# Rainbowboys/fm_spark

Hardware: AMD Instinct MI355X
Metric: FM SGD train samples/sec at k=16, 1/8 GPUs; % of HBM roofline (higher is better)
Workload: dtype f32; 1 GPU; c3: synthetic hashed 100M features, 39 nnz/row, k=16, batch 256K; num_features=100000000, k=16, batch_rows_per_gpu=262144, global_batch=262144, launch=single

## Files before the change

### fm_spark_amd/_native.py

```python

from __future__ import annotations

import ctypes as C
import os
from pathlib import Path

import numpy as np

_LIB_PATH = Path(__file__).resolve().parent / "lib" / "libfm_hip.so"

FM_OK = 0
FM_NOTHING_TO_DO = 1
FM_PARALLEL_NONE, FM_PARALLEL_SHARDED, FM_PARALLEL_REPLICATED = 0, 1, 2
FM_TRANSPORT_AUTO, FM_TRANSPORT_RCCL, FM_TRANSPORT_COPY = 0, 1, 2
FM_MAX_LOCAL = 16
FM_FUSE_DEFAULT, FM_FUSE_ON, FM_FUSE_OFF = 0, 1, -1
FM_WIRE_FP32, FM_WIRE_FP64 = 0, 1
FM_RANK_MAX_TOP = 1024
FM_RANK_SELECT_ALL, FM_RANK_SELECT_ONLY, FM_RANK_SELECT_EXCEPT = 0, 1, 2


class FMError(RuntimeError):
    """A negative return code of the C-ABI, with fm_last_error()'s message."""


class fm_config(C.Structure):
    _fields_ = [
        ("num_features", C.c_int64),
        ("k", C.c_int32),
        ("device", C.c_int32),
        ("seed", C.c_uint64),
        ("init_sd", C.c_double),
        ("w0", C.c_double),
        ("shard_index", C.c_int32),
        ("shard_count", C.c_int32),
        ("parallel", C.c_int32),
        ("n_gpus", C.c_int32),
        ("devices", C.c_int32 * FM_MAX_LOCAL),
        ("transport", C.c_int32),
        ("n_procs", C.c_int32),
        ("proc_rank", C.c_int32),
        ("comm_id", C.c_uint8 * 128),
        ("fuse_single", C.c_int32),
        ("xchg_chunks", C.c_int32),
        ("wire", C.c_int32),
    ]


class fm_csr(C.Structure):
    _fields_ = [
        ("n_rows", C.c_int64),
        ("nnz", C.c_int64),
        ("row_ptr", C.POINTER(C.c_int64)),
        ("col", C.POINTER(C.c_int32)),
        ("val", C.POINTER(C.c_double)),
        ("label", C.POINTER(C.c_double)),
    ]


class fm_step_out(C.Structure):
    _fields_ = [
        ("loss_sum", C.c_double),
        ("n_rows", C.c_int64),
        ("n_loss_rows", C.c_int64),
        ("n_unique", C.c_int64),
    ]


class fm_eval_out(C.Structure):
    _fields_ = [
        ("n_rows", C.c_int64),
        ("n_unlearned", C.c_int64),
        ("epoch", C.c_int64),
        ("sum_err", C.c_double),
        ("sum_abs_err", C.c_double),
        ("sum_sq_err", C.c_double),
    ]


_P = C.c_void_p
_I64P = C.POINTER(C.c_int64)
_I32P = C.POINTER(C.c_int32)
_DP = C.POINTER(C.c_double)

SIGNATURES = {
    "fm_create": (C.c_int, [C.POINTER(fm_config), C.POINTER(_P)]),
    "fm_destroy": (None, [_P]),
    "fm_last_error": (C.c_char_p, []),
    "fm_comm_unique_id": (C.c_int, [C.POINTER(C.c_uint8)]),
    "fm_set_stream": (C.c_int, [_P, _P]),
    "fm_sync": (C.c_int, [_P]),
    "fm_reserve": (C.c_int, [_P, C.c_int64, C.c_int64]),
    "fm_load_tables": (C.c_int, [_P, _I32P, C.c_int64, _DP, _DP]),
    "fm_init_random": (C.c_int, [_P, _I32P, C.c_int64]),
    "fm_init_random_range": (C.c_int, [_P, C.c_int64, C.c_int64]),
    "fm_export_tables": (C.c_int, [_P, _I32P, _DP, _DP, C.c_int64, _I64P]),
    "fm_export_rows": (C.c_int, [_P, _I32P, C.c_int64, _DP, _DP, C.POINTER(C.c_int8)]),
    "fm_num_present": (C.c_int64, [_P]),
    "fm_epoch": (C.c_int64, [_P]),
    "fm_batch_create": (C.c_int, [_P, C.POINTER(fm_csr), C.POINTER(_P)]),
    "fm_batch_destroy": (None, [_P]),
    "fm_batch_prepare": (C.c_int, [_P, _P]),
    "fm_batch_from_rows": (C.c_int, [_P, _P, _I64P, C.c_int64, C.POINTER(_P)]),
    "fm_batch_create_splits": (C.c_int, [_P, C.POINTER(fm_csr), C.c_int32, _I64P, C.POINTER(_P)]),
    "fm_batch_layout_splits": (C.c_int, [_P, C.POINTER(fm_csr), C.c_int32, _I64P, _I64P, C.POINTER(_P)]),
    "fm_batch_split_view": (C.c_int, [_P, _P, C.c_int32, C.POINTER(_P)]),
    "fm_fuse_active": (C.c_int32, [_P]),
    "fm_batch_rows": (C.c_int64, [_P]),
    "fm_batch_nnz": (C.c_int64, [_P]),
    "fm_step": (C.c_int, [_P, C.POINTER(fm_csr), C.c_int32, C.c_double, C.c_double, C.POINTER(fm_step_out)]),
    "fm_step_batch": (C.c_int, [_P, _P, C.c_int32, C.c_double, C.c_double, C.POINTER(fm_step_out)]),
    "fm_loss_history": (C.c_int, [_P, _DP, C.c_int64, _I64P]),
    "fm_predict": (C.c_int, [_P, C.POINTER(fm_csr), C.c_double, C.c_double, _DP]),
    "fm_predict_batch": (C.c_int, [_P, _P, C.c_double, C.c_double, _DP]),
    "fm_evaluate": (C.c_int, [_P, C.POINTER(fm_csr), C.c_double, C.c_double, _DP, C.POINTER(fm_eval_out)]),
    "fm_evaluate_batch": (C.c_int, [_P, _P, C.c_double, C.c_double, _DP, C.POINTER(fm_eval_out)]),
    "fm_eval_history": (C.c_int, [_P, C.POINTER(fm_eval_out), C.c_int64, _I64P]),
    "fm_rank_candidates": (C.c_int, [_P, C.POINTER(fm_csr), C.POINTER(fm_csr), C.c_int32, C.c_double, C.c_double,
                                     _I32P, _DP]),
    "fm_rank_batch": (C.c_int, [_P, _P, _P, C.c_int32, C.c_double, C.c_double, _I32P, _DP]),
    "fm_rank_candidates_select": (C.c_int, [_P, C.POINTER(fm_csr), C.POINTER(fm_csr), C.c_int32, _I64P, _I32P, C.c_int32,
                                            C.c_double, C.c_double, _I32P, _DP]),
    "fm_rank_batch_select": (C.c_int, [_P, _P, _P, C.c_int32, _I64P, _I32P, C.c_int32, C.c_double, C.c_double, _I32P,
                                       _DP]),
    "fm_rank_positions": (C.c_int, [_P, C.POINTER(fm_csr), C.POINTER(fm_csr), _I64P, _I32P, _I64P, _I32P, C.c_double,
                                    C.c_double, _I32P, _DP]),
    "fm_rank_positions_batch": (C.c_int, [_P, _P, _P, _I64P, _I32P, _I64P, _I32P, C.c_double, C.c_double, _I32P, _DP]),
    "fm_init_from_batch": (C.c_int, [_P, _P, _I64P]),
    "fm_loss_grad": (C.c_int, [_P, C.POINTER(fm_csr), _DP, _DP, _DP, _DP]),
    "fm_calc_loss_grad": (C.c_int, [_P, C.POINTER(fm_csr), C.c_double, C.c_uint64, _DP, _DP, _DP, _DP]),
    "fm_vector_sum_by_key": (C.c_int, [_P, _I32P, C.c_int64, _DP, C.c_int32, _I32P, _DP, _I64P]),
    "fm_profile_enable": (C.c_int, [_P, C.c_int32]),
    "fm_profile_read": (C.c_int, [_P, C.c_char_p, C.c_int64, _DP, _I64P, C.c_int64, _I64P]),
    "fm_profile_reset": (C.c_int, [_P]),
    "fm_device_bytes_live": (C.c_int64, []),
    "fm_device_allocs_live": (C.c_int64, []),
    "fm_read_libsvm": (C.c_int, [C.c_char_p, C.c_int64, C.c_int64, _DP, _I64P, _I32P, _DP, _I64P, _I64P, _I64P]),
    "fm_random_split": (
        C.c_int,
        [C.c_int32, _I64P, C.c_char_p, _DP, C.POINTER(C.c_int8), _I32P, _I64P, _I32P, _DP, _I64P,
         C.c_int32, _DP, C.c_int64, _I32P, _I64P, _I64P],
    ),
    "fm_xorshift_hash_seed": (C.c_int64, [C.c_int64]),
    "fm_murmur3_bytes_hash": (C.c_int32, [C.POINTER(C.c_uint8), C.c_int64, C.c_int32]),
    "fm_xorshift_next_doubles": (C.c_int, [C.c_int64, C.c_int64, _DP]),
    "fm_set_side_stream": (C.c_int, [_P, _P]),
    "fm_shard_route": (C.c_int, [_P, _P, _P, _P, _I64P]),
    "fm_shard_owner_prepare": (C.c_int, [_P, _P, _P, _P, C.c_int64, _I64P, _I64P]),
    "fm_shard_owner_forward": (C.c_int, [_P, _P, _P]),
    "fm_shard_combine": (C.c_int, [_P, _P, _P, _P]),
    "fm_shard_owner_update": (C.c_int, [_P, _P, _P, C.c_int32, C.c_double, C.c_double, C.c_int64]),
    "fm_repl_grad": (C.c_int, [_P, _P, _P]),
    "fm_repl_apply": (C.c_int, [_P, _P, C.c_int32, C.c_double, C.c_double, C.c_int64]),
    "fm_last_stats": (C.c_int, [_P, _DP, _I64P, _I64P]),
}

_lib = None


def lib_path() -> Path:
    return _LIB_PATH


def load() -> C.CDLL:
    global _lib
    if _lib is not None:
        return _lib
    path = Path(os.environ.get("FM_HIP_LIB") or _LIB_PATH)
    if not path.exists():
        raise FMError(f"{path} is missing: run __graft_entry__.build() (hipcc, gfx950)")
    if os.environ.get("FM_NO_TORCH_PRELOAD") != "1":
        try:
            import torch
        except Exception:
            pass
    lib = C.CDLL(str(path), mode=C.RTLD_GLOBAL)
    for name, (res, args) in SIGNATURES.items():
        fn = getattr(lib, name)
        fn.restype = res
        fn.argtypes = args
    _lib = lib
    return lib


def check(rc: int, what: str = "") -> int:
    if rc < 0:
        msg = load().fm_last_error()
        raise FMError(f"{what} failed ({rc}): {msg.decode() if msg else ''}")
    return rc


def ptr(a: np.ndarray, ctype):
    return a.ctypes.data_as(C.POINTER(ctype))


class CSRHost:

    def __init__(self, row_ptr, col, val, label):
        self.row_ptr = np.ascontiguousarray(row_ptr, dtype=np.int64)
        self.col = np.ascontiguousarray(col, dtype=np.int32)
        self.val = np.ascontiguousarray(val, dtype=np.float64)
        self.label = np.ascontiguousarray(label, dtype=np.float64)
        if len(self.row_ptr) == 0:
            self.row_ptr = np.zeros(1, dtype=np.int64)
        self.c = fm_csr(
            n_rows=len(self.label),
            nnz=len(self.col),
            row_ptr=ptr(self.row_ptr, C.c_int64),
            col=ptr(self.col, C.c_int32),
            val=ptr(self.val, C.c_double),
            label=ptr(self.label, C.c_double),
        )

    @property
    def n_rows(self) -> int:
        return len(self.label)

    @property
    def nnz(self) -> int:
        return len(self.col)
```

### fm_spark_amd/csrc/fm_capi.hip

```cpp
#include <algorithm>
#include <chrono>
#include <cstdlib>
#include <cmath>
#include <cstring>
#include <atomic>
#include <condition_variable>
#include <cstdio>
#include <functional>
#include <map>
#include <memory>
#include <set>
#include <thread>
#include <utility>

#include "fm_context.h"
#include "fm_hostpool.h"

namespace fmhip {

static thread_local std::string g_last_error;
void set_error(const std::string& msg) { g_last_error = msg; }

void report_stale(hipError_t e) {
  if (e == hipSuccess) return;
// ... 21 lines not shown
  if (p && !borrowed) {
    (void)hipFree(p);
    g_dev_bytes_live.fetch_sub((int64_t)bytes, std::memory_order_relaxed);
    g_dev_allocs_live.fetch_sub(1, std::memory_order_relaxed);
  }
  p = nullptr;
  bytes = 0;
  borrowed = false;
}

static int64_t chunk_count(int64_t n, int64_t min_per_thread) {
  return std::max<int64_t>(1, std::min<int64_t>(HostPool::get().threads(), n / std::max<int64_t>(min_per_thread, 1)));
}

template <class F>
static void parallel_chunks_t(int64_t n, int64_t T, F&& f) {
  if (T <= 1) {
    f(int64_t(0), int64_t(0), n);
    return;
  }
  const std::function<void(int)> job = [&](int t) { f((int64_t)t, n * t / T, n * (t + 1) / T); };
  HostPool::get().run((int)T, job);
}

template <class F>
static void parallel_chunks(int64_t n, int64_t min_per_thread, F&& f) {
  parallel_chunks_t(n, chunk_count(n, min_per_thread), [&](int64_t, int64_t lo, int64_t hi) { f(lo, hi); });
}

static bool selection_row_ptr(const int64_t* hrp, int64_t Bd, const int64_t* rows, int64_t n, int64_t* hrows,
                              int64_t* rp) {
  rp[0] = 0;
  const int64_t T = chunk_count(n, 8192);
  std::vector<int64_t> tot(T + 1, 0);
  std::atomic<int> bad{0};
  parallel_chunks_t(n, T, [&](int64_t t, int64_t lo, int64_t hi) {
    int64_t acc = 0;
    for (int64_t i = lo; i < hi; ++i) {
      const int64_t r = rows[i];
      if (r < 0 || r >= Bd) {
        bad.store(1);
        return;
      }
      hrows[i] = r;
      acc += hrp[r + 1] - hrp[r];
      rp[i + 1] = acc;
    }
    tot[t + 1] = acc;
  });
  if (bad.load()) return false;
  for (int64_t t = 0; t < T; ++t) tot[t + 1] += tot[t];
  if (T > 1)
    parallel_chunks_t(n, T, [&](int64_t t, int64_t lo, int64_t hi) {
      const int64_t add = tot[t];
      if (add)
        for (int64_t i = lo; i < hi; ++i) rp[i + 1] += add;
    });
  return true;
}

struct Staged {
  int64_t B = 0, N = 0, M = 0, max_id = -1, max_len = 0;
  size_t o_lab = 0, o_xoff = 0, o_col = 0, o_x = 0, bytes = 0;
  size_t o_extra = 0;
  int nruns = 0;
  int64_t run_at[16] = {0}, run_n[16] = {0};
  CsrImage view(void* base) const {
    char* p = reinterpret_cast<char*>(base);
    return {reinterpret_cast<int64_t*>(p), reinterpret_cast<double*>(p + o_lab), reinterpret_cast<int32_t*>(p + o_xoff),
            reinterpret_cast<uint32_t*>(p + o_col), reinterpret_cast<float*>(p + o_x)};
  }
  void enqueue_copies(void* dev, const void* pin, hipStream_t st) const {
    FM_HIP_CHECK(hipMemcpyAsync(dev, pin, bytes, hipMemcpyHostToDevice, st));
    for (int r = 0; r < nruns; ++r)
      if (run_n[r] > 0)
        FM_HIP_CHECK(hipMemcpyAsync(reinterpret_cast<char*>(dev) + o_x + sizeof(float) * run_at[r],
                                    reinterpret_cast<const char*>(pin) + o_x + sizeof(float) * run_at[r],
                                    sizeof(float) * run_n[r], hipMemcpyHostToDevice, st));
  }
};

void check_csr(const fm_csr* c) {
  FM_REQUIRE(c != nullptr, "null fm_csr");
  FM_REQUIRE(c->n_rows >= 0 && c->nnz >= 0, "negative n_rows / nnz");
  FM_REQUIRE(c->n_rows < (int64_t(1) << 31), "n_rows must be < 2^31");
  FM_REQUIRE(c->nnz < (int64_t(1) << 31), "nnz must be < 2^31 per batch");
  FM_REQUIRE(c->n_rows == 0 || (c->row_ptr && c->label), "null row_ptr / label");
  FM_REQUIRE(c->nnz == 0 || (c->col && c->val), "null col / val");
  const int64_t B = c->n_rows;
  if (B > 0) {
    FM_REQUIRE(c->row_ptr[0] == 0, "row_ptr[0] must be 0");
    FM_REQUIRE(c->row_ptr[B] == c->nnz, "row_ptr[n_rows] must equal nnz");
    for (int64_t i = 0; i < B; ++i) FM_REQUIRE(c->row_ptr[i] <= c->row_ptr[i + 1], "row_ptr must be non-decreasing");
  } else {
    FM_REQUIRE(c->nnz == 0, "nnz > 0 with n_rows == 0");
  }
}

static Staged stage_csr(fm_ctx* ctx, const fm_csr* c, bool check_range, Pinned& pin, size_t extra = 0) {
  check_csr(c);
  Staged g;
  const int64_t B = c->n_rows, N = c->nnz;
  g.B = B;
  g.N = N;
  g.o_lab = sizeof(int64_t) * (B + 1);
  g.o_xoff = g.o_lab + sizeof(double) * B;
  g.o_col = (g.o_xoff + sizeof(int32_t) * B + 15) / 16 * 16;
  g.o_x = (g.o_col + sizeof(uint32_t) * N + 15) / 16 * 16;
  g.o_extra = (g.o_x + sizeof(float) * N + 16 + 15) / 16 * 16;
  pin.ensure_slack(g.o_extra + extra);
  const CsrImage im = g.view(pin.p);
  if (B > 0) std::memcpy(im.row_ptr, c->row_ptr, sizeof(int64_t) * (B + 1));
  else im.row_ptr[0] = 0;
  const int64_t F = ctx->cfg.num_features;
  std::atomic<int> bad{0};
  std::atomic<int64_t> mx{-1}, mlen{0};
  std::atomic<int> nrun{0};
  parallel_chunks(B, 4096, [&](int64_t r0, int64_t r1) {
    const int64_t x0 = B > 0 ? c->row_ptr[r0] : 0;
    int64_t lmx = -1, m = x0, llen = 0;
    int lbad = 0;
    for (int64_t i = r0; i < r1; ++i) {
      im.label[i] = c->label[i];
      llen = std::max<int64_t>(llen, c->row_ptr[i + 1] - c->row_ptr[i]);
      im.xoff[i] = (int32_t)m;
      for (int64_t e = c->row_ptr[i]; e < c->row_ptr[i + 1]; ++e) {
        const int32_t id = c->col[e];
        if (id < 0) lbad |= 1;
        else if (check_range && id >= F) lbad |= 2;
        const float x = (float)c->val[e];
        const uint32_t valued = x != 1.0f;
        im.col[e] = (uint32_t)id | (valued << 31);
        im.x[m] = x;
        m += valued;
        lmx = std::max<int64_t>(lmx, id);
      }
    }
    const int ri = nrun.fetch_add(1);
    g.run_at[ri] = x0;
    g.run_n[ri] = m - x0;
    if (lbad) bad.fetch_or(lbad);
    int64_t cur = mx.load();
    while (lmx > cur && !mx.compare_exchange_weak(cur, lmx)) {
    }
    cur = mlen.load();
    while (llen > cur && !mlen.compare_exchange_weak(cur, llen)) {
    }
  });
  FM_REQUIRE(!(bad.load() & 1), "negative feature id");
  FM_REQUIRE(!(bad.load() & 2), "feature id >= num_features");
  g.nruns = nrun.load();
  for (int r = 0; r < g.nruns; ++r) g.M += g.run_n[r];
  g.bytes = g.o_col + sizeof(uint32_t) * N;
  g.max_id = mx.load();
  g.max_len = mlen.load();
  return g;
}

bool fuse_rule(const fm_ctx* ctx) {
  if (ctx->cfg.fuse_single == FM_FUSE_OFF || ctx->kp > 16) return false;
  const double table_bytes = (double)ctx->rows * ctx->stride * sizeof(float);
  return ctx->cfg.fuse_single == FM_FUSE_ON || table_bytes > 256.0 * 1024 * 1024;
}

static bool fuse_on(const fm_ctx* ctx) { return ctx->cfg.shard_count == 1 && fuse_rule(ctx); }

static bool batch_fits(const fm_batch* b, const Staged& g) {
  const BatchBytes z = batch_bytes(g.B, g.N);
  return b->dev.row_ptr.bytes >= z.row_ptr && b->dev.col.bytes >= z.col && b->dev.ent.bytes >= z.ent &&
         b->dev.xs.bytes >= z.xs && b->dev.label.bytes >= z.label && b->up.bytes >= g.o_x + sizeof(float) * g.N + 16;
}

static void copy_staged(fm_ctx* ctx, const Staged& g, const Pinned& pin, fm_batch* b, hipStream_t st) {
  b->owner = ctx;
  b->device = ctx->cfg.device;
  b->max_id = g.max_id;
  size_batch(b->dev, g.B, g.N);
  b->up.ensure_slack(g.o_x + sizeof(float) * g.N + 16);
  g.enqueue_copies(b->up.p, pin.p, st);
  launch_explode(g.view(b->up.p), g.B, g.N, b->dev, st);
}

void upload_batch(fm_ctx* ctx, const fm_csr* c, fm_batch* b, bool check_range) {
  FM_HIP_CHECK(hipStreamSynchronize(ctx->stream));
  const Staged g = stage_csr(ctx, c, check_range, ctx->up_pin);
  copy_staged(ctx, g, ctx->up_pin, b, ctx->stream);
  FM_HIP_CHECK(hipStreamSynchronize(ctx->stream));
}

fm_batch* host_batch(fm_ctx* ctx) {
  if (!ctx->host_batch) ctx->host_batch.reset(new fm_batch());
  return ctx->host_batch.get();
}

OutBatch out_batch(fm_ctx* ctx, const fm_batch* data, fm_batch** out, bool group) {
  OutBatch o;
  o.out = out;
  o.b = *out;
  if (o.b == nullptr) {
    o.fresh.reset(group ? new_group_batch(ctx) : new fm_batch());
    o.b = o.fresh.get();
    o.b->owner = ctx;
    o.b->device = ctx->cfg.device;
  } else {
    FM_REQUIRE(o.b->owner == ctx && o.b != data && !o.b->grp == !group && o.b->split_rows.empty(),
               "out must be a batch of this context other than data");
  }
  return o;
}

void wait_built(const fm_batch* b, hipStream_t st) {
  if (b->built) FM_HIP_CHECK(hipStreamWaitEvent(st, b->built, 0));
}

double* eval_next_slot(fm_ctx* ctx) {
  ctx->ensure_eval_hist(ctx->eval_n + 1);
  return ctx->eval_hist.as<double>() + kEvalRec * ctx->eval_n;
}

void eval_read(const double* rec, int64_t epoch, fm_eval_out* out) {
  out->n_rows = (int64_t)rec[0];
  out->n_unlearned = (int64_t)rec[1];
  out->epoch = epoch;
  out->sum_err = rec[2];
  out->sum_abs_err = rec[3];
  out->sum_sq_err = rec[4];
}

void eval_commit(fm_ctx* ctx, fm_eval_out* out) {
  const double* slot = ctx->eval_hist.as<double>() + kEvalRec * ctx->eval_n;
  ctx->eval_epoch.push_back(ctx->epoch);
  ctx->eval_n += 1;
  if (!out) return;
  ctx->pinned.ensure(64);
  FM_HIP_CHECK(hipMemcpyAsync(ctx->pinned.p, slot, sizeof(double) * kEvalRec, hipMemcpyDeviceToHost, ctx->stream));
  FM_HIP_CHECK(hipStreamSynchronize(ctx->stream));
  eval_read(reinterpret_cast<const double*>(ctx->pinned.p), ctx->epoch, out);
}

void reserve_work(fm_ctx* ctx, int64_t B, int64_t N) {
  StepWork& w = ctx->work;
  w.S.ensure_slack(sizeof(float) * (size_t)std::max<int64_t>(B, 1) * s_rec_floats(ctx->kp));
  w.yl.ensure_slack(sizeof(float2) * (size_t)std::max<int64_t>(B, 1));
  w.sort.ensure(std::max<int64_t>(N, 1));
  const int64_t nranges = (N + 255) / 256;
  w.part.ensure_slack(sizeof(double) * (size_t)std::max<int64_t>(nranges, 1) * 2 * (ctx->kp + 2));
  w.ucnt.ensure_slack(sizeof(uint32_t) * (size_t)std::max<int64_t>((N + 1023) / 1024, 1));
  w.loss_part.ensure(sizeof(double2) * kLossPartBlocks);
}

}

namespace {

int step_impl(fm_ctx* ctx, fm_batch* b, int32_t t, double step_size, double reg_param, fm_step_out* out,
              float* emit = nullptr) {
  FM_REQUIRE(b != nullptr, "null batch");
  FM_REQUIRE(b->owner == ctx, "batch belongs to another context");
  FM_REQUIRE(ctx->cfg.shard_count == 1, "sharded contexts step through the fm_shard_* entry points");
  FM_REQUIRE(b->split_rows.empty(), "a dataset made by fm_batch_create_splits is stepped through its split views");
  if (emit) FM_HIP_CHECK(hipMemsetAsync(emit, 0, sizeof(float) * (size_t)ctx->rows * (ctx->kp + 4), ctx->stream));
  if (b->dev.n_rows == 0) return FM_NOTHING_TO_DO;
  FM_REQUIRE(t >= 1, "iteration index t must be >= 1");
  FM_REQUIRE(std::isfinite(step_size) && std::isfinite(reg_param), "non-finite step size / regParam");
  const int64_t B = b->dev.n_rows, N = b->dev.nnz;
  reserve_work(ctx, B, N);
  ctx->ensure_hist(ctx->epoch + 1);
  StepParams p;
  p.n_rows = B;
  p.eta = step_size / std::sqrt((double)t);
  p.lam = p.eta * reg_param;
  p.m = (double)B;
  p.scale_v = p.eta / (double)B;
  p.epoch = ctx->epoch;
  p.cumE = ctx->cum_host.back();
  p.cum_next = p.cumE + p.lam;
  p.w0 = ctx->cfg.w0;
  const TableView T = ctx->view();
  wait_built(b, ctx->stream);
  int64_t nfwd = 0;
  const uint32_t* skeys = nullptr;
  const uint2* sents = nullptr;
  const bool prepared = b->prepared;
  const bool fused = prepared && b->split;
  FM_REQUIRE(!(fused && emit), "a batch prepared for the fused step cannot feed fm_repl_grad");
  FM_REQUIRE(ctx->epoch < (1 << 29), "epoch count beyond the multi tags' range (2^29 steps)");
  if (prepared) {
    skeys = b->skeys.as<uint32_t>();
    sents = b->sents.as<uint2>();
  } else {
    FM_HIP_CHECK(hipEventRecord(ctx->ev_fork, ctx->stream));
    FM_HIP_CHECK(hipStreamWaitEvent(ctx->side, ctx->ev_fork, 0));
    hipEvent_t es = ctx->prof_begin(ctx->side);
    radix_sort_pairs64(ctx->work.sort, b->dev.col.as<uint32_t>(), b->dev.ent.as<uint2>(), N, bits_for(ctx->rows - 1),
                       ctx->side, &skeys, &sents);
    ctx->prof_end("sort", es, ctx->side);
    FM_HIP_CHECK(hipEventRecord(ctx->ev_join, ctx->side));
  }
  hipEvent_t e0 = nullptr;
  FwdOut fx{};
  if (fused) {
    FM_HIP_CHECK(hipStreamWaitEvent(ctx->stream, b->ready, 0));
    e0 = ctx->prof_begin(ctx->stream);
    launch_split(b->fkeys.as<uint32_t>(), b->fents.as<uint2>(), N, ctx->split_work, b->skeys.as<uint32_t>(),
                 b->sents.as<uint2>(), b->split_n.as<int64_t>(), ctx->stream, T, p.epoch);
    ctx->prof_end("split", e0, ctx->stream);
    fx.mode = kTrainFused;
  }
  e0 = ctx->prof_begin(ctx->stream);
  launch_forward(T, b->dev, ctx->work, p, ctx->stream, &nfwd, nullptr, fused ? &fx : nullptr);
  ctx->prof_end("forward", e0, ctx->stream);
  if (!fused) FM_HIP_CHECK(hipStreamWaitEvent(ctx->stream, prepared ? b->ready : ctx->ev_join, 0));
  e0 = ctx->prof_begin(ctx->stream);
  double* stats = ctx->loss_hist.as<double>() + 3 * (int64_t)ctx->epoch;
  launch_segment_update(T, b->dev, ctx->work, p, skeys, sents, nfwd, stats, ctx->stream, emit,
                        fused ? b->split_n.as<int64_t>() : nullptr);
  if (!prepared) FM_HIP_CHECK(hipEventRecord(ctx->ev_upd_done, ctx->stream));
  if (b->last_use) FM_HIP_CHECK(hipEventRecord(b->last_use, ctx->stream));
  b->prepared = false;
  ctx->prof_end("update", e0, ctx->stream);
  if (emit) return FM_OK;
  ctx->epoch += 1;
  ctx->cum_host.push_back(p.cum_next);
  if (out) {
    ctx->pinned.ensure(64);
    FM_HIP_CHECK(hipMemcpyAsync(ctx->pinned.p, stats, sizeof(double) * 3, hipMemcpyDeviceToHost, ctx->stream));
    FM_HIP_CHECK(hipStreamSynchronize(ctx->stream));
    const double* h = reinterpret_cast<const double*>(ctx->pinned.p);
    out->loss_sum = h[0];
    out->n_loss_rows = (int64_t)h[1];
    out->n_unique = (int64_t)h[2];
    out->n_rows = B;
  }
  return FM_OK;
}

}

extern "C" {

const char* fm_last_error(void) { return g_last_error.c_str(); }

int64_t fm_device_bytes_live(void) { return g_dev_bytes_live.load(std::memory_order_relaxed); }
int64_t fm_device_allocs_live(void) { return g_dev_allocs_live.load(std::memory_order_relaxed); }

int fm_create(const fm_config* cfg, fm_ctx** out) {
  return guarded_free([&]() -> int {
    FM_REQUIRE(cfg && out, "null argument");
    FM_REQUIRE(cfg->wire == FM_WIRE_FP32 || cfg->wire == FM_WIRE_FP64, "wire must be FM_WIRE_FP32 or FM_WIRE_FP64");
    FM_REQUIRE(cfg->wire != FM_WIRE_FP64 || cfg->parallel != FM_PARALLEL_REPLICATED,
               "wire = FM_WIRE_FP64 applies to the sharded step only: the replicated gradient all-reduce is fp32");
    if (cfg->parallel != FM_PARALLEL_NONE) return group_create(cfg, out);
    FM_REQUIRE(cfg->num_features >= 1 && cfg->num_features <= (int64_t(1) << 31), "num_features must be in [1, 2^31]");
    FM_REQUIRE(cfg->k >= 1 && cfg->k <= 256, "dimFactorization must be in [1, 256]");
    FM_REQUIRE(cfg->shard_count >= 1 && cfg->shard_index >= 0 && cfg->shard_index < cfg->shard_count,
               "bad shard_index / shard_count");
    FM_REQUIRE(cfg->init_sd >= 0.0, "init_sd must be >= 0");
    FM_REQUIRE(cfg->fuse_single == FM_FUSE_DEFAULT || cfg->fuse_single == FM_FUSE_ON || cfg->fuse_single == FM_FUSE_OFF,
               "fuse_single must be FM_FUSE_DEFAULT, FM_FUSE_ON or FM_FUSE_OFF");
    int ndev = 0;
    FM_HIP_CHECK(hipGetDeviceCount(&ndev));
    FM_REQUIRE(cfg->device >= 0 && cfg->device < ndev, "device ordinal out of range");
    FM_HIP_CHECK(hipSetDevice(cfg->device));
    std::unique_ptr<fm_ctx> c(new fm_ctx());
    c->cfg = *cfg;
    c->kp = (cfg->k + 3) / 4 * 4;
    c->rows = (cfg->num_features - cfg->shard_index + cfg->shard_count - 1) / cfg->shard_count;
    FM_HIP_CHECK(hipStreamCreateWithFlags(&c->stream, hipStreamNonBlocking));
    c->own_stream = true;
    FM_HIP_CHECK(hipStreamCreateWithFlags(&c->side_own, hipStreamNonBlocking));
    c->side = c->side_own;
    FM_HIP_CHECK(hipEventCreateWithFlags(&c->ev_fork, hipEventDisableTiming));
    FM_HIP_CHECK(hipEventCreateWithFlags(&c->ev_join, hipEventDisableTiming));
    FM_HIP_CHECK(hipEventCreateWithFlags(&c->ev_upd_done, hipEventDisableTiming));
    FM_HIP_CHECK(hipEventRecord(c->ev_upd_done, c->stream));
    c->stride = record_stride(c->kp);
    c->rec.ensure(sizeof(float) * (size_t)std::max<int64_t>(c->rows, 1) * c->stride);
    c->ensure_hist(4096);
    launch_table_reset(c->view(), c->stream);
    FM_HIP_CHECK(hipStreamSynchronize(c->stream));
    *out = c.release();
    return FM_OK;
  });
}

void fm_destroy(fm_ctx* ctx) {
  if (!ctx) return;
  try {
    delete ctx;
  } catch (...) {
  }
}

int fm_set_stream(fm_ctx* ctx, void* s) {
  if (ctx && ctx->group) {
    if (ctx->cfg.n_gpus != 1) {
      set_error("fm_set_stream on a context with several local ranks");
      return FM_ERR_ARG;
    }
    return fm_set_stream(group_member0(ctx), s);
  }
  return guarded(ctx, [&]() -> int {
    FM_HIP_CHECK(hipStreamSynchronize(ctx->stream));
    if (ctx->own_stream && ctx->stream) FM_HIP_CHECK(hipStreamDestroy(ctx->stream));
    ctx->stream = reinterpret_cast<hipStream_t>(s);
    ctx->own_stream = false;
    return FM_OK;
  });
}

int fm_set_side_stream(fm_ctx* ctx, void* s) {
  if (ctx && ctx->group) {
    if (ctx->cfg.n_gpus != 1) {
      set_error("fm_set_side_stream on a context with several local ranks");
      return FM_ERR_ARG;
    }
    return fm_set_side_stream(group_member0(ctx), s);
  }
  return guarded(ctx, [&]() -> int {
    FM_HIP_CHECK(hipStreamSynchronize(ctx->side));
    ctx->side = s ? reinterpret_cast<hipStream_t>(s) : ctx->side_own;
    return FM_OK;
  });
}

int fm_sync(fm_ctx* ctx) {
  return guarded(ctx, [&]() -> int {
    if (ctx->group) return group_sync(ctx);
    FM_HIP_CHECK(hipStreamSynchronize(ctx->stream));
    FM_HIP_CHECK(hipStreamSynchronize(ctx->side));
    if (ctx->copy_stream) FM_HIP_CHECK(hipStreamSynchronize(ctx->copy_stream));
    return FM_OK;
  });
}

int fm_reserve(fm_ctx* ctx, int64_t max_rows, int64_t max_nnz) {
  return guarded(ctx, [&]() -> int {
    FM_REQUIRE(max_rows >= 0 && max_nnz >= 0, "negative reserve");
    if (ctx->group) return group_reserve(ctx, max_rows, max_nnz);
    reserve_work(ctx, max_rows, max_nnz);
    return FM_OK;
  });
}

int fm_load_tables(fm_ctx* ctx, const int32_t* ids, int64_t n, const double* w, const double* V) {
  return guarded(ctx, [&]() -> int {
    FM_REQUIRE(n >= 0, "negative n");
    if (n == 0) return FM_OK;
    if (ctx->group) return group_load_tables(ctx, ids, n, w, V);
    FM_REQUIRE(ids && w && V, "null argument");
    for (int64_t i = 0; i < n; ++i)
      FM_REQUIRE(ids[i] >= 0 && ids[i] < ctx->cfg.num_features, "id out of [0, num_features)");
    DevBuf di, dw, dv;
    di.ensure(sizeof(int32_t) * n);
    dw.ensure(sizeof(double) * n);
    dv.ensure(sizeof(double) * n * ctx->cfg.k);
    FM_HIP_CHECK(hipMemcpy(di.p, ids, sizeof(int32_t) * n, hipMemcpyHostToDevice));
    FM_HIP_CHECK(hipMemcpy(dw.p, w, sizeof(double) * n, hipMemcpyHostToDevice));
    FM_HIP_CHECK(hipMemcpy(dv.p, V, sizeof(double) * n * ctx->cfg.k, hipMemcpyHostToDevice));
    launch_load_rows(ctx->view(), di.as<int32_t>(), n, dw.as<double>(), dv.as<double>(), ctx->epoch,
                     ctx->cum_host.back(), ctx->stream);
    FM_HIP_CHECK(hipStreamSynchronize(ctx->stream));
    return FM_OK;
  });
}

int fm_init_random(fm_ctx* ctx, const int32_t* ids, int64_t n) {
  return guarded(ctx, [&]() -> int {
    FM_REQUIRE(n >= 0, "negative n");
    if (n == 0) return FM_OK;
    FM_REQUIRE(ids, "null ids");
    if (ctx->group) return group_init_random(ctx, ids, n, 0, 0);
    for (int64_t i = 0; i < n; ++i)
      FM_REQUIRE(ids[i] >= 0 && ids[i] < ctx->cfg.num_features, "id out of [0, num_features)");
    DevBuf di;
    di.ensure(sizeof(int32_t) * n);
    FM_HIP_CHECK(hipMemcpy(di.p, ids, sizeof(int32_t) * n, hipMemcpyHostToDevice));
    launch_init_random(ctx->view(), di.as<int32_t>(), n, 0, ctx->cfg.seed, ctx->cfg.init_sd, ctx->epoch,
                       ctx->cum_host.back(), ctx->stream);
    FM_HIP_CHECK(hipStreamSynchronize(ctx->stream));
    return FM_OK;
  });
}

int fm_init_random_range(fm_ctx* ctx, int64_t b, int64_t e) {
  return guarded(ctx, [&]() -> int {
    FM_REQUIRE(b >= 0 && e >= b && e <= ctx->cfg.num_features, "bad id range");
    if (ctx->group) return group_init_random(ctx, nullptr, 0, b, e);
    launch_init_random(ctx->view(), nullptr, e - b, b, ctx->cfg.seed, ctx->cfg.init_sd, ctx->epoch,
                       ctx->cum_host.back(), ctx->stream);
    FM_HIP_CHECK(hipStreamSynchronize(ctx->stream));
    return FM_OK;
  });
}

int64_t fm_num_present(fm_ctx* ctx) {
  int64_t n = -1;
  int rc = guarded(ctx, [&]() -> int {
    if (ctx->group) {
      n = group_num_present(ctx);
      return FM_OK;
    }
    DevBuf d;
    d.ensure(sizeof(int64_t));
    launch_count_present(ctx->view(), d.as<int64_t>(), ctx->stream);
    FM_HIP_CHECK(hipMemcpyAsync(&n, d.p, sizeof(int64_t), hipMemcpyDeviceToHost, ctx->stream));
    FM_HIP_CHECK(hipStreamSynchronize(ctx->stream));
    return FM_OK;
  });
  return rc == FM_OK ? n : rc;
}

int64_t fm_epoch(fm_ctx* ctx) { return ctx ? ctx->epoch : -1; }

int fm_export_tables(fm_ctx* ctx, int32_t* ids, double* w, double* V, int64_t cap, int64_t* n) {
  return guarded(ctx, [&]() -> int {
    FM_REQUIRE(n != nullptr && cap >= 0, "bad arguments");
    if (ctx->group) return group_export_tables(ctx, ids, w, V, cap, n);
    launch_flush(ctx->view(), ctx->epoch, ctx->cum_host.back(), ctx->stream);
    FM_HIP_CHECK(hipStreamSynchronize(ctx->stream));
    const int k = ctx->cfg.k, kp = ctx->kp, S = ctx->stride;
    const int64_t chunk_rows = std::max<int64_t>(1, (int64_t(64) << 20) / (4 * S));
    std::vector<float> hv;
    int64_t cnt = 0, o = 0;
    const bool fill = cap > 0;
    for (int64_t r0 = 0; r0 < ctx->rows; r0 += chunk_rows) {
      const int64_t r1 = std::min(ctx->rows, r0 + chunk_rows);
      hv.resize((size_t)(r1 - r0) * S);
      FM_HIP_CHECK(hipMemcpy(hv.data(), ctx->rec.as<float>() + r0 * S, sizeof(float) * (r1 - r0) * S,
                             hipMemcpyDeviceToHost));
      for (int64_t i = r0; i < r1; ++i) {
        const float* row = hv.data() + (size_t)(i - r0) * S;
        RowHdr hd;
        std::memcpy(&hd, row + kp, sizeof(RowHdr));
        if (hd.t < 0) continue;
        ++cnt;
        if (!fill) continue;
        FM_REQUIRE(o < cap && ids && w && V, "export buffers too small or null");
        ids[o] = (int32_t)(i * ctx->cfg.shard_count + ctx->cfg.shard_index);
        w[o] = hd.w;
        for (int f = 0; f < k; ++f) V[o * k + f] = row[f];
        ++o;
      }
    }
    *n = cnt;
    return FM_OK;
  });
}

int fm_export_rows(fm_ctx* ctx, const int32_t* ids, int64_t n, double* w, double* V, int8_t* present) {
  return guarded(ctx, [&]() -> int {
    FM_REQUIRE(n >= 0, "negative n");
    if (n == 0) return FM_OK;
    FM_REQUIRE(ids && w && V && present, "null argument");
    if (ctx->group) return group_export_rows(ctx, ids, n, w, V, present);
    const int R = ctx->cfg.shard_count;
    for (int64_t i = 0; i < n; ++i) {
      FM_REQUIRE(ids[i] >= 0 && ids[i] < ctx->cfg.num_features, "id out of [0, num_features)");
      FM_REQUIRE(ids[i] % R == ctx->cfg.shard_index, "id not owned by this shard");
    }
    const int k = ctx->cfg.k;
    DevBuf di, dw, dv, dp;
    di.ensure(sizeof(int32_t) * n);
    dw.ensure(sizeof(double) * n);
    dv.ensure(sizeof(double) * n * k);
    dp.ensure(sizeof(int8_t) * n);
    FM_HIP_CHECK(hipMemcpyAsync(di.p, ids, sizeof(int32_t) * n, hipMemcpyHostToDevice, ctx->stream));
    launch_gather_rows(ctx->view(), di.as<int32_t>(), n, ctx->cum_host.back(), dw.as<double>(), dv.as<double>(),
                       dp.as<int8_t>(), ctx->stream);
    FM_HIP_CHECK(hipMemcpyAsync(w, dw.p, sizeof(double) * n, hipMemcpyDeviceToHost, ctx->stream));
    FM_HIP_CHECK(hipMemcpyAsync(V, dv.p, sizeof(double) * n * k, hipMemcpyDeviceToHost, ctx->stream));
    FM_HIP_CHECK(hipMemcpyAsync(present, dp.p, sizeof(int8_t) * n, hipMemcpyDeviceToHost, ctx->stream));
    FM_HIP_CHECK(hipStreamSynchronize(ctx->stream));
    return FM_OK;
  });
}

int fm_batch_create(fm_ctx* ctx, const fm_csr* csr, fm_batch** out) {
  return guarded(ctx, [&]() -> int {
    FM_REQUIRE(out != nullptr, "null out");
    if (ctx->group) return group_batch_create(ctx, csr, out);
    std::unique_ptr<fm_batch> b(new fm_batch());
    upload_batch(ctx, csr, b.get(), true);
    b->host_rp.assign(csr->row_ptr, csr->row_ptr + csr->n_rows + 1);
    *out = b.release();
    return FM_OK;
  });
}

void fm_batch_destroy(fm_batch* b) {
  if (!b) return;
  try {
    delete b;
  } catch (...) {
  }
}

int fm_batch_prepare(fm_ctx* ctx, fm_batch* b) {
  return guarded(ctx, [&]() -> int {
    FM_REQUIRE(b != nullptr && b->owner == ctx, "batch belongs to another context");
    if (ctx->group) return group_batch_prepare(ctx, b);
    FM_REQUIRE(ctx->cfg.shard_count == 1, "fm_batch_prepare is for single-table contexts");
    FM_REQUIRE(b->split_rows.empty(), "a dataset made by fm_batch_create_splits is prepared through its split views");
    const int64_t N = b->dev.nnz;
    if (N == 0) return FM_OK;
    b->ensure_events(ctx->stream);
    b->skeys.ensure_slack(sizeof(uint32_t) * N);
    b->sents.ensure_slack(sizeof(uint2) * N);
    FM_HIP_CHECK(hipStreamWaitEvent(ctx->side, ctx->ev_upd_done, 0));
    FM_HIP_CHECK(hipStreamWaitEvent(ctx->side, b->last_use, 0));
    wait_built(b, ctx->side);
    hipEvent_t es = ctx->prof_begin(ctx->side);
    const uint32_t* sk = nullptr;
    const uint2* sv = nullptr;
    b->split = fuse_on(ctx);
    const int kb = bits_for(ctx->rows - 1);
    const uint32_t* col = b->dev.col.as<uint32_t>();
    const uint2* ent = b->dev.ent.as<uint2>();
    if (b->split) {
      b->split_n.ensure(2 * sizeof(int64_t));
      b->fkeys.ensure_slack(sizeof(uint32_t) * N);
      b->fents.ensure_slack(sizeof(uint2) * N);
      radix_sort_pairs64(ctx->work.sort, col, ent, N, kb, ctx->side, &sk, &sv, b->fkeys.as<uint32_t>(),
                         b->fents.as<uint2>());
    } else {
      radix_sort_pairs64(ctx->work.sort, col, ent, N, kb, ctx->side, &sk, &sv, b->skeys.as<uint32_t>(),
                         b->sents.as<uint2>());
    }
    ctx->prof_end("sort", es, ctx->side);
    FM_HIP_CHECK(hipEventRecord(b->ready, ctx->side));
    b->prepared = true;
    return FM_OK;
  });
}

int fm_batch_from_rows(fm_ctx* ctx, const fm_batch* data, const int64_t* rows, int64_t n, fm_batch** out) {
  return guarded(ctx, [&]() -> int {
    FM_REQUIRE(out != nullptr && data != nullptr, "null argument");
    FM_REQUIRE(data->owner == ctx, "data belongs to another context");
    FM_REQUIRE(n >= 0 && n < (int64_t(1) << 31), "n out of range");
    FM_REQUIRE(n == 0 || rows != nullptr, "null rows");
    if (ctx->group) return group_batch_from_rows(ctx, data, rows, n, out);
    const int64_t Bd = data->dev.n_rows;
    FM_REQUIRE((int64_t)data->host_rp.size() == Bd + 1,
               "data must be a batch made by fm_batch_create");
    OutBatch res = out_batch(ctx, data, out, false);
    fm_batch* b = res.b;
    b->detach_view();
    b->ensure_events(ctx->stream);
    if (!b->built) {
      FM_HIP_CHECK(hipEventCreateWithFlags(&b->built, hipEventDisableTiming));
      FM_HIP_CHECK(hipEventCreateWithFlags(&b->sel_copied, hipEventDisableTiming));
      FM_HIP_CHECK(hipEventRecord(b->sel_copied, ctx->side));
    }
    FM_HIP_CHECK(hipEventSynchronize(b->sel_copied));
    const size_t img = sizeof(int64_t) * (2 * (size_t)n + 1);
    b->sel_pin.ensure_slack(img);
    int64_t* hrows = reinterpret_cast<int64_t*>(b->sel_pin.p);
    int64_t* rp = hrows + n;
    FM_REQUIRE(selection_row_ptr(data->host_rp.data(), Bd, rows, n, hrows, rp), "row index out of [0, rows of data)");
    const int64_t N = rp[n];
    FM_REQUIRE(N < (int64_t(1) << 31), "nnz must be < 2^31 per batch");
    if (!ctx->copy_stream) FM_HIP_CHECK(hipStreamCreateWithFlags(&ctx->copy_stream, hipStreamNonBlocking));
    hipStream_t gs = ctx->copy_stream;
    FM_HIP_CHECK(hipStreamWaitEvent(gs, b->last_use, 0));
    if (b->sh && b->sh->last_use) FM_HIP_CHECK(hipStreamWaitEvent(gs, b->sh->last_use, 0));
    if (b->prepared && b->ready) FM_HIP_CHECK(hipStreamWaitEvent(gs, b->ready, 0));
    b->max_id = data->max_id;
    size_batch(b->dev, n, N);
    b->up.ensure_slack(img + 16);
    FM_HIP_CHECK(hipMemcpyAsync(b->up.p, b->sel_pin.p, img, hipMemcpyHostToDevice, gs));
    FM_HIP_CHECK(hipEventRecord(b->sel_copied, gs));
    if (n > 0) {
      const int64_t* up = b->up.as<int64_t>();
      launch_select_rows(data->dev, up, up + n, n, b->dev, gs);
    } else {
      FM_HIP_CHECK(hipMemcpyAsync(b->dev.row_ptr.p, b->up.as<int64_t>(), sizeof(int64_t), hipMemcpyDeviceToDevice, gs));
    }
    FM_HIP_CHECK(hipEventRecord(b->built, gs));
    b->prepared = false;
    b->host_rp.clear();
    res.commit();
    return FM_OK;
  });
}

int fm_batch_create_splits(fm_ctx* ctx, const fm_csr* csr, int32_t n_splits, const int64_t* split_rows,
                           fm_batch** out) {
  return guarded(ctx, [&]() -> int {
    FM_REQUIRE(out != nullptr && csr != nullptr, "null argument");
    FM_REQUIRE(n_splits >= 1 && split_rows != nullptr, "n_splits must be >= 1");
    FM_REQUIRE(split_rows[0] == 0 && split_rows[n_splits] == csr->n_rows, "split_rows must run from 0 to n_rows");
    for (int32_t i = 0; i < n_splits; ++i) FM_REQUIRE(split_rows[i] <= split_rows[i + 1], "split_rows must be non-decreasing");
    if (ctx->group) return group_batch_create_splits(ctx, csr, n_splits, split_rows, out);
    std::unique_ptr<fm_batch> b(new fm_batch());
    upload_batch(ctx, csr, b.get(), true);
    b->host_rp.assign(csr->row_ptr, csr->row_ptr + csr->n_rows + 1);
    b->split_rows.assign(split_rows, split_rows + n_splits + 1);
    DevBuf dsr;
    dsr.ensure(sizeof(int64_t) * (n_splits + 1));
    FM_HIP_CHECK(hipMemcpyAsync(dsr.p, split_rows, sizeof(int64_t) * (n_splits + 1), hipMemcpyHostToDevice, ctx->stream));
    b->split_rp.ensure(sizeof(int64_t) * (csr->n_rows + n_splits));
    launch_split_rebase(b->dev, dsr.as<int64_t>(), n_splits, b->split_rp.as<int64_t>(), ctx->stream);
    FM_HIP_CHECK(hipStreamSynchronize(ctx->stream));
    *out = b.release();
    return FM_OK;
  });
}

int fm_batch_layout_splits(fm_ctx* ctx, const fm_csr* csr, int32_t n_splits, const int64_t* split_rows,
                           const int64_t* order, fm_batch** out) {
  return guarded(ctx, [&]() -> int {
    FM_REQUIRE(out != nullptr && csr != nullptr, "null argument");
    FM_REQUIRE(n_splits >= 1 && split_rows != nullptr, "n_splits must be >= 1");
    FM_REQUIRE(split_rows[0] == 0, "split_rows must start at 0");
    for (int32_t i = 0; i < n_splits; ++i) FM_REQUIRE(split_rows[i] <= split_rows[i + 1], "split_rows must be non-decreasing");
    const int64_t n = split_rows[n_splits];
    FM_REQUIRE(n < (int64_t(1) << 31), "laid-out rows must be < 2^31");
    FM_REQUIRE(n == 0 || order != nullptr, "null order");
    if (ctx->group) return group_batch_layout_splits(ctx, csr, n_splits, split_rows, order, out);
    std::unique_ptr<fm_batch> b(new fm_batch());
    FM_HIP_CHECK(hipStreamSynchronize(ctx->stream));
    const size_t extra = sizeof(int64_t) * (2 * (size_t)n + 1 + (size_t)n_splits + 1);
    const Staged g = stage_csr(ctx, csr, true, ctx->up_pin, extra);
    const int64_t D = g.B;
    int64_t* hord = reinterpret_cast<int64_t*>(reinterpret_cast<char*>(ctx->up_pin.p) + g.o_extra);
    int64_t* rp = hord + n;
    int64_t* hsr = rp + n + 1;
    FM_REQUIRE(selection_row_ptr(csr->row_ptr, D, order, n, hord, rp), "row index out of [0, n_rows of csr)");
    const int64_t N = rp[n];
    FM_REQUIRE(N < (int64_t(1) << 31), "nnz must be < 2^31 per batch");
    std::copy(split_rows, split_rows + n_splits + 1, hsr);
    hipStream_t st = ctx->stream;
    b->owner = ctx;
    b->device = ctx->cfg.device;
    b->max_id = g.max_id;
    size_batch(b->dev, n, N);
    b->split_rp.ensure(sizeof(int64_t) * (n + n_splits));
    b->up.ensure(g.o_extra + extra);
    g.enqueue_copies(b->up.p, ctx->up_pin.p, st);
    int64_t* dord = reinterpret_cast<int64_t*>(b->up.as<char>() + g.o_extra);
    FM_HIP_CHECK(hipMemcpyAsync(dord, hord, extra, hipMemcpyHostToDevice, st));
    launch_layout_splits(g.view(b->up.p), dord, dord + n, dord + 2 * n + 1, n_splits, n, b->dev, b->split_rp.as<int64_t>(),
                         st);
    b->host_rp.assign(rp, rp + n + 1);
    b->split_rows.assign(split_rows, split_rows + n_splits + 1);
    FM_HIP_CHECK(hipStreamSynchronize(st));
    b->up.release();
    *out = b.release();
    return FM_OK;
  });
}

int fm_batch_split_view(fm_ctx* ctx, const fm_batch* data, int32_t split, fm_batch** out) {
  return guarded(ctx, [&]() -> int {
    FM_REQUIRE(out != nullptr && data != nullptr, "null argument");
    FM_REQUIRE(data->owner == ctx, "data belongs to another context");
    if (ctx->group) return group_batch_split_view(ctx, data, split, out);
    const int64_t ns = (int64_t)data->split_rows.size() - 1;
    FM_REQUIRE(ns >= 1, "data must be a dataset made by fm_batch_create_splits");
    FM_REQUIRE(split >= 0 && split < ns, "split index out of range");
    OutBatch res = out_batch(ctx, data, out, false);
    fm_batch* b = res.b;
    if (!b->view_of) {
      for (hipEvent_t e : {b->last_use, b->ready, b->built, b->sel_copied})
        if (e) FM_HIP_CHECK(hipEventSynchronize(e));
      for (DevBuf* d : {&b->dev.row_ptr, &b->dev.col, &b->dev.ent, &b->dev.xs, &b->dev.label, &b->up}) d->release();
    }
    b->ensure_events(ctx->stream);
    const int64_t r0 = data->split_rows[split], r1 = data->split_rows[split + 1];
    const int64_t e0 = data->host_rp[r0], e1 = data->host_rp[r1];
    b->view_of = data;
    b->dev.n_rows = r1 - r0;
    b->dev.nnz = e1 - e0;
    b->dev.row_ptr.borrow(data->split_rp.as<int64_t>() + r0 + split, sizeof(int64_t) * (r1 - r0 + 1));
    b->dev.col.borrow(data->dev.col.as<uint32_t>() + e0, sizeof(uint32_t) * (e1 - e0));
    b->dev.ent.borrow(data->dev.ent.as<uint2>() + e0, sizeof(uint2) * (e1 - e0));
    b->dev.xs.borrow(data->dev.xs.as<float>() + e0, sizeof(float) * (e1 - e0));
    b->dev.label.borrow(data->dev.label.as<double>() + r0, sizeof(double) * (r1 - r0));
    b->max_id = data->max_id;
    b->prepared = false;
    b->host_rp.clear();
    res.commit();
    return FM_OK;
  });
}

int32_t fm_fuse_active(fm_ctx* ctx) {
  if (!ctx) return -1;
  if (ctx->group) return 0;
  return fuse_on(ctx) ? 1 : 0;
}

int64_t fm_batch_rows(const fm_batch* b) { return b ? b->dev.n_rows : -1; }
int64_t fm_batch_nnz(const fm_batch* b) { return b ? b->dev.nnz : -1; }

int fm_step_batch(fm_ctx* ctx, fm_batch* batch, int32_t t, double step_size, double reg_param,
                  fm_step_out* out) {
  return guarded(ctx, [&]() -> int {
    if (ctx->group) return group_step_batch(ctx, batch, t, step_size, reg_param, out);
    return step_impl(ctx, batch, t, step_size, reg_param, out);
  });
}

int fm_step(fm_ctx* ctx, const fm_csr* csr, int32_t t, double step_size, double reg_param, fm_step_out* out) {
  return guarded(ctx, [&]() -> int {
    FM_REQUIRE(csr != nullptr, "null batch");
    if (csr->n_rows == 0) {
      if (out) {
        out->loss_sum = 0.0;
        out->n_rows = 0;
        out->n_loss_rows = 0;
        out->n_unique = 0;
      }
      if (!ctx->group) return FM_NOTHING_TO_DO;
    }
    if (ctx->group) return group_step(ctx, csr, t, step_size, reg_param, out);
    HostSlot& h = ctx->hslot[ctx->hnext];
    ctx->hnext ^= 1;
    if (!h.batch) {
      h.batch.reset(new fm_batch());
      FM_HIP_CHECK(hipEventCreateWithFlags(&h.copied, hipEventDisableTiming));
      FM_HIP_CHECK(hipEventCreateWithFlags(&h.consumed, hipEventDisableTiming));
      FM_HIP_CHECK(hipEventRecord(h.copied, ctx->stream));
      FM_HIP_CHECK(hipEventRecord(h.consumed, ctx->stream));
    }
    if (!ctx->copy_stream) FM_HIP_CHECK(hipStreamCreateWithFlags(&ctx->copy_stream, hipStreamNonBlocking));
    FM_HIP_CHECK(hipEventSynchronize(h.copied));
    const Staged g = stage_csr(ctx, csr, true, h.pin);
    if (!batch_fits(h.batch.get(), g)) FM_HIP_CHECK(hipEventSynchronize(h.consumed));
    FM_HIP_CHECK(hipStreamWaitEvent(ctx->copy_stream, h.consumed, 0));
    copy_staged(ctx, g, h.pin, h.batch.get(), ctx->copy_stream);
    FM_HIP_CHECK(hipEventRecord(h.copied, ctx->copy_stream));
    FM_HIP_CHECK(hipStreamWaitEvent(ctx->stream, h.copied, 0));
    const int rc = step_impl(ctx, h.batch.get(), t, step_size, reg_param, out);
    FM_HIP_CHECK(hipEventRecord(h.consumed, ctx->stream));
    return rc;
  });
}

int fm_loss_history(fm_ctx* ctx, double* loss, int64_t cap, int64_t* n) {
  return guarded(ctx, [&]() -> int {
    FM_REQUIRE(n != nullptr, "null n");
    if (ctx->group) return group_loss_history(ctx, loss, cap, n);
    *n = ctx->epoch;
    if (cap == 0 || ctx->epoch == 0) return FM_OK;
    FM_REQUIRE(loss != nullptr, "null loss buffer");
    const int64_t m = std::min<int64_t>(cap, ctx->epoch);
    std::vector<double> h(3 * m);
    FM_HIP_CHECK(hipMemcpyAsync(h.data(), ctx->loss_hist.p, sizeof(double) * 3 * m, hipMemcpyDeviceToHost, ctx->stream));
    FM_HIP_CHECK(hipStreamSynchronize(ctx->stream));
    for (int64_t i = 0; i < m; ++i) loss[i] = h[3 * i];
    return FM_OK;
  });
}

int fm_predict(fm_ctx* ctx, const fm_csr* csr, double lo, double hi, double* pred) {
  return guarded(ctx, [&]() -> int {
    FM_REQUIRE(csr != nullptr && (csr->n_rows == 0 || pred), "null argument");
    if (ctx->group) return group_predict(ctx, csr, lo, hi, pred);
    if (csr->n_rows == 0) return FM_OK;
    fm_batch* b = host_batch(ctx);
    upload_batch(ctx, csr, b, false);
    DevBuf dp;
    dp.ensure(sizeof(double) * csr->n_rows);
    launch_predict(ctx->view(), b->dev, ctx->cum_host.back(), ctx->cfg.w0, lo, hi, dp.as<double>(), ctx->stream);
    FM_HIP_CHECK(hipMemcpyAsync(pred, dp.p, sizeof(double) * csr->n_rows, hipMemcpyDeviceToHost, ctx->stream));
    FM_HIP_CHECK(hipStreamSynchronize(ctx->stream));
    return FM_OK;
  });
}

int fm_predict_batch(fm_ctx* ctx, fm_batch* b, double lo, double hi, double* pred) {
  return guarded(ctx, [&]() -> int {
    FM_REQUIRE(b != nullptr && b->owner == ctx, "batch belongs to another context");
    if (ctx->group) return group_predict_batch(ctx, b, lo, hi, pred);
    const int64_t B = b->dev.n_rows;
    FM_REQUIRE(B == 0 || pred, "null argument");
    if (B == 0) return FM_OK;
    DevBuf dp;
    dp.ensure(sizeof(double) * B);
    wait_built(b, ctx->stream);
    hipEvent_t e0 = ctx->prof_begin(ctx->stream);
    launch_predict(ctx->view(), b->dev, ctx->cum_host.back(), ctx->cfg.w0, lo, hi, dp.as<double>(), ctx->stream);
    ctx->prof_end("predict", e0, ctx->stream);
    FM_HIP_CHECK(hipMemcpyAsync(pred, dp.p, sizeof(double) * B, hipMemcpyDeviceToHost, ctx->stream));
    FM_HIP_CHECK(hipStreamSynchronize(ctx->stream));
    return FM_OK;
  });
}

static int evaluate_impl(fm_ctx* ctx, fm_batch* b, double lo, double hi, double* pred, fm_eval_out* out) {
  const int64_t B = b->dev.n_rows;
  hipStream_t st = ctx->stream;
  double* slot = eval_next_slot(ctx);
  if (pred) ctx->eval_pred.ensure_slack(sizeof(double) * B);
  wait_built(b, st);
  hipEvent_t e0 = ctx->prof_begin(st);
  const int64_t nblk = launch_evaluate(ctx->view(), b->dev, ctx->work, ctx->cum_host.back(), ctx->cfg.w0, lo, hi,
                                       pred ? ctx->eval_pred.as<double>() : nullptr, st);
  hipEvent_t ef = ctx->prof_begin(st);
  launch_eval_fold(ctx->work.eval_part.as<double>(), nblk, slot, st);
  ctx->prof_end("eval_fold", ef, st);
  ctx->prof_end("evaluate", e0, st);
  if (b->last_use) FM_HIP_CHECK(hipEventRecord(b->last_use, st));
  if (pred) FM_HIP_CHECK(hipMemcpyAsync(pred, ctx->eval_pred.p, sizeof(double) * B, hipMemcpyDeviceToHost, st));
  eval_commit(ctx, out);
  return FM_OK;
}

int fm_evaluate(fm_ctx* ctx, const fm_csr* csr, double lo, double hi, double* pred, fm_eval_out* out) {
  return guarded(ctx, [&]() -> int {
    FM_REQUIRE(csr != nullptr && out != nullptr, "null argument");
    *out = fm_eval_out{};
    if (ctx->group) return group_evaluate(ctx, csr, lo, hi, pred, out);
    if (csr->n_rows == 0) return FM_NOTHING_TO_DO;
    fm_batch* b = host_batch(ctx);
    upload_batch(ctx, csr, b, false);
    return evaluate_impl(ctx, b, lo, hi, pred, out);
  });
}

int fm_evaluate_batch(fm_ctx* ctx, fm_batch* b, double lo, double hi, double* pred, fm_eval_out* out) {
  return guarded(ctx, [&]() -> int {
    FM_REQUIRE(b != nullptr && b->owner == ctx, "batch belongs to another context");
    FM_REQUIRE(out != nullptr || pred == nullptr, "pred needs out: an evaluation that only enqueues returns no predictions");
    FM_REQUIRE(b->split_rows.empty(), "a dataset made by fm_batch_create_splits is evaluated by split");
    if (out) *out = fm_eval_out{};
    if (ctx->group) return group_evaluate_batch(ctx, b, lo, hi, pred, out);
    if (b->dev.n_rows == 0) return FM_NOTHING_TO_DO;
    return evaluate_impl(ctx, b, lo, hi, pred, out);
  });
}

// ... 570 lines not shown
```

### fm_spark_amd/csrc/fm_context.h

```cpp
#pragma once

#include <map>
#include <memory>
#include <utility>

#include "fm_internal.h"

namespace fmhip {

struct Pinned {
  void* p = nullptr;
  size_t bytes = 0;
  void ensure(size_t n) {
    if (n <= bytes && p) return;
    if (p) (void)hipHostFree(p);
    p = nullptr;
    FM_HIP_CHECK(hipHostMalloc(&p, n, hipHostMallocDefault));
    bytes = n;
  }
  void ensure_slack(size_t n) {
    if (n > bytes || !p) ensure(n + n / 8 + 4096);
  }
  ~Pinned() {
    if (p) (void)hipHostFree(p);
  }
};

struct HostSlot {
  std::unique_ptr<fm_batch> batch;
  Pinned pin;
  hipEvent_t copied = nullptr;
  hipEvent_t consumed = nullptr;
};

struct ProfEntry {
  double ms = 0.0;
  int64_t n = 0;
};

struct ShardBatchState {
  DevBuf pairidx;
  std::vector<int64_t> pairs_out;
  int64_t route_nnz = -1;
  DevBuf poff;
  int64_t loss_blocks = 0;
  hipEvent_t fwd_e0 = nullptr;
  bool combined = false;
  bool prepared = false;
  const uint32_t* recv_slot = nullptr;
  const uint2* recv_ent = nullptr;
  int64_t n = 0, P = 0;
  Pinned pin_off;
  DevBuf src_off;
  DevBuf pair_ptr;
  DevBuf skeys, sents;
  hipEvent_t ready_fwd = nullptr;
  hipEvent_t ready_upd = nullptr;
  hipEvent_t last_use = nullptr;
  void release(int device) {
    (void)hipSetDevice(device);
    for (hipEvent_t e : {ready_fwd, ready_upd, last_use})
      if (e) (void)hipEventSynchronize(e);
    for (hipEvent_t e : {ready_fwd, ready_upd, last_use})
      if (e) (void)hipEventDestroy(e);
    ready_fwd = ready_upd = last_use = nullptr;
    for (DevBuf* b : {&pairidx, &poff, &src_off, &pair_ptr, &skeys, &sents}) b->release();
  }
};

struct Group;
struct GroupBatch;
struct GroupDeleter {
  void operator()(Group* g) const;
};
struct GroupBatchDeleter {
  void operator()(GroupBatch* g) const;
};

}

using namespace fmhip;

struct fm_batch {
  fm_ctx* owner = nullptr;
  int device = 0;
  BatchDev dev;
  int64_t max_id = -1;
  DevBuf up;
  DevBuf skeys, sents;
  DevBuf fkeys, fents;
  DevBuf split_n;
  bool split = false;
  hipEvent_t ready = nullptr;
  hipEvent_t last_use = nullptr;
  void ensure_events(hipStream_t main) {
    if (ready) return;
    FM_HIP_CHECK(hipEventCreateWithFlags(&ready, hipEventDisableTiming));
    FM_HIP_CHECK(hipEventCreateWithFlags(&last_use, hipEventDisableTiming));
    FM_HIP_CHECK(hipEventRecord(last_use, main));
  }
  bool prepared = false;
  std::vector<int64_t> host_rp;
  Pinned sel_pin;
  hipEvent_t sel_copied = nullptr, built = nullptr;
  std::vector<int64_t> split_rows;
  DevBuf split_rp;
  const fm_batch* view_of = nullptr;
  void detach_view() {
    if (!view_of) return;
    for (DevBuf* d : {&dev.row_ptr, &dev.col, &dev.ent, &dev.xs, &dev.label}) d->release();
    view_of = nullptr;
  }
  std::unique_ptr<ShardBatchState> sh;
  std::unique_ptr<GroupBatch, GroupBatchDeleter> grp;
  ~fm_batch() {
    grp.reset();
    (void)hipSetDevice(device);
    if (sh) sh->release(device);
    for (hipEvent_t e : {ready, last_use, sel_copied, built})
      if (e) (void)hipEventSynchronize(e);
    for (hipEvent_t e : {ready, last_use, sel_copied, built})
      if (e) (void)hipEventDestroy(e);
    detach_view();
    split_rp.release();
    skeys.release();
    sents.release();
    fkeys.release();
    fents.release();
    split_n.release();
    up.release();
    dev.row_ptr.release();
    dev.col.release();
    dev.ent.release();
    dev.xs.release();
    dev.label.release();
  }
};

struct fm_ctx {
  std::mutex mu;
  fm_config cfg{};
  std::unique_ptr<Group, GroupDeleter> group;
  int32_t kp = 0;
  int64_t rows = 0;
  hipStream_t stream = nullptr;
  bool own_stream = false;
  hipStream_t side = nullptr;
  hipStream_t side_own = nullptr;
  hipEvent_t ev_fork = nullptr, ev_join = nullptr;
  hipEvent_t ev_upd_done = nullptr;
  DevBuf rec;
  int32_t stride = 0;
  std::vector<double> cum_host{0.0};
  int32_t epoch = 0;
  DevBuf loss_hist;
  int64_t hist_cap = 0;
  DevBuf eval_hist;
  int64_t eval_cap = 0, eval_n = 0;
  std::vector<int64_t> eval_epoch;
  std::vector<fm_eval_out> eval_host;
  DevBuf eval_pred;
  StepWork work;
  Pinned pinned;
  Pinned up_pin;
  std::unique_ptr<fm_batch> host_batch;
  std::unique_ptr<fm_batch> host_batch2;
  RankWork rank;
  HostSlot hslot[2];
  int hnext = 0;
  hipStream_t copy_stream = nullptr;
  bool prof = false;
  std::vector<std::pair<std::string, std::pair<hipEvent_t, hipEvent_t>>> pending;
  std::vector<hipEvent_t> free_events;
  std::map<std::string, ProfEntry> prof_acc;
  std::vector<std::string> prof_order;
  DevBuf sh_okey;
  DevBuf sh_mask;
  DevBuf sh_tcnt;
  DevBuf sh_tot;
  DevBuf sh_pay;
  DevBuf sh_skey;
  DevBuf sh_ent2;
  SortWork side_sort;
  SortWork route_sort;
  SplitWork split_work;
  Pinned side_pinned;
  DevBuf repl_cnt;
  bool repl_pending = false;

  TableView view() const {
    TableView T;
    T.rec = rec.as<float>();
    T.rows = rows;
    T.stride = stride;
    T.k = cfg.k;
    T.kp = kp;
    T.shard_count = cfg.shard_count;
    T.shard_index = cfg.shard_index;
    return T;
  }

  hipEvent_t get_event() {
    if (!free_events.empty()) {
      hipEvent_t e = free_events.back();
      free_events.pop_back();
      return e;
    }
    hipEvent_t e;
    FM_HIP_CHECK(hipEventCreate(&e));
    return e;
  }

  hipEvent_t prof_begin(hipStream_t s) {
    if (!prof) return nullptr;
    hipEvent_t e = get_event();
    FM_HIP_CHECK(hipEventRecord(e, s));
    return e;
  }
  void prof_end(const char* name, hipEvent_t e0, hipStream_t s) {
    if (!prof || !e0) return;
    hipEvent_t e1 = get_event();
    FM_HIP_CHECK(hipEventRecord(e1, s));
    pending.push_back({name, {e0, e1}});
    if (pending.size() > 4096) resolve_profile();
  }
  void prof_host(const char* name, double ms) {
    if (!prof) return;
    auto it = prof_acc.find(name);
    if (it == prof_acc.end()) {
      prof_order.push_back(name);
      it = prof_acc.emplace(name, ProfEntry{}).first;
    }
    it->second.ms += ms;
    it->second.n += 1;
  }
  void resolve_profile() {
    if (pending.empty()) return;
    FM_HIP_CHECK(hipStreamSynchronize(stream));
    FM_HIP_CHECK(hipStreamSynchronize(side));
    for (auto& pe : pending) {
      float ms = 0.f;
      FM_HIP_CHECK(hipEventElapsedTime(&ms, pe.second.first, pe.second.second));
      auto it = prof_acc.find(pe.first);
      if (it == prof_acc.end()) {
        prof_order.push_back(pe.first);
        it = prof_acc.emplace(pe.first, ProfEntry{}).first;
      }
      it->second.ms += ms;
      it->second.n += 1;
      free_events.push_back(pe.second.first);
      free_events.push_back(pe.second.second);
    }
    pending.clear();
  }

  void ensure_hist(int64_t need) {
    if (need <= hist_cap) return;
    int64_t c = std::max<int64_t>(4096, hist_cap);
    while (c < need) c *= 2;
    FM_HIP_CHECK(hipStreamSynchronize(stream));
    DevBuf nb;
    nb.ensure(sizeof(double) * 3 * c);
    FM_HIP_CHECK(hipMemset(nb.p, 0, sizeof(double) * 3 * c));
    if (hist_cap > 0)
      FM_HIP_CHECK(hipMemcpy(nb.p, loss_hist.p, sizeof(double) * 3 * hist_cap, hipMemcpyDeviceToDevice));
    loss_hist = std::move(nb);
    hist_cap = c;
  }

  void ensure_eval_hist(int64_t need) {
    if (need <= eval_cap) return;
    int64_t c = std::max<int64_t>(4096, eval_cap);
    while (c < need) c *= 2;
    FM_HIP_CHECK(hipStreamSynchronize(stream));
    DevBuf nb;
    nb.ensure(sizeof(double) * kEvalRec * c);
    FM_HIP_CHECK(hipMemset(nb.p, 0, sizeof(double) * kEvalRec * c));
    if (eval_cap > 0)
      FM_HIP_CHECK(hipMemcpy(nb.p, eval_hist.p, sizeof(double) * kEvalRec * eval_cap, hipMemcpyDeviceToDevice));
    eval_hist = std::move(nb);
    eval_cap = c;
  }

  ~fm_ctx() {
    group.reset();
    (void)hipSetDevice(cfg.device);
    if (stream) (void)hipStreamSynchronize(stream);
    if (copy_stream) (void)hipStreamSynchronize(copy_stream);
    for (auto& h : hslot) {
      if (h.copied) (void)hipEventDestroy(h.copied);
      if (h.consumed) (void)hipEventDestroy(h.consumed);
    }
    if (copy_stream) (void)hipStreamDestroy(copy_stream);
    for (auto& pe : pending) {
      (void)hipEventDestroy(pe.second.first);
      (void)hipEventDestroy(pe.second.second);
    }
    for (auto e : free_events) (void)hipEventDestroy(e);
    if (side) (void)hipStreamSynchronize(side);
    if (ev_fork) (void)hipEventDestroy(ev_fork);
    if (ev_join) (void)hipEventDestroy(ev_join);
    if (ev_upd_done) (void)hipEventDestroy(ev_upd_done);
    if (side_own) (void)hipStreamSynchronize(side_own);
    if (side_own) (void)hipStreamDestroy(side_own);
    rec.release();
    loss_hist.release();
    eval_hist.release();
    DevBuf* bufs[] = {&work.S, &work.yl, &work.loss_part, &work.part, &work.ucnt, &work.eval_part, &eval_pred,
                      &work.sort.keys_a, &work.sort.keys_b, &work.sort.vals_a, &work.sort.vals_b,
                      &work.sort.counts, &work.sort.digit_tot, &side_sort.keys_a, &side_sort.keys_b,
                      &side_sort.vals_a, &side_sort.vals_b, &side_sort.counts, &side_sort.digit_tot,
                      &route_sort.keys_a, &route_sort.keys_b, &route_sort.vals_a, &route_sort.vals_b,
                      &route_sort.counts, &route_sort.digit_tot,
                      &sh_okey, &sh_mask, &sh_tcnt, &sh_tot, &sh_pay, &sh_skey, &sh_ent2, &repl_cnt,
                      &split_work.cnt, &split_work.off, &rank.sum_u, &rank.sum_c, &rank.cnt_u, &rank.cnt_c,
                      &rank.bias_u, &rank.bias_c, &rank.lkey, &rank.lidx, &rank.out_idx, &rank.out_score,
                      &rank.sel_ptr, &rank.sel_rows, &rank.tgt_ptr, &rank.tgt_rows, &rank.position, &rank.pos_score};
    for (auto* b : bufs) b->release();
    if (own_stream && stream) (void)hipStreamDestroy(stream);
  }
};


namespace fmhip {
void report_stale(hipError_t e);

template <class F>
int guarded(fm_ctx* ctx, F&& f) {
  if (!ctx) {
    set_error("null fm_ctx");
    return FM_ERR_ARG;
  }
  std::lock_guard<std::mutex> lk(ctx->mu);
  int prev_dev = -1;
  if (hipGetDevice(&prev_dev) != hipSuccess) prev_dev = -1;
  struct Restore {
    int d;
    ~Restore() {
      if (d >= 0) (void)hipSetDevice(d);
    }
  } restore{prev_dev};
  try {
    report_stale(hipGetLastError());
    FM_HIP_CHECK(hipSetDevice(ctx->cfg.device));
    return f();
  } catch (const Error& e) {
    set_error(e.msg);
    return e.code;
  } catch (const std::bad_alloc&) {
    set_error("host allocation failed");
    return FM_ERR_OOM;
  } catch (const std::exception& e) {
    set_error(e.what());
    return FM_ERR_HIP;
  } catch (...) {
    set_error("unknown error");
    return FM_ERR_HIP;
  }
}

template <class F>
int guarded_free(F&& f) {
  try {
    return f();
  } catch (const Error& e) {
    set_error(e.msg);
    return e.code;
  } catch (const std::bad_alloc&) {
    set_error("host allocation failed");
    return FM_ERR_OOM;
  } catch (const std::exception& e) {
    set_error(e.what());
    return FM_ERR_HIP;
  } catch (...) {
    set_error("unknown error");
    return FM_ERR_HIP;
  }
}

inline int bits_for(int64_t max_value) {
  int b = 1;
  while (b < 63 && (int64_t(1) << b) <= max_value) ++b;
  return b;
}

bool fuse_rule(const fm_ctx* ctx);
void wait_built(const fm_batch* b, hipStream_t st);
void upload_batch(fm_ctx* ctx, const fm_csr* c, fm_batch* b, bool check_range);
void check_csr(const fm_csr* c);
struct OutBatch {
  fm_batch* b = nullptr;
  std::unique_ptr<fm_batch> fresh;
  fm_batch** out = nullptr;
  void commit() {
    if (fresh) *out = fresh.release();
// ... 49 lines not shown
```

### fm_spark_amd/csrc/fm_internal.h

```cpp
#pragma once

#include <hip/hip_runtime.h>

#include <cstdint>
#include <mutex>
#include <string>
#include <vector>

#include "../../include/fm_hip.h"

namespace fmhip {

void set_error(const std::string& msg);

struct Error {
  int code;
  std::string msg;
};

#define FM_HIP_CHECK(expr)                                                            \
  do {                                                                                \
    hipError_t _e = (expr);                                                           \
    if (_e != hipSuccess)                                                             \
      throw ::fmhip::Error{_e == hipErrorOutOfMemory ? FM_ERR_OOM : FM_ERR_HIP,        \
                           std::string(#expr) + ": " + hipGetErrorString(_e)};        \
  } while (0)

#define FM_REQUIRE(cond, msg)                                \
  do {                                                       \
    if (!(cond)) throw ::fmhip::Error{FM_ERR_ARG, (msg)};    \
  } while (0)

struct alignas(16) RowHdr {
  float w;
  int32_t t;
  double cum;
};

struct TableView {
  float* rec;
  int64_t rows;
  int32_t k;
  int32_t kp;
  int32_t stride;
  int32_t shard_count;
  int32_t shard_index;
  __host__ __device__ float* v(int64_t slot) const { return rec + slot * stride; }
  __host__ __device__ RowHdr* hdr(int64_t slot) const {
    return reinterpret_cast<RowHdr*>(rec + slot * stride + kp);
  }
};

inline int32_t record_stride(int32_t kp) {
  const int32_t need = kp + 4;
  if (need <= 16) return 16;
  if (need <= 32) return 32;
  return (need + 31) / 32 * 32;
}

struct DevBuf {
  void* p = nullptr;
  size_t bytes = 0;
  bool borrowed = false;
  DevBuf() = default;
  DevBuf(const DevBuf&) = delete;
  DevBuf& operator=(const DevBuf&) = delete;
  DevBuf(DevBuf&& o) noexcept : p(o.p), bytes(o.bytes), borrowed(o.borrowed) {
    o.p = nullptr;
    o.bytes = 0;
    o.borrowed = false;
  }
  DevBuf& operator=(DevBuf&& o) noexcept {
    if (this != &o) {
      release();
      p = o.p;
      bytes = o.bytes;
      borrowed = o.borrowed;
      o.p = nullptr;
      o.bytes = 0;
      o.borrowed = false;
    }
    return *this;
  }
  ~DevBuf() { release(); }
  void borrow(const void* q, size_t n) {
    release();
    p = const_cast<void*>(q);
    bytes = n;
    borrowed = true;
  }
  void ensure(size_t n);
  void ensure_slack(size_t n) {
    if (n > bytes || !p) ensure(n + n / 8 + 4096);
  }
  void release();
  template <class T>
  T* as() const { return reinterpret_cast<T*>(p); }
};

struct SortWork {
  DevBuf keys_a, keys_b, vals_a, vals_b, counts, digit_tot;
  int64_t cap = 0;
  void ensure(int64_t n);
};

void radix_sort_pairs(SortWork& w, const uint32_t* keys_in, const uint32_t* vals_in, int64_t n,
                      int key_bits, hipStream_t st, const uint32_t** keys_out,
                      const uint32_t** vals_out);
void radix_sort_pairs64(SortWork& w, const uint32_t* keys_in, const uint2* vals_in, int64_t n,
                        int key_bits, hipStream_t st, const uint32_t** keys_out,
                        const uint2** vals_out, uint32_t* final_keys = nullptr,
                        uint2* final_vals = nullptr);
void radix_sort_pairs64_bits(SortWork& w, const uint32_t* keys_in, const uint2* vals_in, int64_t n, int lo_bit,
                             int hi_bit, hipStream_t st, uint32_t* final_keys, uint2* final_vals);

struct BatchDev {
  int64_t n_rows = 0, nnz = 0;
  DevBuf row_ptr, col, ent, label;
  DevBuf xs;
};
struct BatchBytes {
  size_t row_ptr, col, ent, xs, label;
};
inline BatchBytes batch_bytes(int64_t B, int64_t N) {
  const size_t n = (size_t)(N > 4 ? N : 4), b = (size_t)(B > 4 ? B : 4);
  return {sizeof(int64_t) * (size_t)(B + 1), sizeof(uint32_t) * n + 16, sizeof(uint2) * n + 16, sizeof(float) * n + 16,
          sizeof(double) * b + 16};
}
inline void size_batch(BatchDev& d, int64_t B, int64_t N) {
  const BatchBytes z = batch_bytes(B, N);
  d.n_rows = B;
  d.nnz = N;
  d.row_ptr.ensure_slack(z.row_ptr);
  d.col.ensure_slack(z.col);
  d.ent.ensure_slack(z.ent);
  d.xs.ensure_slack(z.xs);
  d.label.ensure_slack(z.label);
}

inline bool s_rec_yl(int kp) { return kp <= 16; }
inline int s_rec_floats(int kp) { return s_rec_yl(kp) ? (kp + 2 <= 16 ? 16 : 32) : kp; }

struct StepWork {
  DevBuf S;
  DevBuf yl;
  DevBuf loss_part;
  DevBuf part;
  DevBuf ucnt;
  DevBuf eval_part;
  SortWork sort;
};

struct StepParams {
  int64_t n_rows;
  double eta;
  double lam;
  double scale_v;
  double m;
  int32_t epoch;
  double cumE;
  double cum_next;
  double w0;
};

enum FwdMode : int {
  kTrain = 0, kPartial = 1, kPredict = 2, kLossGrad = 3, kTrainFused = 4, kPartial64 = 5, kSummary = 6, kEvaluate = 7
};
constexpr int kEvalRec = 5;
struct FwdOut {
  int mode = kTrain;
  double lo = 0.0, hi = 0.0;
  double* pred = nullptr;
  double* loss = nullptr;
  double* dw = nullptr;
  double* dv = nullptr;
  int32_t* absent = nullptr;
  uint32_t* pcount = nullptr;
  double* summary = nullptr;
  const int64_t* ch_off = nullptr;
  int32_t ch_R = 0, ch_c = 0, ch_C = 1;
  double fill_sd = 0.0;
  uint64_t fill_seed = 0;
  StepParams sp{};
};
constexpr int kMaxChunkSources = 64;
void launch_forward(const TableView& T, const BatchDev& b, StepWork& w, const StepParams& p,
                    hipStream_t st, int64_t* n_fwd_blocks, float* partial_out = nullptr,
                    const FwdOut* pred = nullptr, bool partial_wide = false);
struct FwdLaunchRec {
  int32_t mode, gs, team, u;
  int32_t chunk, chunks;
  int64_t blocks, rows;
};
constexpr int kFwdLogCap = 256;
struct FwdConsts {
  int32_t grid, block, fuse_ns, fuse_u;
};
void set_forward_grid_cap(int64_t blocks);
void clear_forward_log();
int read_forward_log(FwdLaunchRec* out, int cap);
FwdConsts forward_consts();

struct SegSource {
  const float* S;
  int64_t s_stride;
  const float2* yl;
  int64_t yl_stride;
  const int64_t* n_dev = nullptr;
};
void launch_segment_update(const TableView& T, const BatchDev& b, StepWork& w, const StepParams& p,
                           const uint32_t* skeys, const uint2* sents, int64_t n_fwd_blocks,
                           double* stats_out, hipStream_t st, float* emit = nullptr, const int64_t* n_dev = nullptr);
struct SplitWork {
  DevBuf cnt, off;
};
void launch_split(const uint32_t* skeys, const uint2* sents, int64_t N, SplitWork& sw, uint32_t* mkeys, uint2* ments,
                  int64_t* n_out, hipStream_t st, const TableView& tag_T, int32_t epoch);
void launch_segment_update(const TableView& T, int64_t N, const SegSource& src, StepWork& w, const StepParams& p,
                           const uint32_t* skeys, const uint2* sents, int64_t n_loss_blocks, double* stats_out,
                           hipStream_t st, float* emit = nullptr);
struct UpdGeometry {
  int32_t wave_entries;
  int32_t group_entries;
  int32_t block_entries;
  int32_t paired;
  int32_t comb_lanes;
  int32_t comb_cols;
  int32_t split_chunk;
  int32_t scan_round_chunks;
};
UpdGeometry update_geometry(int kp);
constexpr int kReplApplyBlocks = 256 * 16;
constexpr int kLossPartBlocks = 256 * 8;
void launch_repl_apply(const TableView& T, const float* grad, const StepParams& p, uint32_t* blk_touched,
                       double* n_touched, hipStream_t st);

void launch_init_random(const TableView& T, const int32_t* ids, int64_t n, int64_t id_begin,
                        uint64_t seed, double sd, int32_t epoch, double cumE, hipStream_t st);
void launch_load_rows(const TableView& T, const int32_t* ids, int64_t n, const double* w,
                      const double* V, int32_t epoch, double cumE, hipStream_t st);
void launch_flush(const TableView& T, int32_t epoch, double cumE, hipStream_t st);
void launch_gather_rows(const TableView& T, const int32_t* ids, int64_t n, double cumE, double* w, double* V,
                        int8_t* present, hipStream_t st);
void launch_table_reset(const TableView& T, hipStream_t st);
void launch_predict(const TableView& T, const BatchDev& b, double cumE, double w0, double lo, double hi,
                    double* pred, hipStream_t st);
int64_t launch_evaluate(const TableView& T, const BatchDev& b, StepWork& w, double cumE, double w0, double lo, double hi,
                        double* pred, hipStream_t st);
void launch_eval_fold(const double* part, int64_t n_blocks, double* out, hipStream_t st);
void launch_summary(const TableView& T, const BatchDev& b, double cumE, double* summary, uint32_t* present,
                    hipStream_t st);
void launch_init_entries(const TableView& T, const uint32_t* col, int64_t n, uint64_t seed, double sd,
                         int32_t epoch, double cumE, hipStream_t st);
void launch_loss_grad(const TableView& T, const BatchDev& b, double cumE, double w0, double* pred,
                      double* loss, double* dw, double* dv, int32_t* absent_flag, hipStream_t st,
                      double fill_sd = 0.0, uint64_t fill_seed = 0);
void launch_segment_sum(const uint32_t* skeys, const uint32_t* svals, int64_t n, const double* vecs,
                        int32_t k, uint32_t* run_index, int32_t* out_keys, double* out_sums,
                        int64_t* n_out_dev, hipStream_t st);
void launch_count_present(const TableView& T, int64_t* out, hipStream_t st);
struct CsrImage {
  int64_t* row_ptr;
  double* label;
  int32_t* xoff;
  uint32_t* col;
  float* x;
};
void launch_explode(const CsrImage& in, int64_t B, int64_t N, BatchDev& dst, hipStream_t st);
void launch_layout_splits(const CsrImage& src, const int64_t* order, const int64_t* row_ptr_in, const int64_t* split_rows,
                          int32_t n_splits, int64_t B, BatchDev& dst, int64_t* split_rp, hipStream_t st);

struct RankWork {
  DevBuf sum_u, sum_c;
  DevBuf cnt_u, cnt_c;
  DevBuf bias_u, bias_c;
  DevBuf lkey, lidx;
  DevBuf out_idx, out_score;
  DevBuf sel_ptr, sel_rows;
  DevBuf tgt_ptr, tgt_rows;
  DevBuf position, pos_score;
};
struct RankSelect {
  int32_t mode = FM_RANK_SELECT_ALL;
  const int64_t* ptr = nullptr;
  const int32_t* rows = nullptr;
  int64_t longest = 0;
};
int rank_splits(int64_t C, int64_t U);
int64_t rank_ctx_tile(int splits, int n_top);
void launch_rank_bias(const double* summary, int64_t n, int kp, double* bias, hipStream_t st);
void launch_rank_score(const double* sum_u, const double* bias_u, const uint32_t* cnt_u, int64_t Ut,
                       const double* sum_c, const double* bias_c, const uint32_t* cnt_c, int64_t C, int kp, int splits,
                       int n_top, double w0, uint64_t* lkey, uint32_t* lidx, hipStream_t st);
void launch_rank_score_select(int select, const double* sum_u, const double* bias_u, const uint32_t* cnt_u, int64_t Ut,
                              const double* sum_c, const double* bias_c, const uint32_t* cnt_c, int64_t C,
                              const int64_t* sel_ptr, const int32_t* sel_rows, int kp, int splits, int n_top, double w0,
                              uint64_t* lkey, uint32_t* lidx, hipStream_t st);
void launch_rank_merge(const uint64_t* lkey, const uint32_t* lidx, int64_t Ut, int splits, int n_top,
                       const uint32_t* cnt_u, const uint32_t* cnt_c, double w0, double lo, double hi, int32_t* out_idx,
                       double* out_score, hipStream_t st);
int64_t rank_position_ctx_tile();
void launch_rank_position(const double* sum_u, const double* bias_u, const uint32_t* cnt_u, int64_t Ut, const double* sum_c,
                          const double* bias_c, const uint32_t* cnt_c, int64_t C, const int64_t* tgt_ptr,
                          const int32_t* tgt_rows, int64_t longest, const int64_t* ex_ptr, const int32_t* ex_rows, int kp,
                          int splits, double w0, double lo, double hi, int32_t* position, double* score, hipStream_t st);

void launch_select_rows(const BatchDev& src, const int64_t* rows, const int64_t* row_ptr_in, int64_t B, BatchDev& dst,
                        hipStream_t st);
void launch_split_rebase(const BatchDev& b, const int64_t* split_rows, int32_t n_splits, int64_t* split_rp,
                         hipStream_t st);

}
```

### fm_spark_amd/csrc/fm_sort.hip

```cpp
#include <type_traits>

#include "fm_device.h"
#include "fm_internal.h"

namespace fmhip {

namespace {

constexpr int kMaxRB = 10;
constexpr int kSortBlock = 512;
constexpr int kWaves = kSortBlock / 64;
constexpr int kMinRB = 9;
template <int R>
constexpr int digits_per_thread() { return R >= kSortBlock ? R / kSortBlock : 1; }
constexpr int kRounds = 8;
constexpr int kTile = kSortBlock * kRounds;
constexpr int kMaxRadix = 1 << kMaxRB;
constexpr int kChunk = 16;

__device__ __forceinline__ int64_t tile_of_block(int64_t ntiles) {
  const int64_t per = (ntiles + 7) / 8;
  return (int64_t)(blockIdx.x % 8) * per + blockIdx.x / 8;
}

inline int64_t blocks_for_tiles(int64_t ntiles) { return (ntiles + 7) / 8 * 8; }

static_assert(kTile % (4 * kSortBlock) == 0, "count block must divide the tile into uint4 rounds");

struct TileGeo {
  int64_t tile, base, end;
};

__device__ __forceinline__ bool tile_geo(TileGeo& g, int64_t n, int64_t ntiles) {
  g.tile = tile_of_block(ntiles);
  if (g.tile >= ntiles) return false;
  g.base = g.tile * kTile;
  g.end = n;
  return true;
}

template <int RB>
__global__ __launch_bounds__(kSortBlock) void k_radix_count(const uint32_t* __restrict__ keys, int64_t n, int shift,
                                                        uint32_t* __restrict__ counts, int64_t ntiles, bool vec) {
  constexpr int R = 1 << RB;
  constexpr uint32_t M = R - 1;
  __shared__ uint32_t hist[R];
  TileGeo g;
  if (!tile_geo(g, n, ntiles)) return;
  const int64_t base = g.base;
  constexpr int NV = kTile / (4 * kSortBlock), NS = kTile / kSortBlock;
  const bool wide = vec && base + kTile <= g.end;
  uint4 q[NV];
  uint32_t kk[NS];
  if (wide) {
    const uint4* k4 = reinterpret_cast<const uint4*>(keys + base);
#pragma unroll
    for (int i = 0; i < NV; ++i) q[i] = k4[i * kSortBlock + threadIdx.x];
  } else {
#pragma unroll
    for (int i = 0; i < NS; ++i) {
      const int64_t idx = base + (int64_t)i * kSortBlock + threadIdx.x;
      kk[i] = keys[idx < g.end ? idx : g.end - 1];
    }
  }
  for (int d = threadIdx.x; d < R; d += kSortBlock) hist[d] = 0;
  lds_barrier();
  if (wide) {
#pragma unroll
    for (int i = 0; i < NV; ++i) {
      atomicAdd(&hist[(q[i].x >> shift) & M], 1u);
      atomicAdd(&hist[(q[i].y >> shift) & M], 1u);
      atomicAdd(&hist[(q[i].z >> shift) & M], 1u);
      atomicAdd(&hist[(q[i].w >> shift) & M], 1u);
    }
  } else {
#pragma unroll
    for (int i = 0; i < NS; ++i)
      if (base + (int64_t)i * kSortBlock + threadIdx.x < g.end) atomicAdd(&hist[(kk[i] >> shift) & M], 1u);
  }
  lds_barrier();
  for (int d = threadIdx.x; d < R; d += kSortBlock) counts[g.tile * R + d] = hist[d];
}

__device__ __forceinline__ uint32_t wave_incl_scan_u32(uint32_t v, int lane) {
#pragma unroll
  for (int o = 1; o < 64; o <<= 1) {
    const uint32_t t = __shfl_up(v, o);
    if (lane >= o) v += t;
  }
  return v;
}

template <int RB>
__global__ __launch_bounds__(256) void k_radix_chunk_scan(uint32_t* __restrict__ counts, int64_t ntiles,
                                                             uint32_t* __restrict__ csum) {
  constexpr int R = 1 << RB;
  constexpr int TB = R < 256 ? R : 256;
  constexpr int S = R / TB;
  const int64_t c = blockIdx.x / S;
  const int d = (int)(blockIdx.x % S) * TB + threadIdx.x;
  const int64_t t0 = c * kChunk;
  uint32_t v[kChunk];
#pragma unroll
  for (int j = 0; j < kChunk; ++j) v[j] = t0 + j < ntiles ? counts[(t0 + j) * R + d] : 0u;
  uint32_t run = 0;
#pragma unroll
  for (int j = 0; j < kChunk; ++j) {
    if (t0 + j < ntiles) counts[(t0 + j) * R + d] = run;
    run += v[j];
  }
  csum[c * R + d] = run;
}


__global__ __launch_bounds__(256) void k_radix_chunk_top(uint32_t* __restrict__ csum, int64_t nchunks, int R,
                                                         uint32_t* __restrict__ digit_tot) {
  constexpr int kDig = 32, kSl = 8;
  __shared__ uint32_t part[kSl][kDig];
  const int dl = threadIdx.x % kDig, sl = threadIdx.x / kDig;
  const int d = blockIdx.x * kDig + dl;
  const int64_t nch = nchunks;
  const int64_t per = (nch + kSl - 1) / kSl;
  const int64_t c0 = min(nch, sl * per), c1 = min(nch, c0 + per);
  constexpr int kTopLd = 8;
  uint32_t s = 0;
  for (int64_t cb = c0; cb < c1; cb += kTopLd) {
    uint32_t x[kTopLd];
#pragma unroll
    for (int j = 0; j < kTopLd; ++j) x[j] = csum[(cb + j < c1 ? cb + j : c1 - 1) * R + d];
#pragma unroll
    for (int j = 0; j < kTopLd; ++j) s += cb + j < c1 ? x[j] : 0u;
  }
  part[sl][dl] = s;
  __syncthreads();
  if (sl == 0) {
    uint32_t run = 0;
#pragma unroll
    for (int q = 0; q < kSl; ++q) {
      const uint32_t x = part[q][dl];
      part[q][dl] = run;
      run += x;
    }
    digit_tot[d] = run;
  }
  __syncthreads();
  uint32_t run = part[sl][dl];
  for (int64_t cb = c0; cb < c1; cb += kTopLd) {
    uint32_t x[kTopLd];
#pragma unroll
    for (int j = 0; j < kTopLd; ++j) x[j] = csum[(cb + j < c1 ? cb + j : c1 - 1) * R + d];
#pragma unroll
    for (int j = 0; j < kTopLd; ++j) {
      if (cb + j < c1) csum[(cb + j) * R + d] = run;
      run += cb + j < c1 ? x[j] : 0u;
    }
  }
}

template <int D>
__device__ __forceinline__ void block_excl_scan(uint32_t (&v)[D], uint32_t* wsum, int lane, int wave) {
  uint32_t t = 0;
#pragma unroll
  for (int i = 0; i < D; ++i) t += v[i];
  const uint32_t incl = wave_incl_scan_u32(t, lane);
  if (lane == 63) wsum[wave] = incl;
  lds_barrier();
  uint32_t run = incl - t;
#pragma unroll
  for (int w = 0; w < kWaves; ++w) run += (w < wave) ? wsum[w] : 0u;
#pragma unroll
  for (int i = 0; i < D; ++i) {
    const uint32_t c = v[i];
    v[i] = run;
    run += c;
  }
}

template <class P>
__device__ __forceinline__ P implicit_payload(int64_t idx);
template <>
__device__ __forceinline__ uint32_t implicit_payload<uint32_t>(int64_t idx) {
  return (uint32_t)idx;
}
template <>
__device__ __forceinline__ uint2 implicit_payload<uint2>(int64_t idx) {
  return make_uint2((uint32_t)idx, 0u);
}

template <class P, int RB, bool IMPLICIT>
__global__ __launch_bounds__(kSortBlock) void k_radix_scatter(const uint32_t* __restrict__ keys_in,
                                                          const P* __restrict__ vals_in,
                                                          uint32_t* __restrict__ keys_out,
                                                          P* __restrict__ vals_out, int64_t n,
                                                          int shift, const uint32_t* __restrict__ counts,
                                                          const uint32_t* __restrict__ csum,
                                                          const uint32_t* __restrict__ digit_tot,
                                                          int64_t ntiles) {
  constexpr int R = 1 << RB;
  constexpr uint32_t M = R - 1;
  constexpr int D = digits_per_thread<R>();
  const bool own = R >= kSortBlock || (int)threadIdx.x * D < R;
  using HistT = typename std::conditional<(RB >= 10), uint16_t, uint32_t>::type;
  static_assert(kTile < 65536 || RB < 10, "16-bit tile histograms need tiles below 64K keys");
  __shared__ uint32_t s_keys[kTile];
  __shared__ P s_vals[kTile];
  __shared__ HistT wave_hist[kWaves][R];
  __shared__ uint32_t tile_start[R];
  __shared__ uint32_t glob_off[R];
  __shared__ uint32_t wsum[kWaves];

  TileGeo g;
  if (!tile_geo(g, n, ntiles)) return;
  const int64_t tile = g.tile;
  const int tid = threadIdx.x, lane = tid & 63, wave = tid >> 6;
  const uint64_t lt_mask = (lane == 0) ? 0ull : (~0ull >> (64 - lane));
  const int64_t tile_base = g.base;
  const int64_t wbase = tile_base + (int64_t)wave * (kTile / kWaves);
  uint32_t my_key[kRounds], my_rank[kRounds];
  P my_val[kRounds];
  uint32_t tot[D], pcs[D], pct[D];
#pragma unroll
  for (int i = 0; i < D; ++i) {
    const int d = own ? tid * D + i : 0;
    tot[i] = digit_tot[d];
    pcs[i] = csum[(tile / kChunk) * R + d];
    pct[i] = counts[tile * R + d];
  }
#pragma unroll
  for (int r = 0; r < kRounds; ++r) {
    const int64_t idx = wbase + (int64_t)r * 64 + lane;
    my_key[r] = keys_in[idx < g.end ? idx : g.end - 1];
  }
#pragma unroll
  for (int r = 0; r < kRounds; ++r) {
    const int64_t idx = wbase + (int64_t)r * 64 + lane;
    if constexpr (IMPLICIT) my_val[r] = P{};
    else my_val[r] = vals_in[idx < g.end ? idx : g.end - 1];
  }
  __builtin_amdgcn_sched_barrier(0);
#pragma unroll
  for (int w = 0; w < kWaves; ++w)
    for (int d = tid; d < R; d += kSortBlock) wave_hist[w][d] = 0;

  {
    uint32_t v[D];
#pragma unroll
    for (int i = 0; i < D; ++i) v[i] = own ? tot[i] : 0u;
    block_excl_scan<D>(v, wsum, lane, wave);
#pragma unroll
    for (int i = 0; i < D; ++i)
      if (own) glob_off[tid * D + i] = v[i] + (pcs[i] + pct[i]);
  }
  lds_barrier();

#pragma unroll
  for (int r = 0; r < kRounds; ++r) {
    const int64_t idx = wbase + (int64_t)r * 64 + lane;
    const bool valid = idx < g.end;
    const uint32_t d = (my_key[r] >> shift) & M;
    uint64_t peers = __ballot(valid);
#pragma unroll
    for (int b = 0; b < RB; ++b) {
      const bool bit = (d >> b) & 1u;
      const uint64_t m = __ballot(bit);
      peers &= bit ? m : ~m;
    }
    const uint32_t below = (uint32_t)__popcll(peers & lt_mask);
    const uint32_t cnt = (uint32_t)__popcll(peers);
    const uint32_t prev = wave_hist[wave][d];
    __builtin_amdgcn_wave_barrier();
    if (valid && below == 0) wave_hist[wave][d] = (HistT)(prev + cnt);
    __builtin_amdgcn_wave_barrier();
    my_rank[r] = valid ? prev + below : 0xFFFFFFFFu;
  }
  lds_barrier();

  {
    uint32_t v[D];
#pragma unroll
    for (int i = 0; i < D; ++i) {
      const int d = tid * D + i;
      uint32_t acc = 0;
      if (own) {
#pragma unroll
        for (int w = 0; w < kWaves; ++w) {
          const uint32_t c = wave_hist[w][d];
          wave_hist[w][d] = (HistT)acc;
          acc += c;
        }
      }
      v[i] = acc;
    }
    block_excl_scan<D>(v, wsum, lane, wave);
#pragma unroll
    for (int i = 0; i < D; ++i) {
      if (own) {
        tile_start[tid * D + i] = v[i];
        glob_off[tid * D + i] -= v[i];
      }
    }
  }
  lds_barrier();

#pragma unroll
  for (int r = 0; r < kRounds; ++r) {
    if (my_rank[r] != 0xFFFFFFFFu) {
      const uint32_t d = (my_key[r] >> shift) & M;
      const uint32_t pos = tile_start[d] + wave_hist[wave][d] + my_rank[r];
      s_keys[pos] = my_key[r];
      s_vals[pos] = IMPLICIT ? implicit_payload<P>(wbase + (int64_t)r * 64 + lane) : my_val[r];
    }
  }
  lds_barrier();

  const int64_t rem = g.end - tile_base;
  const int tile_n = rem < kTile ? (int)rem : kTile;
#pragma unroll
  for (int r = 0; r < kRounds; ++r) {
    const int j = r * kSortBlock + tid;
    if (j >= tile_n) break;
    const uint32_t key = s_keys[j];
    const uint32_t d = (key >> shift) & M;
    const uint32_t dest = glob_off[d] + (uint32_t)j;
    keys_out[dest] = key;
    vals_out[dest] = s_vals[j];
  }
}

}

inline int64_t count_rows(int64_t ntiles) { return ntiles + 1 + (ntiles + 1 + kChunk - 1) / kChunk; }

void SortWork::ensure(int64_t n) {
  if (n <= cap) return;
  const int64_t c = n + n / 8 + 4096;
  keys_a.ensure(sizeof(uint32_t) * c);
  keys_b.ensure(sizeof(uint32_t) * c);
  vals_a.ensure(sizeof(uint64_t) * c);
  vals_b.ensure(sizeof(uint64_t) * c);
  const int64_t ntiles = (c + kTile - 1) / kTile;
  counts.ensure(sizeof(uint32_t) * kMaxRadix * count_rows(ntiles));
  digit_tot.ensure(sizeof(uint32_t) * kMaxRadix);
  cap = c;
}

template <class P, int RB>
static void radix_pass_impl(const uint32_t* kin, const P* vin, uint32_t* ko, P* vo, int64_t n, int shift,
                       SortWork& w, int64_t ntiles, hipStream_t st) {
  uint32_t* counts = w.counts.as<uint32_t>();
  uint32_t* csum = counts + (ntiles + 1) * (int64_t(1) << RB);
  const int64_t nchunks = (ntiles + kChunk - 1) / kChunk;
  const bool vec = (reinterpret_cast<uintptr_t>(kin) & 15u) == 0;
  hipLaunchKernelGGL(k_radix_count<RB>, dim3((unsigned)blocks_for_tiles(ntiles)), dim3(kSortBlock), 0, st, kin, n, shift,
                     counts, ntiles, vec);
  constexpr int TB = (1 << RB) < 256 ? (1 << RB) : 256;
  hipLaunchKernelGGL(k_radix_chunk_scan<RB>, dim3((unsigned)(nchunks * ((1 << RB) / TB))), dim3(TB), 0, st, counts,
                     ntiles, csum);
  hipLaunchKernelGGL(k_radix_chunk_top, dim3((1u << RB) / 32), dim3(256), 0, st, csum, nchunks, 1 << RB,
                     w.digit_tot.as<uint32_t>());
  auto scatter = vin ? k_radix_scatter<P, RB, false> : k_radix_scatter<P, RB, true>;
  hipLaunchKernelGGL(scatter, dim3((unsigned)blocks_for_tiles(ntiles)), dim3(kSortBlock), 0, st, kin, vin, ko, vo, n,
                     shift, (const uint32_t*)counts, (const uint32_t*)csum,
                     (const uint32_t*)w.digit_tot.as<uint32_t>(), ntiles);
  FM_HIP_CHECK(hipGetLastError());
}

template <class P, int RB>
static void radix_pass(const uint32_t* kin, const P* vin, uint32_t* ko, P* vo, int64_t n, int shift,
                       SortWork& w, int64_t ntiles, hipStream_t st) {
  radix_pass_impl<P, RB>(kin, vin, ko, vo, n, shift, w, ntiles, st);
}

inline int digit_bits(int key_bits, int* passes) {
  const int kb = key_bits < 1 ? 1 : key_bits;
  int p = (kb + kMaxRB - 1) / kMaxRB;
  int rb = (kb + p - 1) / p;
  if (rb < kMinRB) rb = kMinRB;
  p = (kb + rb - 1) / rb;
  *passes = p;
  return rb;
}

template <class P>
static void radix_sort_impl(SortWork& w, const uint32_t* keys_in, const P* vals_in, int64_t n, int key_bits,
                            hipStream_t st, const uint32_t** keys_out, const P** vals_out,
                            uint32_t* final_keys = nullptr, P* final_vals = nullptr, int lo_bit = 0) {
  FM_REQUIRE(n >= 0 && n < (int64_t(1) << 32) - 1, "sort size out of range");
  w.ensure(n > 0 ? n : 1);
  if (n == 0) {
    *keys_out = w.keys_a.as<uint32_t>();
    *vals_out = w.vals_a.as<P>();
    return;
  }
  int passes = 0;
  const int rb = digit_bits(key_bits, &passes);
  const int64_t ntiles = (n + kTile - 1) / kTile;
  FM_REQUIRE(ntiles < (int64_t(1) << 31), "too many sort tiles");
  const uint32_t* kin = keys_in;
  const P* vin = vals_in;
  uint32_t* kbuf[2] = {w.keys_a.as<uint32_t>(), w.keys_b.as<uint32_t>()};
  P* vbuf[2] = {w.vals_a.as<P>(), w.vals_b.as<P>()};
  int which = 0;
  for (int p = 0; p < passes; ++p) {
    const int shift = lo_bit + rb * p;
    const bool last = p == passes - 1 && final_keys != nullptr;
    uint32_t* ko = last ? final_keys : kbuf[which];
    P* vo = last ? final_vals : vbuf[which];
    switch (rb) {
      case 6: radix_pass<P, 6>(kin, vin, ko, vo, n, shift, w, ntiles, st); break;
      case 7: radix_pass<P, 7>(kin, vin, ko, vo, n, shift, w, ntiles, st); break;
      case 8: radix_pass<P, 8>(kin, vin, ko, vo, n, shift, w, ntiles, st); break;
      case 9: radix_pass<P, 9>(kin, vin, ko, vo, n, shift, w, ntiles, st); break;
      default: radix_pass<P, 10>(kin, vin, ko, vo, n, shift, w, ntiles, st); break;
    }
    kin = ko;
    vin = vo;
    which ^= 1;
  }
  *keys_out = kin;
  *vals_out = vin;
}

void radix_sort_pairs(SortWork& w, const uint32_t* keys_in, const uint32_t* vals_in, int64_t n, int key_bits,
                      hipStream_t st, const uint32_t** keys_out, const uint32_t** vals_out) {
  radix_sort_impl<uint32_t>(w, keys_in, vals_in, n, key_bits, st, keys_out, vals_out);
}

void radix_sort_pairs64_bits(SortWork& w, const uint32_t* keys_in, const uint2* vals_in, int64_t n, int lo_bit,
                             int hi_bit, hipStream_t st, uint32_t* final_keys, uint2* final_vals) {
  FM_REQUIRE(lo_bit >= 0 && hi_bit > lo_bit && hi_bit <= 32, "bad sort bit range");
  const uint32_t* ko = nullptr;
  const uint2* vo = nullptr;
  radix_sort_impl<uint2>(w, keys_in, vals_in, n, hi_bit - lo_bit, st, &ko, &vo, final_keys, final_vals, lo_bit);
}

void radix_sort_pairs64(SortWork& w, const uint32_t* keys_in, const uint2* vals_in, int64_t n, int key_bits,
                        hipStream_t st, const uint32_t** keys_out, const uint2** vals_out, uint32_t* final_keys,
                        uint2* final_vals) {
  radix_sort_impl<uint2>(w, keys_in, vals_in, n, key_bits, st, keys_out, vals_out, final_keys, final_vals);
}

}
```

### fm_spark_amd/csrc/fm_update.hip

```cpp
#include <algorithm>
#include <cstdlib>

#include "fm_device.h"

namespace fmhip {

namespace {

constexpr int kWaveEnt = 256;
constexpr int kUpdD = 2;
constexpr int kUpdD4 = 1;
constexpr int kUpdD2 = 1;

struct SegArgs {
  TableView T;
  const uint32_t* skeys;
  const uint2* sents;
  int64_t N;
  const float* S;
  const float2* yl;
  int64_t s_stride;
  int64_t yl_stride;
  double* part;
  int64_t nranges;
// ... 300 lines not shown
    }
    if (tail) {
      if (extend(acc, accb, accw, g + 1)) {
        float4 vq[NF];
#pragma unroll
        for (int n = 0; n < NF; ++n) {
          const int c = 4 * (q + Q * n);
          vq[n] = c < kp ? *reinterpret_cast<const float4*>(T.v(lastkey) + c) : make_float4(0.f, 0.f, 0.f, 0.f);
        }
        const float4 hq = *reinterpret_cast<const float4*>(T.hdr(lastkey));
        close_run(lastkey, vq, hq, acc, accb, accw, false);
      } else {
        write_part(1, acc, accb, accw);
      }
    }
  }
  if (lane == 0) wcnt[wave] = ucount;
  __syncthreads();
  if (threadIdx.x == 0) {
    uint32_t t = 0;
#pragma unroll
    for (int w = 0; w < kBlock / 64; ++w) t += wcnt[w];
    a.ucnt[lblk] = t;
  }
  __syncthreads();
  }
}

struct RowCur {
  bool present;
  double ac;
  float w;
};
__device__ __forceinline__ RowCur row_current(const SegArgs& a, uint32_t key) {
  const RowHdr h = *a.T.hdr(key);
  RowCur r;
  r.present = h.t >= 0;
  r.ac = r.present ? a.p.cumE - h.cum : 0.0;
  r.w = r.present ? h.w : 0.f;
  if (r.ac > 0.0) r.w = shrink_f(r.w, r.ac);
  return r;
}
__device__ __forceinline__ void close_col(const SegArgs& a, uint32_t key, const RowCur& rc, int c, float vraw, double b,
                                          double sum) {
  float v = rc.present ? vraw : 0.f;
  if (rc.ac > 0.0) v = shrink_f(v, rc.ac);
  const double gv = sum - (double)v * b;
  if (a.emit) a.emit[(int64_t)key * (a.T.kp + 4) + c] = (float)gv;
  else a.T.v(key)[c] = upd_v(v, gv, a.p);
}
__device__ __forceinline__ void close_cols(const SegArgs& a, uint32_t key, const RowCur& rc, int c_lo, int c_hi,
                                           int c_step, double b, const double* sums) {
  const float* vrow = a.T.v(key);
  for (int c = c_lo, j = 0; c < c_hi; c += c_step, ++j) close_col(a, key, rc, c, vrow[c], b, sums[j]);
}
__device__ __forceinline__ void close_hdr(const SegArgs& a, uint32_t key, const RowCur& rc, double gw) {
  const int kp = a.T.kp;
  if (a.emit) {
    *reinterpret_cast<float2*>(a.emit + (int64_t)key * (kp + 4) + kp) = make_float2((float)gw, 1.f);
  } else {
    store_hdr(a.T, key, next_hdr(upd_w(rc.w, gw, a.p), a.p));
  }
}

constexpr int kStatLd = 8;
constexpr int kCombLanes = 16;
constexpr int kCombCols = 10;
__global__ __launch_bounds__(kBlock) void k_segment_combine(SegArgs a, const double2* __restrict__ loss_part,
                                                            int64_t n_loss_blocks, int64_t n_ucnt,
                                                            double* __restrict__ stats_out) {
  const int tid = threadIdx.x, lane = tid & 63, wave = tid >> 6;
  const int kp = a.T.kp;
  const int64_t W = kp + 2;
  const int64_t N = a.n_dev ? a.n_dev[0] : a.N;
  const int64_t nranges = (N + a.L - 1) / a.L;
  __shared__ double run_sum[kBlock / 64][258];
  if (blockIdx.x == 0) {
    __shared__ double rl[kBlock], rc[kBlock], ru[kBlock];
    double l = 0.0, c = 0.0, u = 0.0;
    for (int64_t i0 = tid; i0 < n_loss_blocks; i0 += kStatLd * kBlock) {
      double2 v[kStatLd];
#pragma unroll
      for (int j = 0; j < kStatLd; ++j) {
        const int64_t i = i0 + j * kBlock;
        v[j] = loss_part[i < n_loss_blocks ? i : n_loss_blocks - 1];
      }
#pragma unroll
      for (int j = 0; j < kStatLd; ++j) {
        const bool in = i0 + j * kBlock < n_loss_blocks;
        l += in ? v[j].x : 0.0;
        c += in ? v[j].y : 0.0;
      }
    }
    const int64_t per_blk = (int64_t)kWaveEnt * (kBlock / 64);
    const int64_t nu = a.n_dev ? min(n_ucnt, (N + per_blk - 1) / per_blk) : n_ucnt;
    for (int64_t i0 = tid; i0 < nu; i0 += kStatLd * kBlock) {
      uint32_t v[kStatLd];
#pragma unroll
      for (int j = 0; j < kStatLd; ++j) {
        const int64_t i = i0 + j * kBlock;
        v[j] = a.ucnt[i < nu ? i : nu - 1];
      }
#pragma unroll
      for (int j = 0; j < kStatLd; ++j) u += i0 + j * kBlock < nu ? (double)v[j] : 0.0;
    }
    if (a.n_dev && tid == 0) u += (double)a.n_dev[1];
    rl[tid] = l;
    rc[tid] = c;
    ru[tid] = u;
    __syncthreads();
    for (int o = kBlock / 2; o > 0; o >>= 1) {
      if (tid < o) {
        rl[tid] += rl[tid + o];
        rc[tid] += rc[tid + o];
        ru[tid] += ru[tid + o];
      }
      __syncthreads();
    }
    if (tid == 0) {
      stats_out[0] = rl[0];
      stats_out[1] = rc[0];
      stats_out[2] = ru[0];
    }
  }
  const int64_t chunk = ((int64_t)blockIdx.x * kBlock + tid) / kCombLanes;
  const int f = tid & (kCombLanes - 1);
  const int64_t L = a.L;
  bool owner = false, two = false;
  uint32_t key = 0;
  if (chunk < nranges) {
    const int64_t p0 = chunk * L;
    const int64_t p1 = p0 + L < N ? p0 + L : N;
    if (p1 < N) {
      const int64_t p2 = (chunk + 2) * L;
      const uint32_t kl = a.skeys[p1 - 1], kn = a.skeys[p1], kf = a.skeys[p0];
      const uint32_t kb = a.skeys[p0 > 0 ? p0 - 1 : 0], k2 = a.skeys[p2 < N ? p2 : N - 1];
      key = kl;
      owner = kn == kl && !(kf == kl && p0 > 0 && kb == kl);
      two = owner && !(p2 < N && k2 == kl);
    }
  }
  if (owner && two) {
    const double* pt = a.part + (chunk * 2 + 1) * W;
    const double* ph = a.part + ((chunk + 1) * 2) * W;
    const int cf = f < kp ? f : kp - 1;
    const double bt = pt[kp + 1], bh = ph[kp + 1], wt = pt[0], wh = ph[0];
    const double st = pt[1 + cf], sh = ph[1 + cf];
    const float vf = a.T.v(key)[cf];
    const RowCur rc = row_current(a, key);
    const double b = bt + bh;
    if (f < kp) close_col(a, key, rc, f, vf, b, st + sh);
    for (int c = f + kCombLanes; c < kp; c += kCombLanes) {
      const double sm = pt[1 + c] + ph[1 + c];
      close_cols(a, key, rc, c, c + 1, 1, b, &sm);
    }
    if (f == 0) close_hdr(a, key, rc, wt + wh);
  }
  uint64_t owners = __ballot(owner && !two && f == 0);
  while (owners) {
    const int l = __ffsll((unsigned long long)owners) - 1;
    owners &= owners - 1;
    const int64_t c0 = __shfl(chunk, l);
    const uint32_t k0 = __shfl(key, l);
    int64_t cend = c0 + 1;
    for (;;) {
      const int64_t c = cend + lane;
      const bool cont = c < nranges && a.skeys[c * L] == k0;
      const uint64_t m = __ballot(cont);
      if (m == ~0ull) {
        cend += 64;
        continue;
      }
      cend += __ffsll((unsigned long long)~m) - 1;
      break;
    }
    for (int col0 = 0; col0 < (int)W; col0 += kCombCols) {
      double s[kCombCols];
#pragma unroll
      for (int j = 0; j < kCombCols; ++j) s[j] = 0.0;
      for (int64_t c = c0 + 1 + lane; c < cend; c += 64) {
        const double* pr = a.part + (c * 2) * W;
#pragma unroll
        for (int j = 0; j < kCombCols / 2; ++j) {
          const int cc = col0 + 2 * j;
          const double2 v = *reinterpret_cast<const double2*>(pr + (cc < (int)W ? cc : (int)W - 2));
          s[2 * j] += cc < (int)W ? v.x : 0.0;
          s[2 * j + 1] += cc < (int)W ? v.y : 0.0;
        }
      }
#pragma unroll
      for (int o = 1; o < 64; o <<= 1)
#pragma unroll
        for (int j = 0; j < kCombCols; ++j) s[j] += __shfl_xor(s[j], o);
      if (lane == 0) {
#pragma unroll
        for (int j = 0; j < kCombCols; ++j)
          if (col0 + j < (int)W) run_sum[wave][col0 + j] = s[j];
      }
    }
    wave_lds_sync();
    for (int col = lane; col < (int)W; col += 64) run_sum[wave][col] = a.part[(c0 * 2 + 1) * W + col] + run_sum[wave][col];
    wave_lds_sync();
    const double gw = run_sum[wave][0], b = run_sum[wave][kp + 1];
    double sums[4];
    int j = 0;
    for (int col = lane; col < kp; col += 64, ++j) sums[j] = run_sum[wave][1 + col];
    const RowCur rc = row_current(a, k0);
    close_cols(a, k0, rc, lane, kp, 64, b, sums);
    if (lane == 0) close_hdr(a, k0, rc, gw);
    wave_lds_sync();
  }
}

template <int G>
__global__ __launch_bounds__(kBlock) void k_repl_apply(TableView T, const float* __restrict__ grad, StepParams p,
                                                       uint32_t* __restrict__ blk_touched) {
  const int g = threadIdx.x % G;
  const int kp = T.kp, nq = kp >> 2, W = kp + 4;
  uint32_t touched = 0;
  for (int64_t i = ((int64_t)blockIdx.x * kBlock + threadIdx.x) / G; i < T.rows;
       i += (int64_t)gridDim.x * kBlock / G) {
    const float* gr = grad + i * W;
    const float2 wt = *reinterpret_cast<const float2*>(gr + kp);
    if (wt.y == 0.f) continue;
    touched += g == 0 ? 1u : 0u;
    const RowHdr h = *T.hdr(i);
    const bool present = h.t >= 0;
    const double ac = present ? p.cumE - h.cum : 0.0;
    float4* rec = reinterpret_cast<float4*>(T.v(i));
    for (int q = g; q < nq; q += G) {
      float4 v = present ? rec[q] : make_float4(0.f, 0.f, 0.f, 0.f);
      if (ac > 0.0) v = shrink4(v, ac);
      const float4 d = reinterpret_cast<const float4*>(gr)[q];
      rec[q] = make_float4(upd_v(v.x, d.x, p), upd_v(v.y, d.y, p), upd_v(v.z, d.z, p), upd_v(v.w, d.w, p));
    }
    if (g == 0) {
      float w = present ? h.w : 0.f;
      if (ac > 0.0) w = shrink_f(w, ac);
      store_hdr(T, i, next_hdr(upd_w(w, (double)wt.x, p), p));
    }
  }
  __shared__ uint32_t wt[kBlock / 64];
#pragma unroll
  for (int o = 32; o > 0; o >>= 1) touched += __shfl_xor(touched, o);
  if ((threadIdx.x & 63) == 0) wt[threadIdx.x >> 6] = touched;
  __syncthreads();
  if (threadIdx.x == 0) {
    uint32_t t = 0;
    for (int w = 0; w < kBlock / 64; ++w) t += wt[w];
    blk_touched[blockIdx.x] = t;
  }
}

__global__ __launch_bounds__(kBlock) void k_sum_counts(const uint32_t* __restrict__ c, int64_t n, double* __restrict__ out) {
  __shared__ uint64_t ws[kBlock / 64];
  uint64_t t = 0;
  for (int64_t i = threadIdx.x; i < n; i += kBlock) t += c[i];
#pragma unroll
  for (int o = 32; o > 0; o >>= 1) t += __shfl_xor(t, o);
  if ((threadIdx.x & 63) == 0) ws[threadIdx.x >> 6] = t;
  __syncthreads();
  if (threadIdx.x == 0) {
    uint64_t a = 0;
    for (int w = 0; w < kBlock / 64; ++w) a += ws[w];
    *out = (double)a;
  }
}
}

constexpr int kSplitChunk = 1024;

constexpr int kSplitRows = kSplitChunk / 64;
constexpr uint32_t kSplitNone = 0xFFFFFFFFu;
struct SplitChunk {
  uint32_t key[kSplitRows];
  uint32_t multi = 0, first = 0;
};
__device__ __forceinline__ void split_chunk(const uint32_t* __restrict__ skeys, int64_t N, int64_t c, int lane,
                                            SplitChunk& sc) {
  const int64_t base = c * kSplitChunk;
#pragma unroll
  for (int r = 0; r < kSplitRows; ++r) {
    const int64_t p = base + r * 64 + lane;
    sc.key[r] = skeys[p < N ? p : N - 1];
  }
  const int64_t eb = lane == 0 ? (base > 0 ? base - 1 : 0) : (base + kSplitChunk < N ? base + kSplitChunk : N - 1);
  const uint32_t edge = skeys[eb];
  const uint32_t before = base > 0 ? __shfl(edge, 0) : kSplitNone;
  const uint32_t after = base + kSplitChunk < N ? __shfl(edge, 1) : kSplitNone;
#pragma unroll
  for (int r = 0; r < kSplitRows; ++r) {
    const int64_t p = base + r * 64 + lane;
    const uint32_t up = __shfl_up(sc.key[r], 1), dn = __shfl_down(sc.key[r], 1);
    const uint32_t pl = r > 0 ? __shfl(sc.key[r > 0 ? r - 1 : 0], 63) : before;
    const uint32_t nf = r + 1 < kSplitRows ? __shfl(sc.key[r + 1 < kSplitRows ? r + 1 : r], 0) : after;
    const uint32_t prev = lane == 0 ? pl : up;
    const uint32_t next = p + 1 >= N ? kSplitNone : (lane == 63 ? nf : dn);
    const bool valid = p < N;
    sc.multi |= (uint32_t)(valid && (prev == sc.key[r] || next == sc.key[r])) << r;
    sc.first |= (uint32_t)(valid && prev != sc.key[r]) << r;
  }
}

__global__ __launch_bounds__(kBlock) void k_split_count(const uint32_t* __restrict__ skeys, int64_t N,
                                                        uint2* __restrict__ cnt, int64_t nchunks, TableView T,
                                                        int32_t epoch) {
  const int lane = threadIdx.x & 63;
  const int64_t c = (int64_t)blockIdx.x * (kBlock / 64) + (threadIdx.x >> 6);
  if (c >= nchunks) return;
  SplitChunk sc;
  split_chunk(skeys, N, c, lane, sc);
  const uint32_t tag = sc.multi & sc.first;
  int32_t tv[kSplitRows];
#pragma unroll
  for (int r = 0; r < kSplitRows; ++r) tv[r] = T.hdr((tag >> r) & 1u ? sc.key[r] : 0u)->t;
#pragma unroll
  for (int r = 0; r < kSplitRows; ++r)
    if ((tag >> r) & 1u) T.hdr(sc.key[r])->t = multi_tag(epoch, tv[r] >= 0);
  uint32_t nm = 0, ns = 0;
  const int64_t base = c * kSplitChunk;
#pragma unroll
  for (int r = 0; r < kSplitRows; ++r) {
    const bool valid = base + r * 64 + lane < N;
    const bool m = (sc.multi >> r) & 1u;
    nm += (uint32_t)__popcll(__ballot(m));
    ns += (uint32_t)__popcll(__ballot(valid && !m));
  }
  if (lane == 0) cnt[c] = make_uint2(nm, ns);
}

constexpr int kSplitPer = 12;
constexpr int kSplitScanNT = 1024;
__global__ __launch_bounds__(kSplitScanNT) void k_split_scan(const uint2* __restrict__ cnt, int64_t nchunks,
                                                             int64_t* __restrict__ off, int64_t* __restrict__ n_out) {
  constexpr int NW = kSplitScanNT / 64;
  __shared__ int64_t wsum[NW], ssum[NW];
  const int lane = threadIdx.x & 63, wave = threadIdx.x >> 6;
  int64_t carry = 0, singles = 0;
  for (int64_t b = 0; b < nchunks; b += kSplitScanNT * kSplitPer) {
    const int64_t i0 = b + (int64_t)threadIdx.x * kSplitPer;
    uint2 v[kSplitPer];
#pragma unroll
    for (int j = 0; j < kSplitPer; ++j) v[j] = cnt[i0 + j < nchunks ? i0 + j : nchunks - 1];
#pragma unroll
    for (int j = 0; j < kSplitPer; ++j)
      if (i0 + j >= nchunks) v[j] = make_uint2(0u, 0u);
    int64_t t = 0, sg = 0;
#pragma unroll
    for (int j = 0; j < kSplitPer; ++j) {
      t += v[j].x;
      sg += v[j].y;
    }
    int64_t incl = t;
#pragma unroll
    for (int o = 1; o < 64; o <<= 1) {
      const int64_t u = __shfl_up(incl, o);
      if (lane >= o) incl += u;
    }
#pragma unroll
    for (int o = 32; o > 0; o >>= 1) sg += __shfl_xor(sg, o);
    if (lane == 63) wsum[wave] = incl;
    if (lane == 0) ssum[wave] = sg;
    __syncthreads();
    int64_t wpre = 0, tot = 0, stot = 0;
    for (int w = 0; w < NW; ++w) {
      wpre += w < wave ? wsum[w] : 0;
      tot += wsum[w];
      stot += ssum[w];
    }
    int64_t run = carry + wpre + incl - t;
#pragma unroll
    for (int j = 0; j < kSplitPer; ++j) {
      if (i0 + j < nchunks) off[i0 + j] = run;
      run += v[j].x;
    }
    carry += tot;
    singles += stot;
    __syncthreads();
  }
  if (threadIdx.x == 0) {
    n_out[0] = carry;
    n_out[1] = singles;
  }
}

__global__ __launch_bounds__(kBlock) void k_split_scatter(const uint32_t* __restrict__ skeys,
                                                          const uint2* __restrict__ sents, int64_t N,
                                                          const int64_t* __restrict__ off, int64_t nchunks,
                                                          uint32_t* __restrict__ mkeys, uint2* __restrict__ ments) {
  const int lane = threadIdx.x & 63;
  const int64_t c = (int64_t)blockIdx.x * (kBlock / 64) + (threadIdx.x >> 6);
  if (c >= nchunks) return;
  const uint64_t lt = lane == 0 ? 0ull : (~0ull >> (64 - lane));
  const int64_t base = c * kSplitChunk;
  uint2 en[kSplitRows];
#pragma unroll
  for (int r = 0; r < kSplitRows; ++r) {
    const int64_t p = base + r * 64 + lane;
    en[r] = sents[p < N ? p : N - 1];
  }
  int64_t o = off[c];
  SplitChunk sc;
  split_chunk(skeys, N, c, lane, sc);
#pragma unroll
  for (int r = 0; r < kSplitRows; ++r) {
    const bool m = (sc.multi >> r) & 1u;
    const uint64_t bm = __ballot(m);
    if (m) {
      const int64_t d = o + __popcll(bm & lt);
      mkeys[d] = sc.key[r];
      ments[d] = en[r];
    }
    o += __popcll(bm);
  }
}

void launch_split(const uint32_t* skeys, const uint2* sents, int64_t N, SplitWork& sw, uint32_t* mkeys, uint2* ments,
                  int64_t* n_out, hipStream_t st, const TableView& tag_T, int32_t epoch) {
  const int64_t nchunks = (N + kSplitChunk - 1) / kSplitChunk;
  sw.cnt.ensure_slack(sizeof(uint2) * (size_t)std::max<int64_t>(nchunks, 1));
  sw.off.ensure_slack(sizeof(int64_t) * (size_t)std::max<int64_t>(nchunks, 1));
  if (N <= 0) {
    FM_HIP_CHECK(hipMemsetAsync(n_out, 0, 2 * sizeof(int64_t), st));
    return;
  }
  const unsigned blocks = (unsigned)((nchunks + kBlock / 64 - 1) / (kBlock / 64));
  hipLaunchKernelGGL(k_split_count, dim3(blocks), dim3(kBlock), 0, st, skeys, N, sw.cnt.as<uint2>(), nchunks, tag_T,
                     epoch);
  hipLaunchKernelGGL(k_split_scan, dim3(1), dim3(kSplitScanNT), 0, st, sw.cnt.as<uint2>(), nchunks, sw.off.as<int64_t>(), n_out);
  hipLaunchKernelGGL(k_split_scatter, dim3(blocks), dim3(kBlock), 0, st, skeys, sents, N, sw.off.as<int64_t>(), nchunks,
                     mkeys, ments);
  FM_HIP_CHECK(hipGetLastError());
}
void launch_segment_update(const TableView& T, const BatchDev& b, StepWork& w, const StepParams& p,
                           const uint32_t* skeys, const uint2* sents, int64_t n_fwd_blocks,
                           double* stats_out, hipStream_t st, float* emit, const int64_t* n_dev) {
  SegSource src{w.S.as<float>(), s_rec_floats(T.kp),
                 s_rec_yl(T.kp) ? reinterpret_cast<const float2*>(w.S.as<float>() + T.kp) : w.yl.as<float2>(),
                 s_rec_yl(T.kp) ? s_rec_floats(T.kp) / 2 : 1};
  src.n_dev = n_dev;
  launch_segment_update(T, b.nnz, src, w, p, skeys, sents, n_fwd_blocks, stats_out, st, emit);
}

void launch_segment_update(const TableView& T, int64_t N, const SegSource& src, StepWork& w, const StepParams& p,
                           const uint32_t* skeys, const uint2* sents, int64_t n_fwd_blocks, double* stats_out,
                           hipStream_t st, float* emit) {
  const int64_t L = kWaveEnt;
  const int64_t nranges = (N + L - 1) / L;
  w.part.ensure(sizeof(double) * (size_t)(nranges > 0 ? nranges : 1) * 2 * (T.kp + 2));
  const int64_t per_block = (int64_t)kWaveEnt * (kBlock / 64);
  const int64_t ublocks = (N + per_block - 1) / per_block;
  w.ucnt.ensure(sizeof(uint32_t) * (size_t)(ublocks > 0 ? ublocks : 1));
  SegArgs a;
  a.T = T;
  a.skeys = skeys;
  a.sents = sents;
  a.N = N;
  a.S = src.S;
  a.yl = src.yl;
  a.s_stride = src.s_stride;
  a.yl_stride = src.yl_stride;
  a.part = w.part.as<double>();
  a.nranges = nranges;
  a.L = L;
  a.p = p;
  a.ucnt = w.ucnt.as<uint32_t>();
  a.emit = emit;
  a.n_dev = src.n_dev;
  if (ublocks > 0) {
    const dim3 grid((unsigned)ublocks), blk(kBlock);
    with_update_cfg(T.kp, [&](auto cfg) {
      using Cfg = decltype(cfg);
      hipLaunchKernelGGL((k_segment_update<Cfg::Q, Cfg::NF, Cfg::D>), grid, blk, 0, st, a);
    });
    FM_HIP_CHECK(hipGetLastError());
  }
  int64_t cblocks = (nranges * kCombLanes + kBlock - 1) / kBlock;
  if (cblocks < 1) cblocks = 1;
  hipLaunchKernelGGL(k_segment_combine, dim3((unsigned)cblocks), dim3(kBlock), 0, st, a,
                     w.loss_part.as<double2>(), n_fwd_blocks, ublocks, stats_out);
  FM_HIP_CHECK(hipGetLastError());
}

UpdGeometry update_geometry(int kp) {
  UpdGeometry g{};
  g.wave_entries = kWaveEnt;
  g.block_entries = kWaveEnt * (kBlock / 64);
  with_update_cfg(kp, [&](auto cfg) {
    using Geo = UpdGeom<decltype(cfg)::Q, decltype(cfg)::NF>;
    g.group_entries = Geo::RL;
    g.paired = Geo::PAIR && kp == 4 * decltype(cfg)::Q;
  });
  g.comb_lanes = kCombLanes;
  g.comb_cols = kCombCols;
  g.split_chunk = kSplitChunk;
  g.scan_round_chunks = kSplitScanNT * kSplitPer;
  return g;
}

void launch_repl_apply(const TableView& T, const float* grad, const StepParams& p, uint32_t* blk_touched,
                       double* n_touched, hipStream_t st) {
  if (T.rows <= 0) {
    FM_HIP_CHECK(hipMemsetAsync(n_touched, 0, sizeof(double), st));
    return;
  }
  const int nq = T.kp / 4;
  const int G = nq <= 1 ? 1 : nq <= 2 ? 2 : nq <= 4 ? 4 : nq <= 8 ? 8 : 16;
  const unsigned grid = grid_for(T.rows * G, kBlock);
  switch (G) {
    case 1: hipLaunchKernelGGL(k_repl_apply<1>, dim3(grid), dim3(kBlock), 0, st, T, grad, p, blk_touched); break;
    case 2: hipLaunchKernelGGL(k_repl_apply<2>, dim3(grid), dim3(kBlock), 0, st, T, grad, p, blk_touched); break;
    case 4: hipLaunchKernelGGL(k_repl_apply<4>, dim3(grid), dim3(kBlock), 0, st, T, grad, p, blk_touched); break;
    case 8: hipLaunchKernelGGL(k_repl_apply<8>, dim3(grid), dim3(kBlock), 0, st, T, grad, p, blk_touched); break;
    default: hipLaunchKernelGGL(k_repl_apply<16>, dim3(grid), dim3(kBlock), 0, st, T, grad, p, blk_touched); break;
  }
  hipLaunchKernelGGL(k_sum_counts, dim3(1), dim3(kBlock), 0, st, blk_touched, (int64_t)grid, n_touched);
  FM_HIP_CHECK(hipGetLastError());
}

}
```

### fm_spark_amd/engine.py

```python

from __future__ import annotations

import ctypes as C
from dataclasses import dataclass

import numpy as np

from . import _native as N


@dataclass
class StepOut:
    loss_sum: float
    n_rows: int
    n_loss_rows: int
    n_unique: int
    executed: bool = True


@dataclass(frozen=True)
class EvalSums:

    n_rows: int
    n_unlearned: int
    epoch: int
    sum_err: float
    sum_abs_err: float
    sum_sq_err: float
    executed: bool = True

    @staticmethod
    def from_struct(o: "N.fm_eval_out", executed: bool = True) -> "EvalSums":
        return EvalSums(int(o.n_rows), int(o.n_unlearned), int(o.epoch), float(o.sum_err), float(o.sum_abs_err),
                        float(o.sum_sq_err), executed)

    @property
    def mae(self) -> float:
        return self.sum_abs_err / self.n_rows

    @property
    def mse(self) -> float:
        return self.sum_sq_err / self.n_rows

    @property
    def rmse(self) -> float:
        return float(np.sqrt(self.mse))

    @property
    def bias(self) -> float:
        return self.sum_err / self.n_rows

    def r2(self, ss_tot: float) -> float:
        return 1.0 - self.sum_sq_err / ss_tot


class DeviceBatch:

    def __init__(self, ctx: "FMContext", csr: N.CSRHost | None):
        self._lib = N.load()
        self.ctx = ctx
        h = C.c_void_p()
        self.handle = h
        self.n_rows = self.nnz = 0
        if csr is not None:
            N.check(self._lib.fm_batch_create(ctx.handle, C.byref(csr.c), C.byref(h)), "fm_batch_create")
            self.n_rows = csr.n_rows
            self.nnz = csr.nnz

    def select_rows(self, data: "DeviceBatch", rows):
        rows = np.ascontiguousarray(rows, dtype=np.int64)
        h = self.handle if self.handle else C.c_void_p()
        N.check(self._lib.fm_batch_from_rows(self.ctx.handle, data.handle, N.ptr(rows, C.c_int64), len(rows),
                                             C.byref(h)), "fm_batch_from_rows")
        self.handle = h
        self.n_rows = len(rows)
        self.nnz = int(self._lib.fm_batch_nnz(h))
        self._data = data
        return self

    def view_split(self, data: "DeviceBatch", split: int):
        h = self.handle if self.handle else C.c_void_p()
        N.check(self._lib.fm_batch_split_view(self.ctx.handle, data.handle, int(split), C.byref(h)),
                "fm_batch_split_view")
        self.handle = h
        self.n_rows = int(self._lib.fm_batch_rows(h))
        self.nnz = int(self._lib.fm_batch_nnz(h))
        self._data = data
        return self

    def prepare(self):
        N.check(self._lib.fm_batch_prepare(self.ctx.handle, self.handle), "fm_batch_prepare")

    def close(self):
        if self.handle:
            self._lib.fm_batch_destroy(self.handle)
            self.handle = None

    def __del__(self):
        try:
            self.close()
        except Exception:
            pass


def comm_unique_id() -> bytes:
    lib = N.load()
    buf = (C.c_uint8 * 128)()
    N.check(lib.fm_comm_unique_id(buf), "fm_comm_unique_id")
    return bytes(buf)


def normalize_row_lists(lists, n_ctx: int):
    if (isinstance(lists, tuple) and len(lists) == 2 and all(isinstance(a, np.ndarray) and a.ndim == 1 for a in lists)
            and len(lists[0]) == n_ctx + 1):
        ptr, flat = lists
        if ptr.dtype.kind not in "iu" or (flat.size and flat.dtype.kind not in "iu"):
            raise ValueError("row lists must hold integers")
        ptr = ptr.astype(np.int64)
        if ptr[0] != 0 or np.any(np.diff(ptr) < 0) or ptr[-1] != flat.size:
            raise ValueError("(ptr, rows): ptr must start at 0, not decrease and end at len(rows)")
        parts = [flat[ptr[u]:ptr[u + 1]] for u in range(n_ctx)]
    else:
        parts = [np.asarray(r) for r in lists]
        if len(parts) != n_ctx:
            raise ValueError(f"expected one row list per context ({n_ctx}), got {len(parts)}")
    out = []
    for u, r in enumerate(parts):
        if r.ndim != 1 or (r.size and r.dtype.kind not in "iu"):
            raise ValueError(f"row list of context {u} must be a flat sequence of integers")
        r = np.unique(r.astype(np.int64))
        if r.size and (r[0] < -2**31 or r[-1] >= 2**31):
            raise ValueError(f"row list of context {u} holds a row outside int32")
        out.append(r.astype(np.int32))
    ptr = np.zeros(n_ctx + 1, dtype=np.int64)
    np.cumsum([len(r) for r in out], out=ptr[1:])
    rows = np.concatenate(out) if out else np.zeros(0, np.int32)
    return ptr, np.ascontiguousarray(rows, dtype=np.int32)


class FMContext:

    _PAR = {None: N.FM_PARALLEL_NONE, "none": N.FM_PARALLEL_NONE, "sharded": N.FM_PARALLEL_SHARDED,
            "replicated": N.FM_PARALLEL_REPLICATED}
    _TR = {"auto": N.FM_TRANSPORT_AUTO, "rccl": N.FM_TRANSPORT_RCCL, "copy": N.FM_TRANSPORT_COPY}
    _WIRE = {"fp32": N.FM_WIRE_FP32, "fp64": N.FM_WIRE_FP64}

    def __init__(self, num_features: int, k: int, *, device: int = 0, seed: int = 0, init_sd: float = 0.01,
                 w0: float = 0.0, shard_index: int = 0, shard_count: int = 1, parallel: str | None = None,
                 n_gpus: int = 1, devices=None, transport: str = "auto", n_procs: int = 1, proc_rank: int = 0,
                 comm_id: bytes | None = None, fuse: bool | None = None, xchg_chunks: int = 0, wire: str = "fp32"):
        self._lib = N.load()
        if wire not in self._WIRE:
            raise ValueError('wire must be "fp32" or "fp64"')
        cfg = N.fm_config(num_features=int(num_features), k=int(k), device=int(device), seed=int(seed) & (2**64 - 1),
                          init_sd=float(init_sd), w0=float(w0), shard_index=int(shard_index),
                          shard_count=int(shard_count))
        cfg.parallel = self._PAR[parallel]
        cfg.n_gpus = int(n_gpus)
        devs = list(devices) if devices is not None else [int(device) + i for i in range(int(n_gpus))]
        if cfg.parallel != N.FM_PARALLEL_NONE and len(devs) != n_gpus:
            raise ValueError("devices must list n_gpus devices")
        for i, d in enumerate(devs[: N.FM_MAX_LOCAL]):
            cfg.devices[i] = int(d)
        if cfg.parallel != N.FM_PARALLEL_NONE:
            cfg.device = int(devs[0])
        cfg.transport = self._TR[transport]
        cfg.fuse_single = N.FM_FUSE_DEFAULT if fuse is None else (N.FM_FUSE_ON if fuse else N.FM_FUSE_OFF)
        cfg.xchg_chunks = int(xchg_chunks)
        cfg.wire = self._WIRE[wire]
        cfg.n_procs = int(n_procs)
        cfg.proc_rank = int(proc_rank)
        if comm_id is not None:
            if len(comm_id) != 128:
                raise ValueError("comm_id must be 128 bytes")
            for i, b in enumerate(comm_id):
                cfg.comm_id[i] = b
        self.parallel = parallel if parallel not in (None, "none") else None
        self.n_gpus = int(n_gpus)
        h = C.c_void_p()
        N.check(self._lib.fm_create(C.byref(cfg), C.byref(h)), "fm_create")
        self.handle = h
        self.num_features = int(num_features)
        self.k = int(k)
        self.w0 = float(w0)
        self.shard_index = int(shard_index)
        self.shard_count = int(shard_count)
        self.wire = wire

    def close(self):
        if getattr(self, "handle", None):
            self._lib.fm_destroy(self.handle)
            self.handle = None

    def __del__(self):
        try:
            self.close()
        except Exception:
            pass

    def set_stream(self, stream_ptr: int | None):
        N.check(self._lib.fm_set_stream(self.handle, C.c_void_p(stream_ptr or None)), "fm_set_stream")

    def sync(self):
        N.check(self._lib.fm_sync(self.handle), "fm_sync")

    def reserve(self, max_rows: int, max_nnz: int):
        N.check(self._lib.fm_reserve(self.handle, int(max_rows), int(max_nnz)), "fm_reserve")

    def load_tables(self, ids, w, V):
        ids = np.ascontiguousarray(ids, dtype=np.int32)
        w = np.ascontiguousarray(w, dtype=np.float64)
        V = np.ascontiguousarray(V, dtype=np.float64).reshape(len(ids), self.k)
        N.check(self._lib.fm_load_tables(self.handle, N.ptr(ids, C.c_int32), len(ids), N.ptr(w, C.c_double),
                                         N.ptr(V, C.c_double)), "fm_load_tables")

    def init_random(self, ids):
        ids = np.ascontiguousarray(ids, dtype=np.int32)
        N.check(self._lib.fm_init_random(self.handle, N.ptr(ids, C.c_int32), len(ids)), "fm_init_random")

    def init_random_range(self, begin: int, end: int):
        N.check(self._lib.fm_init_random_range(self.handle, int(begin), int(end)), "fm_init_random_range")

    def init_from_batch(self, b: "DeviceBatch") -> int:
        n = C.c_int64()
        N.check(self._lib.fm_init_from_batch(self.handle, b.handle, C.byref(n)), "fm_init_from_batch")
        return n.value

    def export_tables(self):
        n = C.c_int64()
        N.check(self._lib.fm_export_tables(self.handle, None, None, None, 0, C.byref(n)), "fm_export_tables")
        cnt = n.value
        ids = np.zeros(max(cnt, 1), dtype=np.int32)
        w = np.zeros(max(cnt, 1))
        V = np.zeros((max(cnt, 1), self.k))
        if cnt:
            N.check(self._lib.fm_export_tables(self.handle, N.ptr(ids, C.c_int32), N.ptr(w, C.c_double),
                                               N.ptr(V, C.c_double), cnt, C.byref(n)), "fm_export_tables")
        return ids[:cnt], w[:cnt], V[:cnt]

    def export_rows(self, ids):
        ids = np.ascontiguousarray(ids, dtype=np.int32)
        n = len(ids)
        w = np.zeros(max(n, 1))
        V = np.zeros((max(n, 1), self.k))
        pres = np.zeros(max(n, 1), dtype=np.int8)
        N.check(self._lib.fm_export_rows(self.handle, N.ptr(ids, C.c_int32), n, N.ptr(w, C.c_double),
                                         N.ptr(V, C.c_double), N.ptr(pres, C.c_int8)), "fm_export_rows")
        return w[:n], V[:n], pres[:n].astype(bool)

    def num_present(self) -> int:
        return N.check(self._lib.fm_num_present(self.handle), "fm_num_present")

    @property
    def epoch(self) -> int:
        return int(self._lib.fm_epoch(self.handle))

    def batch(self, csr: N.CSRHost) -> DeviceBatch:
        return DeviceBatch(self, csr)

    def batch_splits(self, csr: N.CSRHost, split_rows) -> DeviceBatch:
        sr = np.ascontiguousarray(split_rows, dtype=np.int64)
        b = DeviceBatch(self, None)
        h = C.c_void_p()
        N.check(self._lib.fm_batch_create_splits(self.handle, C.byref(csr.c), len(sr) - 1, N.ptr(sr, C.c_int64),
                                                 C.byref(h)), "fm_batch_create_splits")
        b.handle = h
        b.n_rows, b.nnz = csr.n_rows, csr.nnz
        b.split_rows = sr
        return b

    def batch_layout_splits(self, csr: N.CSRHost, split_rows, order) -> DeviceBatch:
        sr = np.ascontiguousarray(split_rows, dtype=np.int64)
        od = np.ascontiguousarray(order, dtype=np.int64)
        if len(sr) < 2 or len(od) != sr[-1]:
            raise ValueError("order must hold split_rows[-1] row indices")
        b = DeviceBatch(self, None)
        h = C.c_void_p()
        N.check(self._lib.fm_batch_layout_splits(self.handle, C.byref(csr.c), len(sr) - 1, N.ptr(sr, C.c_int64),
                                                 N.ptr(od, C.c_int64), C.byref(h)), "fm_batch_layout_splits")
        b.handle = h
        b.n_rows = int(self._lib.fm_batch_rows(h))
        b.nnz = int(self._lib.fm_batch_nnz(h))
        b.split_rows = sr
        return b

    def split_view(self, data: DeviceBatch, split: int, into: DeviceBatch | None = None) -> DeviceBatch:
        b = into if into is not None else DeviceBatch(self, None)
        return b.view_split(data, split)

    def batch_from_rows(self, data: DeviceBatch, rows, into: DeviceBatch | None = None) -> DeviceBatch:
        b = into if into is not None else DeviceBatch(self, None)
        return b.select_rows(data, rows)

    @property
    def fuse_active(self) -> bool:
        return int(self._lib.fm_fuse_active(self.handle)) == 1

    def step(self, csr: N.CSRHost, t: int, step_size: float, reg_param: float, sync: bool = True):
        if not sync:
            N.check(self._lib.fm_step(self.handle, C.byref(csr.c), int(t), float(step_size), float(reg_param), None),
                    "fm_step")
            return None
        out = N.fm_step_out()
        rc = N.check(self._lib.fm_step(self.handle, C.byref(csr.c), int(t), float(step_size), float(reg_param),
                                       C.byref(out)), "fm_step")
        if rc == N.FM_NOTHING_TO_DO:
            return StepOut(0.0, 0, 0, 0, executed=False)
        return StepOut(out.loss_sum, out.n_rows, out.n_loss_rows, out.n_unique)

    def step_batch(self, b: DeviceBatch, t: int, step_size: float, reg_param: float, sync: bool = True):
        if sync:
            out = N.fm_step_out()
            rc = N.check(self._lib.fm_step_batch(self.handle, b.handle, int(t), float(step_size), float(reg_param),
                                                 C.byref(out)), "fm_step_batch")
            if rc == N.FM_NOTHING_TO_DO:
                return StepOut(0.0, 0, 0, 0, executed=False)
            return StepOut(out.loss_sum, out.n_rows, out.n_loss_rows, out.n_unique)
        N.check(self._lib.fm_step_batch(self.handle, b.handle, int(t), float(step_size), float(reg_param), None),
                "fm_step_batch")
        return None

    def loss_history(self) -> np.ndarray:
        n = C.c_int64()
        N.check(self._lib.fm_loss_history(self.handle, None, 0, C.byref(n)), "fm_loss_history")
        out = np.zeros(max(n.value, 1))
        if n.value:
            N.check(self._lib.fm_loss_history(self.handle, N.ptr(out, C.c_double), n.value, C.byref(n)),
                    "fm_loss_history")
        return out[: n.value]

    def predict(self, csr: N.CSRHost, min_label: float, max_label: float) -> np.ndarray:
        out = np.zeros(max(csr.n_rows, 1))
        N.check(self._lib.fm_predict(self.handle, C.byref(csr.c), float(min_label), float(max_label),
                                     N.ptr(out, C.c_double)), "fm_predict")
        return out[: csr.n_rows]

    def predict_batch(self, b: DeviceBatch, min_label: float, max_label: float) -> np.ndarray:
        out = np.zeros(max(b.n_rows, 1))
        N.check(self._lib.fm_predict_batch(self.handle, b.handle, float(min_label), float(max_label),
                                           N.ptr(out, C.c_double)), "fm_predict_batch")
        return out[: b.n_rows]

    def evaluate(self, csr: N.CSRHost, min_label: float, max_label: float, want_pred: bool = False):
        return self._evaluate(self._lib.fm_evaluate, "fm_evaluate", C.byref(csr.c), csr.n_rows, min_label, max_label,
                              True, want_pred)

    def evaluate_batch(self, b: DeviceBatch, min_label: float, max_label: float, sync: bool = True,
                       want_pred: bool = False):
        if not sync and want_pred:
            raise ValueError("want_pred needs sync=True")
        return self._evaluate(self._lib.fm_evaluate_batch, "fm_evaluate_batch", b.handle, b.n_rows, min_label,
                              max_label, sync, want_pred)

    def _evaluate(self, fn, what, rows, n_rows, min_label, max_label, sync, want_pred):
        pred = np.zeros(max(n_rows, 1)) if want_pred else None
        pp = N.ptr(pred, C.c_double) if want_pred else None
        if not sync:
            N.check(fn(self.handle, rows, float(min_label), float(max_label), None, None), what)
            return None
        out = N.fm_eval_out()
        rc = N.check(fn(self.handle, rows, float(min_label), float(max_label), pp, C.byref(out)), what)
        sums = EvalSums.from_struct(out, executed=rc != N.FM_NOTHING_TO_DO)
        return (sums, pred[:n_rows]) if want_pred else sums

    def eval_history(self) -> list:
        n = C.c_int64()
        N.check(self._lib.fm_eval_history(self.handle, None, 0, C.byref(n)), "fm_eval_history")
        if not n.value:
            return []
        buf = (N.fm_eval_out * n.value)()
        N.check(self._lib.fm_eval_history(self.handle, buf, n.value, C.byref(n)), "fm_eval_history")
        return [EvalSums.from_struct(o) for o in buf[: n.value]]

    def rank(self, contexts: N.CSRHost, candidates: N.CSRHost, n_top: int, min_label: float, max_label: float, *,
             only=None, exclude=None):
        return self._rank(self._lib.fm_rank_candidates, self._lib.fm_rank_candidates_select, "fm_rank_candidates",
                          C.byref(contexts.c), C.byref(candidates.c), contexts.n_rows, n_top, min_label, max_label,
                          only, exclude)

    def rank_batch(self, contexts: DeviceBatch, candidates: DeviceBatch, n_top: int, min_label: float,
                   max_label: float, *, only=None, exclude=None):
        return self._rank(self._lib.fm_rank_batch, self._lib.fm_rank_batch_select, "fm_rank_batch", contexts.handle,
                          candidates.handle, contexts.n_rows, n_top, min_label, max_label, only, exclude)

    def _rank(self, fn, fn_select, what, contexts, candidates, n_ctx, n_top, min_label, max_label, only, exclude):
        if only is not None and exclude is not None:
            raise ValueError("give only= or exclude=, not both")
        n_top = int(n_top)
        n = max(n_ctx * max(n_top, 0), 1)
        idx = np.zeros(n, dtype=np.int32)
        score = np.zeros(n)
        out = (n_top, float(min_label), float(max_label), N.ptr(idx, C.c_int32), N.ptr(score, C.c_double))
        if only is None and exclude is None:
            N.check(fn(self.handle, contexts, candidates, *out), what)
# ... 73 lines not shown
```

### include/fm_hip.h

```cpp
#ifndef FM_HIP_H
#define FM_HIP_H

#include <stdint.h>

#ifdef __cplusplus
extern "C" {
#endif

#define FM_OK 0
#define FM_NOTHING_TO_DO 1
#define FM_ERR_ARG (-1)
#define FM_ERR_OOM (-2)
#define FM_ERR_HIP (-3)
#define FM_ERR_RCCL (-4)
#define FM_ERR_STATE (-5)

#define FM_PARALLEL_NONE 0
#define FM_PARALLEL_SHARDED 1
#define FM_PARALLEL_REPLICATED 2
#define FM_TRANSPORT_AUTO 0
#define FM_TRANSPORT_RCCL 1
#define FM_TRANSPORT_COPY 2
#define FM_MAX_LOCAL 16
#define FM_FUSE_DEFAULT 0
#define FM_FUSE_ON 1
#define FM_FUSE_OFF (-1)
#define FM_WIRE_FP32 0
#define FM_WIRE_FP64 1

typedef struct fm_ctx fm_ctx;
typedef struct fm_batch fm_batch;

typedef struct fm_config {
  int64_t num_features;
  int32_t k;
  int32_t device;
  uint64_t seed;
  double init_sd;
  double w0;
  int32_t shard_index;
  int32_t shard_count;
  int32_t parallel;
  int32_t n_gpus;
  int32_t devices[FM_MAX_LOCAL];
  int32_t transport;
  int32_t n_procs;
  int32_t proc_rank;
  uint8_t comm_id[128];
  int32_t fuse_single;
  int32_t xchg_chunks;
  int32_t wire;
} fm_config;

typedef struct fm_csr {
  int64_t n_rows;
  int64_t nnz;
  const int64_t* row_ptr;
  const int32_t* col;
  const double* val;
  const double* label;
} fm_csr;

typedef struct fm_step_out {
  double loss_sum;
  int64_t n_rows;
  int64_t n_loss_rows;
  int64_t n_unique;
} fm_step_out;

int fm_create(const fm_config* cfg, fm_ctx** out);
int fm_comm_unique_id(uint8_t* id);
void fm_destroy(fm_ctx* ctx);
const char* fm_last_error(void);
int fm_set_stream(fm_ctx* ctx, void* hip_stream);
int fm_set_side_stream(fm_ctx* ctx, void* hip_stream);
int fm_sync(fm_ctx* ctx);
int fm_reserve(fm_ctx* ctx, int64_t max_rows, int64_t max_nnz);

int fm_load_tables(fm_ctx* ctx, const int32_t* ids, int64_t n, const double* w, const double* V);
int fm_init_random(fm_ctx* ctx, const int32_t* ids, int64_t n);
int fm_init_random_range(fm_ctx* ctx, int64_t id_begin, int64_t id_end);
int fm_init_from_batch(fm_ctx* ctx, fm_batch* data, int64_t* n_present);
int fm_export_tables(fm_ctx* ctx, int32_t* ids, double* w, double* V, int64_t cap, int64_t* n);
int fm_export_rows(fm_ctx* ctx, const int32_t* ids, int64_t n, double* w, double* V, int8_t* present);
int64_t fm_num_present(fm_ctx* ctx);
int64_t fm_epoch(fm_ctx* ctx);

int fm_batch_create(fm_ctx* ctx, const fm_csr* csr, fm_batch** out);
void fm_batch_destroy(fm_batch* b);
int fm_batch_prepare(fm_ctx* ctx, fm_batch* batch);
int fm_batch_from_rows(fm_ctx* ctx, const fm_batch* data, const int64_t* rows, int64_t n, fm_batch** out);
int fm_batch_create_splits(fm_ctx* ctx, const fm_csr* csr, int32_t n_splits, const int64_t* split_rows,
                           fm_batch** out);
int fm_batch_layout_splits(fm_ctx* ctx, const fm_csr* csr, int32_t n_splits, const int64_t* split_rows,
                           const int64_t* order, fm_batch** out);
int fm_batch_split_view(fm_ctx* ctx, const fm_batch* data, int32_t split, fm_batch** out);
int32_t fm_fuse_active(fm_ctx* ctx);
int64_t fm_batch_rows(const fm_batch* b);
int64_t fm_batch_nnz(const fm_batch* b);

int fm_step(fm_ctx* ctx, const fm_csr* batch, int32_t t, double step_size, double reg_param,
            fm_step_out* out);
int fm_step_batch(fm_ctx* ctx, fm_batch* batch, int32_t t, double step_size,
                  double reg_param, fm_step_out* out);
int fm_loss_history(fm_ctx* ctx, double* loss, int64_t cap, int64_t* n);

int fm_predict(fm_ctx* ctx, const fm_csr* csr, double min_label, double max_label, double* pred);
int fm_predict_batch(fm_ctx* ctx, fm_batch* batch, double min_label, double max_label, double* pred);
typedef struct fm_eval_out {
  int64_t n_rows;
  int64_t n_unlearned;
  int64_t epoch;
  double sum_err;
  double sum_abs_err;
  double sum_sq_err;
} fm_eval_out;
int fm_evaluate(fm_ctx* ctx, const fm_csr* csr, double min_label, double max_label, double* pred, fm_eval_out* out);
int fm_evaluate_batch(fm_ctx* ctx, fm_batch* batch, double min_label, double max_label, double* pred,
                      fm_eval_out* out);
int fm_eval_history(fm_ctx* ctx, fm_eval_out* out, int64_t cap, int64_t* n);
#define FM_RANK_MAX_TOP 1024
int fm_rank_candidates(fm_ctx* ctx, const fm_csr* contexts, const fm_csr* candidates, int32_t n_top,
                       double min_label, double max_label, int32_t* top_index, double* top_score);
int fm_rank_batch(fm_ctx* ctx, fm_batch* contexts, fm_batch* candidates, int32_t n_top,
                  double min_label, double max_label, int32_t* top_index, double* top_score);
#define FM_RANK_SELECT_ALL 0
#define FM_RANK_SELECT_ONLY 1
#define FM_RANK_SELECT_EXCEPT 2
int fm_rank_candidates_select(fm_ctx* ctx, const fm_csr* contexts, const fm_csr* candidates, int32_t select,
                              const int64_t* sel_ptr, const int32_t* sel_rows, int32_t n_top,
                              double min_label, double max_label, int32_t* top_index, double* top_score);
int fm_rank_batch_select(fm_ctx* ctx, fm_batch* contexts, fm_batch* candidates, int32_t select,
                         const int64_t* sel_ptr, const int32_t* sel_rows, int32_t n_top,
                         double min_label, double max_label, int32_t* top_index, double* top_score);
int fm_rank_positions(fm_ctx* ctx, const fm_csr* contexts, const fm_csr* candidates, const int64_t* tgt_ptr,
                      const int32_t* tgt_rows, const int64_t* excl_ptr, const int32_t* excl_rows,
                      double min_label, double max_label, int32_t* position, double* score);
int fm_rank_positions_batch(fm_ctx* ctx, fm_batch* contexts, fm_batch* candidates, const int64_t* tgt_ptr,
                            const int32_t* tgt_rows, const int64_t* excl_ptr, const int32_t* excl_rows,
                            double min_label, double max_label, int32_t* position, double* score);
int fm_loss_grad(fm_ctx* ctx, const fm_csr* csr, double* pred, double* loss, double* delta_w,
                 double* delta_v);
int fm_calc_loss_grad(fm_ctx* ctx, const fm_csr* csr, double initial_sd, uint64_t seed, double* pred,
                      double* loss, double* delta_w, double* delta_v);
int fm_vector_sum_by_key(fm_ctx* ctx, const int32_t* keys, int64_t n, const double* vecs,
                         int32_t k, int32_t* out_keys, double* out_sums, int64_t* n_out);

int fm_profile_enable(fm_ctx* ctx, int32_t on);
int fm_profile_read(fm_ctx* ctx, char* names, int64_t names_cap, double* total_ms,
                    int64_t* launches, int64_t cap, int64_t* n);
int fm_profile_reset(fm_ctx* ctx);
int64_t fm_device_bytes_live(void);
int64_t fm_device_allocs_live(void);

int fm_read_libsvm(const char* path, int64_t cap_rows, int64_t cap_nnz, double* label, int64_t* row_ptr,
                   int32_t* col, double* val, int64_t* n_rows, int64_t* nnz, int64_t* num_features);

int fm_random_split(int32_t n_parts, const int64_t* part_ptr, const char* column_order,
                    const double* label, const int8_t* vec_type, const int32_t* vec_size,
                    const int64_t* vec_ptr, const int32_t* vec_idx, const double* vec_val,
                    const int64_t* extra, int32_t n_weights, const double* weights,
                    int64_t seed, int32_t* split_of, int64_t* sample_id, int64_t* order);
int64_t fm_xorshift_hash_seed(int64_t seed);
int32_t fm_murmur3_bytes_hash(const uint8_t* data, int64_t len, int32_t seed);
int fm_xorshift_next_doubles(int64_t seed, int64_t n, double* out);

int fm_shard_route(fm_ctx* ctx, fm_batch* batch, void* send_slot, void* send_ent, int64_t* counts);
int fm_shard_owner_prepare(fm_ctx* ctx, fm_batch* batch, const void* recv_slot, const void* recv_ent,
                           int64_t n, const int64_t* src_entries, const int64_t* src_pairs);
int fm_shard_owner_forward(fm_ctx* ctx, fm_batch* batch, void* partials_out);
int fm_shard_combine(fm_ctx* ctx, fm_batch* batch, const void* partials_in, void* s_send);
int fm_shard_owner_update(fm_ctx* ctx, fm_batch* batch, const void* s_recv, int32_t t, double step_size,
                          double reg_param, int64_t global_rows);

int fm_repl_grad(fm_ctx* ctx, fm_batch* batch, void* grad);
int fm_repl_apply(fm_ctx* ctx, const void* grad, int32_t t, double step_size, double reg_param,
                  int64_t global_rows);

int fm_last_stats(fm_ctx* ctx, double* loss_sum, int64_t* n_loss_rows, int64_t* n_unique);

#ifdef __cplusplus
}
#endif

#endif
```

Measured before the change: 325.3 million samples/s.

## Prune tile-local singleton keys during final radix pass before fused split

The final radix-sort pass for the fused-split path now marks keys that appear only once and sit wholly inside their tile. Those keys are dropped from the scatter, and a device-side kept count feeds the split kernels, which now read N from device memory. This is meant to cut the sort-scatter and split traffic for the many singleton features in a hashed 100M-feature batch. It adds a count-with-keep kernel and mask storage, and forces at least two passes when there are multiple tiles. Dropped singletons are added back to the singles count, so correctness depends on the split path handling them elsewhere.

```diff
diff --git a/fm_spark_amd/_native.py b/fm_spark_amd/_native.py
--- a/fm_spark_amd/_native.py
+++ b/fm_spark_amd/_native.py
@@ -101,6 +101,7 @@
     "fm_batch_create": (C.c_int, [_P, C.POINTER(fm_csr), C.POINTER(_P)]),
     "fm_batch_destroy": (None, [_P]),
     "fm_batch_prepare": (C.c_int, [_P, _P]),
+    "fm_batch_view_stats": (C.c_int, [_P, _P, _I64P]),
     "fm_batch_from_rows": (C.c_int, [_P, _P, _I64P, C.c_int64, C.POINTER(_P)]),
     "fm_batch_create_splits": (C.c_int, [_P, C.POINTER(fm_csr), C.c_int32, _I64P, C.POINTER(_P)]),
     "fm_batch_layout_splits": (C.c_int, [_P, C.POINTER(fm_csr), C.c_int32, _I64P, _I64P, C.POINTER(_P)]),
diff --git a/fm_spark_amd/csrc/fm_capi.hip b/fm_spark_amd/csrc/fm_capi.hip
--- a/fm_spark_amd/csrc/fm_capi.hip
+++ b/fm_spark_amd/csrc/fm_capi.hip
@@ -347,8 +347,8 @@
   if (fused) {
     FM_HIP_CHECK(hipStreamWaitEvent(ctx->stream, b->ready, 0));
     e0 = ctx->prof_begin(ctx->stream);
-    launch_split(b->fkeys.as<uint32_t>(), b->fents.as<uint2>(), N, ctx->split_work, b->skeys.as<uint32_t>(),
-                 b->sents.as<uint2>(), b->split_n.as<int64_t>(), ctx->stream, T, p.epoch);
+    launch_split(b->fkeys.as<uint32_t>(), b->fents.as<uint2>(), N, b->split_n.as<int64_t>() + 2, ctx->split_work,
+                 b->skeys.as<uint32_t>(), b->sents.as<uint2>(), b->split_n.as<int64_t>(), ctx->stream, T, p.epoch);
     ctx->prof_end("split", e0, ctx->stream);
     fx.mode = kTrainFused;
   }
@@ -663,18 +663,37 @@
     const uint32_t* col = b->dev.col.as<uint32_t>();
     const uint2* ent = b->dev.ent.as<uint2>();
     if (b->split) {
-      b->split_n.ensure(2 * sizeof(int64_t));
+      b->split_n.ensure(4 * sizeof(int64_t));
       b->fkeys.ensure_slack(sizeof(uint32_t) * N);
       b->fents.ensure_slack(sizeof(uint2) * N);
-      radix_sort_pairs64(ctx->work.sort, col, ent, N, kb, ctx->side, &sk, &sv, b->fkeys.as<uint32_t>(),
-                         b->fents.as<uint2>());
+      int passes = 0;
+      radix_sort_pairs64_pruned(ctx->work.sort, col, ent, N, kb, ctx->side, b->fkeys.as<uint32_t>(), b->fents.as<uint2>(),
+                                b->split_n.as<int64_t>() + 2, &passes);
+      b->view_passes = passes;
     } else {
       radix_sort_pairs64(ctx->work.sort, col, ent, N, kb, ctx->side, &sk, &sv, b->skeys.as<uint32_t>(),
                          b->sents.as<uint2>());
+      b->view_passes = 0;
     }
     ctx->prof_end("sort", es, ctx->side);
     FM_HIP_CHECK(hipEventRecord(b->ready, ctx->side));
     b->prepared = true;
+    return FM_OK;
+  });
+}
+
+int fm_batch_view_stats(fm_ctx* ctx, const fm_batch* b, int64_t* out) {
+  return guarded(ctx, [&]() -> int {
+    FM_REQUIRE(b != nullptr && out != nullptr, "null argument");
+    FM_REQUIRE(b->owner == ctx && !b->grp, "batch belongs to another context");
+    FM_REQUIRE(b->prepared && b->split && b->ready, "the batch is not prepared for the fused step");
+    FM_HIP_CHECK(hipEventSynchronize(b->ready));
+    int64_t h[2] = {0, 0};
+    FM_HIP_CHECK(hipMemcpy(h, b->split_n.as<int64_t>() + 2, sizeof(h), hipMemcpyDeviceToHost));
+    out[0] = h[0];
+    out[1] = h[1];
+    out[2] = sort_tile_keys();
+    out[3] = b->view_passes;
     return FM_OK;
   });
 }
diff --git a/fm_spark_amd/csrc/fm_context.h b/fm_spark_amd/csrc/fm_context.h
--- a/fm_spark_amd/csrc/fm_context.h
+++ b/fm_spark_amd/csrc/fm_context.h
@@ -91,6 +91,7 @@
   DevBuf fkeys, fents;
   DevBuf split_n;
   bool split = false;
+  int32_t view_passes = 0;
   hipEvent_t ready = nullptr;
   hipEvent_t last_use = nullptr;
   void ensure_events(hipStream_t main) {
diff --git a/fm_spark_amd/csrc/fm_internal.h b/fm_spark_amd/csrc/fm_internal.h
--- a/fm_spark_amd/csrc/fm_internal.h
+++ b/fm_spark_amd/csrc/fm_internal.h
@@ -100,6 +100,8 @@
 
 struct SortWork {
   DevBuf keys_a, keys_b, vals_a, vals_b, counts, digit_tot;
+  int64_t keep_off = 0;
+  uint64_t* keep() const { return reinterpret_cast<uint64_t*>(static_cast<char*>(counts.p) + keep_off); }
   int64_t cap = 0;
   void ensure(int64_t n);
 };
@@ -111,6 +113,9 @@
                         int key_bits, hipStream_t st, const uint32_t** keys_out,
                         const uint2** vals_out, uint32_t* final_keys = nullptr,
                         uint2* final_vals = nullptr);
+void radix_sort_pairs64_pruned(SortWork& w, const uint32_t* keys_in, const uint2* vals_in, int64_t n, int key_bits,
+                               hipStream_t st, uint32_t* final_keys, uint2* final_vals, int64_t* n_out, int* passes);
+int sort_tile_keys();
 void radix_sort_pairs64_bits(SortWork& w, const uint32_t* keys_in, const uint2* vals_in, int64_t n, int lo_bit,
                              int hi_bit, hipStream_t st, uint32_t* final_keys, uint2* final_vals);
 
@@ -214,8 +219,8 @@
 struct SplitWork {
   DevBuf cnt, off;
 };
-void launch_split(const uint32_t* skeys, const uint2* sents, int64_t N, SplitWork& sw, uint32_t* mkeys, uint2* ments,
-                  int64_t* n_out, hipStream_t st, const TableView& tag_T, int32_t epoch);
+void launch_split(const uint32_t* skeys, const uint2* sents, int64_t N, const int64_t* n_in, SplitWork& sw,
+                  uint32_t* mkeys, uint2* ments, int64_t* n_out, hipStream_t st, const TableView& tag_T, int32_t epoch);
 void launch_segment_update(const TableView& T, int64_t N, const SegSource& src, StepWork& w, const StepParams& p,
                            const uint32_t* skeys, const uint2* sents, int64_t n_loss_blocks, double* stats_out,
                            hipStream_t st, float* emit = nullptr);
diff --git a/fm_spark_amd/csrc/fm_sort.hip b/fm_spark_amd/csrc/fm_sort.hip
--- a/fm_spark_amd/csrc/fm_sort.hip
+++ b/fm_spark_amd/csrc/fm_sort.hip
@@ -176,6 +176,146 @@
   }
 }
 
+template <int RB>
+using TileHistT = typename std::conditional<(RB >= 10), uint16_t, uint32_t>::type;
+
+template <int RB>
+__device__ __forceinline__ void rank_wave_keys(const uint32_t (&my_key)[kRounds], uint32_t valid, int shift,
+                                               TileHistT<RB>* wh, uint64_t lt_mask, uint32_t (&my_rank)[kRounds]) {
+  constexpr uint32_t M = (1u << RB) - 1;
+#pragma unroll
+  for (int r = 0; r < kRounds; ++r) {
+    const bool v = (valid >> r) & 1u;
+    const uint32_t d = (my_key[r] >> shift) & M;
+    uint64_t peers = __ballot(v);
+#pragma unroll
+    for (int b = 0; b < RB; ++b) {
+      const bool bit = (d >> b) & 1u;
+      const uint64_t m = __ballot(bit);
+      peers &= bit ? m : ~m;
+    }
+    const uint32_t below = (uint32_t)__popcll(peers & lt_mask);
+    const uint32_t cnt = (uint32_t)__popcll(peers);
+    const uint32_t prev = wh[d];
+    __builtin_amdgcn_wave_barrier();
+    if (v && below == 0) wh[d] = (TileHistT<RB>)(prev + cnt);
+    __builtin_amdgcn_wave_barrier();
+    my_rank[r] = v ? prev + below : 0xFFFFFFFFu;
+  }
+}
+
+template <int RB>
+__device__ __forceinline__ void tile_digit_starts(TileHistT<RB> (*wave_hist)[1 << RB], uint32_t* tile_start,
+                                                  uint32_t* wsum, bool own, int tid, int lane, int wave,
+                                                  uint32_t (&v)[digits_per_thread<(1 << RB)>()]) {
+  constexpr int D = digits_per_thread<(1 << RB)>();
+#pragma unroll
+  for (int i = 0; i < D; ++i) {
+    const int d = tid * D + i;
+    uint32_t acc = 0;
+    if (own) {
+#pragma unroll
+      for (int w = 0; w < kWaves; ++w) {
+        const uint32_t c = wave_hist[w][d];
+        wave_hist[w][d] = (TileHistT<RB>)acc;
+        acc += c;
+      }
+    }
+    v[i] = acc;
+  }
+  block_excl_scan<D>(v, wsum, lane, wave);
+#pragma unroll
+  for (int i = 0; i < D; ++i)
+    if (own) tile_start[tid * D + i] = v[i];
+}
+
+constexpr int kMaskWords = kWaves * kRounds;
+
+template <int RB>
+__global__ __launch_bounds__(kSortBlock) void k_radix_count_keep(const uint32_t* __restrict__ keys, int64_t n, int shift,
+                                                             uint32_t* __restrict__ counts, int64_t ntiles,
+                                                             uint64_t* __restrict__ mask) {
+  constexpr int R = 1 << RB;
+  constexpr uint32_t M = R - 1;
+  constexpr int D = digits_per_thread<R>();
+  __shared__ uint32_t s_keys[kTile];
+  __shared__ TileHistT<RB> wave_hist[kWaves][R];
+  __shared__ uint32_t tile_start[R];
+  __shared__ uint32_t hist[R];
+  __shared__ uint32_t wsum[kWaves];
+  TileGeo g;
+  if (!tile_geo(g, n, ntiles)) return;
+  const int tid = threadIdx.x, lane = tid & 63, wave = tid >> 6;
+  const bool own = R >= kSortBlock || tid * D < R;
+  const uint64_t lt_mask = (lane == 0) ? 0ull : (~0ull >> (64 - lane));
+  const int64_t wbase = g.base + (int64_t)wave * (kTile / kWaves);
+  uint32_t my_key[kRounds], my_rank[kRounds];
+  uint32_t valid = 0;
+#pragma unroll
+  for (int r = 0; r < kRounds; ++r) {
+    const int64_t idx = wbase + (int64_t)r * 64 + lane;
+    my_key[r] = keys[idx < g.end ? idx : g.end - 1];
+    valid |= (uint32_t)(idx < g.end) << r;
+  }
+  const bool has_before = g.base > 0, has_after = g.base + kTile < g.end;
+  const uint32_t before = keys[has_before ? g.base - 1 : 0];
+  const uint32_t after = keys[has_after ? g.base + kTile : g.end - 1];
+#pragma unroll
+  for (int w = 0; w < kWaves; ++w)
+    for (int d = tid; d < R; d += kSortBlock) wave_hist[w][d] = 0;
+  for (int d = tid; d < R; d += kSortBlock) hist[d] = 0;
+  lds_barrier();
+  rank_wave_keys<RB>(my_key, valid, shift, wave_hist[wave], lt_mask, my_rank);
+  lds_barrier();
+  {
+    uint32_t v[D];
+    tile_digit_starts<RB>(wave_hist, tile_start, wsum, own, tid, lane, wave, v);
+  }
+  lds_barrier();
+  uint32_t pos[kRounds];
+#pragma unroll
+  for (int r = 0; r < kRounds; ++r) {
+    const uint32_t d = (my_key[r] >> shift) & M;
+    pos[r] = tile_start[d] + wave_hist[wave][d] + my_rank[r];
+    if ((valid >> r) & 1u) s_keys[pos[r]] = my_key[r];
+  }
+  lds_barrier();
+  const int64_t rem = g.end - g.base;
+  const uint32_t tile_n = rem < kTile ? (uint32_t)rem : (uint32_t)kTile;
+  const uint32_t lowm = (1u << shift) - 1u;
+#pragma unroll
+  for (int r = 0; r < kRounds; ++r) {
+    const bool v = (valid >> r) & 1u;
+    const uint32_t key = my_key[r];
+    const uint32_t p = v ? pos[r] : 0u;
+    const uint32_t left = s_keys[p > 0 ? p - 1 : 0], right = s_keys[p + 1 < tile_n ? p + 1 : p];
+    const bool alone = (p == 0 || left != key) && (p + 1 >= tile_n || right != key);
+    const bool inside = (!has_before || ((before ^ key) & lowm) != 0) && (!has_after || ((after ^ key) & lowm) != 0);
+    const bool keep = v && !(alone && inside);
+    const uint64_t kb = __ballot(keep);
+    if (lane == 0) mask[g.tile * kMaskWords + wave * kRounds + r] = kb;
+    if (keep) atomicAdd(&hist[(key >> shift) & M], 1u);
+  }
+  lds_barrier();
+  for (int d = tid; d < R; d += kSortBlock) counts[g.tile * R + d] = hist[d];
+}
+
+__global__ __launch_bounds__(256) void k_radix_keep_total(const uint32_t* __restrict__ digit_tot, int R, int64_t n,
+                                                          int64_t* __restrict__ n_out) {
+  __shared__ int64_t ws[4];
+  int64_t t = 0;
+  for (int d = threadIdx.x; d < R; d += 256) t += digit_tot[d];
+#pragma unroll
+  for (int o = 32; o > 0; o >>= 1) t += __shfl_xor(t, o);
+  if ((threadIdx.x & 63) == 0) ws[threadIdx.x >> 6] = t;
+  __syncthreads();
+  if (threadIdx.x == 0) {
+    const int64_t kept = ws[0] + ws[1] + ws[2] + ws[3];
+    n_out[0] = kept;
+    n_out[1] = n - kept;
+  }
+}
+
 template <class P>
 __device__ __forceinline__ P implicit_payload(int64_t idx);
 template <>
@@ -187,7 +327,7 @@
   return make_uint2((uint32_t)idx, 0u);
 }
 
-template <class P, int RB, bool IMPLICIT>
+template <class P, int RB, bool IMPLICIT, bool KEEP = false>
 __global__ __launch_bounds__(kSortBlock) void k_radix_scatter(const uint32_t* __restrict__ keys_in,
                                                           const P* __restrict__ vals_in,
                                                           uint32_t* __restrict__ keys_out,
@@ -195,12 +335,12 @@
                                                           int shift, const uint32_t* __restrict__ counts,
                                                           const uint32_t* __restrict__ csum,
                                                           const uint32_t* __restrict__ digit_tot,
-                                                          int64_t ntiles) {
+                                                          int64_t ntiles, const uint64_t* __restrict__ mask = nullptr) {
   constexpr int R = 1 << RB;
   constexpr uint32_t M = R - 1;
   constexpr int D = digits_per_thread<R>();
   const bool own = R >= kSortBlock || (int)threadIdx.x * D < R;
-  using HistT = typename std::conditional<(RB >= 10), uint16_t, uint32_t>::type;
+  using HistT = TileHistT<RB>;
   static_assert(kTile < 65536 || RB < 10, "16-bit tile histograms need tiles below 64K keys");
   __shared__ uint32_t s_keys[kTile];
   __shared__ P s_vals[kTile];
@@ -226,6 +366,12 @@
     pcs[i] = csum[(tile / kChunk) * R + d];
     pct[i] = counts[tile * R + d];
   }
+  uint32_t keep_lo = 0, keep_hi = 0;
+  if constexpr (KEEP) {
+    const uint64_t kw = mask[tile * kMaskWords + wave * kRounds + (lane & (kRounds - 1))];
+    keep_lo = (uint32_t)kw;
+    keep_hi = (uint32_t)(kw >> 32);
+  }
 #pragma unroll
   for (int r = 0; r < kRounds; ++r) {
     const int64_t idx = wbase + (int64_t)r * 64 + lane;
@@ -253,52 +399,26 @@
   }
   lds_barrier();
 
+  uint32_t valid = 0;
 #pragma unroll
   for (int r = 0; r < kRounds; ++r) {
     const int64_t idx = wbase + (int64_t)r * 64 + lane;
-    const bool valid = idx < g.end;
-    const uint32_t d = (my_key[r] >> shift) & M;
-    uint64_t peers = __ballot(valid);
-#pragma unroll
-    for (int b = 0; b < RB; ++b) {
-      const bool bit = (d >> b) & 1u;
-      const uint64_t m = __ballot(bit);
-      peers &= bit ? m : ~m;
-    }
-    const uint32_t below = (uint32_t)__popcll(peers & lt_mask);
-    const uint32_t cnt = (uint32_t)__popcll(peers);
-    const uint32_t prev = wave_hist[wave][d];
-    __builtin_amdgcn_wave_barrier();
-    if (valid && below == 0) wave_hist[wave][d] = (HistT)(prev + cnt);
-    __builtin_amdgcn_wave_barrier();
-    my_rank[r] = valid ? prev + below : 0xFFFFFFFFu;
-  }
+    bool v = idx < g.end;
+    if constexpr (KEEP) {
+      const uint32_t lo = __builtin_amdgcn_readlane(keep_lo, r), hi = __builtin_amdgcn_readlane(keep_hi, r);
+      v = v && (((lane < 32 ? lo : hi) >> (lane & 31)) & 1u);
+    }
+    valid |= (uint32_t)v << r;
+  }
+  rank_wave_keys<RB>(my_key, valid, shift, wave_hist[wave], lt_mask, my_rank);
   lds_barrier();
 
   {
     uint32_t v[D];
-#pragma unroll
-    for (int i = 0; i < D; ++i) {
-      const int d = tid * D + i;
-      uint32_t acc = 0;
-      if (own) {
-#pragma unroll
-        for (int w = 0; w < kWaves; ++w) {
-          const uint32_t c = wave_hist[w][d];
-          wave_hist[w][d] = (HistT)acc;
-          acc += c;
-        }
-      }
-      v[i] = acc;
-    }
-    block_excl_scan<D>(v, wsum, lane, wave);
-#pragma unroll
-    for (int i = 0; i < D; ++i) {
-      if (own) {
-        tile_start[tid * D + i] = v[i];
-        glob_off[tid * D + i] -= v[i];
-      }
-    }
+    tile_digit_starts<RB>(wave_hist, tile_start, wsum, own, tid, lane, wave, v);
+#pragma unroll
+    for (int i = 0; i < D; ++i)
+      if (own) glob_off[tid * D + i] -= v[i];
   }
   lds_barrier();
 
@@ -314,7 +434,12 @@
   lds_barrier();
 
   const int64_t rem = g.end - tile_base;
-  const int tile_n = rem < kTile ? (int)rem : kTile;
+  int tile_n = rem < kTile ? (int)rem : kTile;
+  if constexpr (KEEP) {
+    tile_n = 0;
+#pragma unroll
+    for (int w = 0; w < kWaves; ++w) tile_n += (int)wsum[w];
+  }
 #pragma unroll
   for (int r = 0; r < kRounds; ++r) {
     const int j = r * kSortBlock + tid;
@@ -339,36 +464,51 @@
   vals_a.ensure(sizeof(uint64_t) * c);
   vals_b.ensure(sizeof(uint64_t) * c);
   const int64_t ntiles = (c + kTile - 1) / kTile;
-  counts.ensure(sizeof(uint32_t) * kMaxRadix * count_rows(ntiles));
+  keep_off = (int64_t)(sizeof(uint32_t) * kMaxRadix * count_rows(ntiles));
+  counts.ensure((size_t)keep_off + sizeof(uint64_t) * kMaskWords * ntiles);
   digit_tot.ensure(sizeof(uint32_t) * kMaxRadix);
   cap = c;
 }
 
 template <class P, int RB>
 static void radix_pass_impl(const uint32_t* kin, const P* vin, uint32_t* ko, P* vo, int64_t n, int shift,
-                       SortWork& w, int64_t ntiles, hipStream_t st) {
+                       SortWork& w, int64_t ntiles, hipStream_t st, bool prune = false) {
   uint32_t* counts = w.counts.as<uint32_t>();
   uint32_t* csum = counts + (ntiles + 1) * (int64_t(1) << RB);
   const int64_t nchunks = (ntiles + kChunk - 1) / kChunk;
   const bool vec = (reinterpret_cast<uintptr_t>(kin) & 15u) == 0;
-  hipLaunchKernelGGL(k_radix_count<RB>, dim3((unsigned)blocks_for_tiles(ntiles)), dim3(kSortBlock), 0, st, kin, n, shift,
-                     counts, ntiles, vec);
+  constexpr bool kCanPrune = std::is_same<P, uint2>::value && (RB == 9 || RB == 10);
+  FM_REQUIRE(kCanPrune || !prune, "pruned pass: unsupported digit");
+  bool counted = false;
+  if constexpr (kCanPrune) {
+    if (prune) {
+      hipLaunchKernelGGL(k_radix_count_keep<RB>, dim3((unsigned)blocks_for_tiles(ntiles)), dim3(kSortBlock), 0, st, kin, n,
+                         shift, counts, ntiles, w.keep());
+      counted = true;
+    }
+  }
+  if (!counted)
+    hipLaunchKernelGGL(k_radix_count<RB>, dim3((unsigned)blocks_for_tiles(ntiles)), dim3(kSortBlock), 0, st, kin, n, shift,
+                       counts, ntiles, vec);
   constexpr int TB = (1 << RB) < 256 ? (1 << RB) : 256;
   hipLaunchKernelGGL(k_radix_chunk_scan<RB>, dim3((unsigned)(nchunks * ((1 << RB) / TB))), dim3(TB), 0, st, counts,
                      ntiles, csum);
   hipLaunchKernelGGL(k_radix_chunk_top, dim3((1u << RB) / 32), dim3(256), 0, st, csum, nchunks, 1 << RB,
                      w.digit_tot.as<uint32_t>());
   auto scatter = vin ? k_radix_scatter<P, RB, false> : k_radix_scatter<P, RB, true>;
+  if constexpr (kCanPrune) {
+    if (prune) scatter = k_radix_scatter<P, RB, false, true>;
+  }
   hipLaunchKernelGGL(scatter, dim3((unsigned)blocks_for_tiles(ntiles)), dim3(kSortBlock), 0, st, kin, vin, ko, vo, n,
                      shift, (const uint32_t*)counts, (const uint32_t*)csum,
-                     (const uint32_t*)w.digit_tot.as<uint32_t>(), ntiles);
+                     (const uint32_t*)w.digit_tot.as<uint32_t>(), ntiles, (const uint64_t*)w.keep());
   FM_HIP_CHECK(hipGetLastError());
 }
 
 template <class P, int RB>
 static void radix_pass(const uint32_t* kin, const P* vin, uint32_t* ko, P* vo, int64_t n, int shift,
-                       SortWork& w, int64_t ntiles, hipStream_t st) {
-  radix_pass_impl<P, RB>(kin, vin, ko, vo, n, shift, w, ntiles, st);
+                       SortWork& w, int64_t ntiles, hipStream_t st, bool prune = false) {
+  radix_pass_impl<P, RB>(kin, vin, ko, vo, n, shift, w, ntiles, st, prune);
 }
 
 inline int digit_bits(int key_bits, int* passes) {
@@ -384,7 +524,8 @@
 template <class P>
 static void radix_sort_impl(SortWork& w, const uint32_t* keys_in, const P* vals_in, int64_t n, int key_bits,
                             hipStream_t st, const uint32_t** keys_out, const P** vals_out,
-                            uint32_t* final_keys = nullptr, P* final_vals = nullptr, int lo_bit = 0) {
+                            uint32_t* final_keys = nullptr, P* final_vals = nullptr, int lo_bit = 0,
+                            int64_t* prune_n = nullptr, int* passes_out = nullptr) {
   FM_REQUIRE(n >= 0 && n < (int64_t(1) << 32) - 1, "sort size out of range");
   w.ensure(n > 0 ? n : 1);
   if (n == 0) {
@@ -393,9 +534,18 @@
     return;
   }
   int passes = 0;
-  const int rb = digit_bits(key_bits, &passes);
+  int rb = digit_bits(key_bits, &passes);
   const int64_t ntiles = (n + kTile - 1) / kTile;
   FM_REQUIRE(ntiles < (int64_t(1) << 31), "too many sort tiles");
+  if (prune_n) {
+    if (ntiles > 1 && passes < 2) {
+      rb = kMinRB;
+      passes = 2;
+    }
+    FM_REQUIRE(vals_in != nullptr && final_keys != nullptr && lo_bit == 0 && (rb == 9 || rb == 10),
+               "pruned sort: explicit payloads, an output view, whole keys");
+  }
+  if (passes_out) *passes_out = passes;
   const uint32_t* kin = keys_in;
   const P* vin = vals_in;
   uint32_t* kbuf[2] = {w.keys_a.as<uint32_t>(), w.keys_b.as<uint32_t>()};
@@ -406,16 +556,22 @@
     const bool last = p == passes - 1 && final_keys != nullptr;
     uint32_t* ko = last ? final_keys : kbuf[which];
     P* vo = last ? final_vals : vbuf[which];
+    const bool prune = prune_n != nullptr && p == passes - 1;
     switch (rb) {
-      case 6: radix_pass<P, 6>(kin, vin, ko, vo, n, shift, w, ntiles, st); break;
-      case 7: radix_pass<P, 7>(kin, vin, ko, vo, n, shift, w, ntiles, st); break;
-      case 8: radix_pass<P, 8>(kin, vin, ko, vo, n, shift, w, ntiles, st); break;
-      case 9: radix_pass<P, 9>(kin, vin, ko, vo, n, shift, w, ntiles, st); break;
-      default: radix_pass<P, 10>(kin, vin, ko, vo, n, shift, w, ntiles, st); break;
+      case 6: radix_pass<P, 6>(kin, vin, ko, vo, n, shift, w, ntiles, st, prune); break;
+      case 7: radix_pass<P, 7>(kin, vin, ko, vo, n, shift, w, ntiles, st, prune); break;
+      case 8: radix_pass<P, 8>(kin, vin, ko, vo, n, shift, w, ntiles, st, prune); break;
+      case 9: radix_pass<P, 9>(kin, vin, ko, vo, n, shift, w, ntiles, st, prune); break;
+      default: radix_pass<P, 10>(kin, vin, ko, vo, n, shift, w, ntiles, st, prune); break;
     }
     kin = ko;
     vin = vo;
     which ^= 1;
+  }
+  if (prune_n) {
+    hipLaunchKernelGGL(k_radix_keep_total, dim3(1), dim3(256), 0, st, (const uint32_t*)w.digit_tot.as<uint32_t>(), 1 << rb,
+                       n, prune_n);
+    FM_HIP_CHECK(hipGetLastError());
   }
   *keys_out = kin;
   *vals_out = vin;
@@ -440,4 +596,16 @@
   radix_sort_impl<uint2>(w, keys_in, vals_in, n, key_bits, st, keys_out, vals_out, final_keys, final_vals);
 }
 
-}
+void radix_sort_pairs64_pruned(SortWork& w, const uint32_t* keys_in, const uint2* vals_in, int64_t n, int key_bits,
+                               hipStream_t st, uint32_t* final_keys, uint2* final_vals, int64_t* n_out, int* passes) {
+  FM_REQUIRE(n_out != nullptr, "pruned sort: null n_out");
+  if (passes) *passes = 0;
+  if (n == 0) FM_HIP_CHECK(hipMemsetAsync(n_out, 0, 2 * sizeof(int64_t), st));
+  const uint32_t* ko = nullptr;
+  const uint2* vo = nullptr;
+  radix_sort_impl<uint2>(w, keys_in, vals_in, n, key_bits, st, &ko, &vo, final_keys, final_vals, 0, n_out, passes);
+}
+
+int sort_tile_keys() { return kTile; }
+
+}
diff --git a/fm_spark_amd/csrc/fm_update.hip b/fm_spark_amd/csrc/fm_update.hip
--- a/fm_spark_amd/csrc/fm_update.hip
+++ b/fm_spark_amd/csrc/fm_update.hip
@@ -626,12 +626,13 @@
   }
 }
 
-__global__ __launch_bounds__(kBlock) void k_split_count(const uint32_t* __restrict__ skeys, int64_t N,
-                                                        uint2* __restrict__ cnt, int64_t nchunks, TableView T,
-                                                        int32_t epoch) {
+__global__ __launch_bounds__(kBlock) void k_split_count(const uint32_t* __restrict__ skeys,
+                                                        const int64_t* __restrict__ n_in, uint2* __restrict__ cnt,
+                                                        TableView T, int32_t epoch) {
   const int lane = threadIdx.x & 63;
   const int64_t c = (int64_t)blockIdx.x * (kBlock / 64) + (threadIdx.x >> 6);
-  if (c >= nchunks) return;
+  const int64_t N = n_in[0];
+  if (c * kSplitChunk >= N) return;
   SplitChunk sc;
   split_chunk(skeys, N, c, lane, sc);
   const uint32_t tag = sc.multi & sc.first;
@@ -655,9 +656,11 @@
 
 constexpr int kSplitPer = 12;
 constexpr int kSplitScanNT = 1024;
-__global__ __launch_bounds__(kSplitScanNT) void k_split_scan(const uint2* __restrict__ cnt, int64_t nchunks,
+__global__ __launch_bounds__(kSplitScanNT) void k_split_scan(const uint2* __restrict__ cnt,
+                                                             const int64_t* __restrict__ n_in,
                                                              int64_t* __restrict__ off, int64_t* __restrict__ n_out) {
   constexpr int NW = kSplitScanNT / 64;
+  const int64_t nchunks = (n_in[0] + kSplitChunk - 1) / kSplitChunk;
   __shared__ int64_t wsum[NW], ssum[NW];
   const int lane = threadIdx.x & 63, wave = threadIdx.x >> 6;
   int64_t carry = 0, singles = 0;
@@ -704,17 +707,19 @@
   }
   if (threadIdx.x == 0) {
     n_out[0] = carry;
-    n_out[1] = singles;
+    n_out[1] = singles + n_in[1];
   }
 }
 
 __global__ __launch_bounds__(kBlock) void k_split_scatter(const uint32_t* __restrict__ skeys,
-                                                          const uint2* __restrict__ sents, int64_t N,
-                                                          const int64_t* __restrict__ off, int64_t nchunks,
+                                                          const uint2* __restrict__ sents,
+                                                          const int64_t* __restrict__ n_in,
+                                                          const int64_t* __restrict__ off,
                                                           uint32_t* __restrict__ mkeys, uint2* __restrict__ ments) {
   const int lane = threadIdx.x & 63;
   const int64_t c = (int64_t)blockIdx.x * (kBlock / 64) + (threadIdx.x >> 6);
-  if (c >= nchunks) return;
+  const int64_t N = n_in[0];
+  if (c * kSplitChunk >= N) return;
   const uint64_t lt = lane == 0 ? 0ull : (~0ull >> (64 - lane));
   const int64_t base = c * kSplitChunk;
   uint2 en[kSplitRows];
@@ -739,8 +744,8 @@
   }
 }
 
-void launch_split(const uint32_t* skeys, const uint2* sents, int64_t N, SplitWork& sw, uint32_t* mkeys, uint2* ments,
-                  int64_t* n_out, hipStream_t st, const TableView& tag_T, int32_t epoch) {
+void launch_split(const uint32_t* skeys, const uint2* sents, int64_t N, const int64_t* n_in, SplitWork& sw,
+                  uint32_t* mkeys, uint2* ments, int64_t* n_out, hipStream_t st, const TableView& tag_T, int32_t epoch) {
   const int64_t nchunks = (N + kSplitChunk - 1) / kSplitChunk;
   sw.cnt.ensure_slack(sizeof(uint2) * (size_t)std::max<int64_t>(nchunks, 1));
   sw.off.ensure_slack(sizeof(int64_t) * (size_t)std::max<int64_t>(nchunks, 1));
@@ -749,11 +754,10 @@
     return;
   }
   const unsigned blocks = (unsigned)((nchunks + kBlock / 64 - 1) / (kBlock / 64));
-  hipLaunchKernelGGL(k_split_count, dim3(blocks), dim3(kBlock), 0, st, skeys, N, sw.cnt.as<uint2>(), nchunks, tag_T,
-                     epoch);
-  hipLaunchKernelGGL(k_split_scan, dim3(1), dim3(kSplitScanNT), 0, st, sw.cnt.as<uint2>(), nchunks, sw.off.as<int64_t>(), n_out);
-  hipLaunchKernelGGL(k_split_scatter, dim3(blocks), dim3(kBlock), 0, st, skeys, sents, N, sw.off.as<int64_t>(), nchunks,
-                     mkeys, ments);
+  hipLaunchKernelGGL(k_split_count, dim3(blocks), dim3(kBlock), 0, st, skeys, n_in, sw.cnt.as<uint2>(), tag_T, epoch);
+  hipLaunchKernelGGL(k_split_scan, dim3(1), dim3(kSplitScanNT), 0, st, sw.cnt.as<uint2>(), n_in, sw.off.as<int64_t>(), n_out);
+  hipLaunchKernelGGL(k_split_scatter, dim3(blocks), dim3(kBlock), 0, st, skeys, sents, n_in, sw.off.as<int64_t>(), mkeys,
+                     ments);
   FM_HIP_CHECK(hipGetLastError());
 }
 void launch_segment_update(const TableView& T, const BatchDev& b, StepWork& w, const StepParams& p,
diff --git a/fm_spark_amd/engine.py b/fm_spark_amd/engine.py
--- a/fm_spark_amd/engine.py
+++ b/fm_spark_amd/engine.py
@@ -90,6 +90,11 @@
 
     def prepare(self):
         N.check(self._lib.fm_batch_prepare(self.ctx.handle, self.handle), "fm_batch_prepare")
+
+    def view_stats(self):
+        out = (C.c_int64 * 4)()
+        N.check(self._lib.fm_batch_view_stats(self.ctx.handle, self.handle, out), "fm_batch_view_stats")
+        return tuple(int(v) for v in out)
 
     def close(self):
         if self.handle:
diff --git a/include/fm_hip.h b/include/fm_hip.h
--- a/include/fm_hip.h
+++ b/include/fm_hip.h
@@ -89,6 +89,7 @@
 int fm_batch_create(fm_ctx* ctx, const fm_csr* csr, fm_batch** out);
 void fm_batch_destroy(fm_batch* b);
 int fm_batch_prepare(fm_ctx* ctx, fm_batch* batch);
+int fm_batch_view_stats(fm_ctx* ctx, const fm_batch* batch, int64_t out[4]);
 int fm_batch_from_rows(fm_ctx* ctx, const fm_batch* data, const int64_t* rows, int64_t n, fm_batch** out);
 int fm_batch_create_splits(fm_ctx* ctx, const fm_csr* csr, int32_t n_splits, const int64_t* split_rows,
                            fm_batch** out);
```

Result: no change. 322.6 million samples/s (-0.8%).
